# JuanJoZP/cfd-hemodynamic

Measured on AMD Instinct MI355X. Metric: time-steps/sec, dfg_1 ~1M DOF (stabilized_schur), higher is better.
Workload: dtype f64 (fp32 only in the AMG matrix values of the flexible preconditioner and in a read-only copy of the Krylov basis that Gram-Schmidt reads in solves of >= 20 iterations)

## Files before the change

### cfd_hemodynamic_amd/_lib.py

```python
from __future__ import annotations

import ctypes as C
import os
import subprocess

import numpy as np

_HERE = os.path.dirname(os.path.abspath(__file__))
_SO = os.path.join(_HERE, "libcfdh.so")
_LIB = None

dp = C.POINTER(C.c_double)
ip = C.POINTER(C.c_int32)
lp = C.POINTER(C.c_int64)


class Options(C.Structure):
    _fields_ = [
        ("snes_rtol", C.c_double), ("snes_atol", C.c_double), ("snes_stol", C.c_double), ("snes_max_it", C.c_int32),
        ("ksp_rtol", C.c_double), ("ksp_atol", C.c_double), ("ksp_max_it", C.c_int32), ("ksp_restart", C.c_int32),
        ("cheb_degree", C.c_int32), ("cheb_ratio", C.c_double), ("schur_full", C.c_int32),
        ("amg_smooth_degree", C.c_int32), ("amg_smooth_ratio", C.c_double), ("amg_theta", C.c_double),
        ("amg_max_coarse", C.c_int32), ("pc_refresh", C.c_int32), ("remove_p_mean", C.c_int32), ("verbose", C.c_int32),
        ("pc_type", C.c_int32), ("cc_smooth_degree", C.c_int32), ("ksp_guess", C.c_int32),
    ]


class Stats(C.Structure):
    _fields_ = [
        ("newton_its", C.c_int32), ("krylov_its", C.c_int32), ("reason", C.c_int32), ("pc_refreshes", C.c_int32),
        ("fnorm0", C.c_double), ("fnorm", C.c_double), ("ms_assemble", C.c_double), ("ms_solve", C.c_double),
        ("ms_pc_setup", C.c_double), ("ms_total", C.c_double),
    ]


class IpcsStats(C.Structure):
    _fields_ = [
        ("its", C.c_int32 * 3), ("reason", C.c_int32 * 3), ("rel_res", C.c_double * 3), ("ms_assemble", C.c_double),
        ("ms_solve", C.c_double * 3), ("ms_total", C.c_double), ("launches", C.c_int32), ("host_syncs", C.c_int32),
    ]


ALLREDUCE_FN = C.CFUNCTYPE(C.c_int, C.c_void_p, dp, C.c_int, C.c_int)
EXCHANGE_FN = C.CFUNCTYPE(C.c_int, C.c_void_p, dp, dp)

SYMBOLS = [
    "cfdh_create", "cfdh_create_elem", "cfdh_create_elem_part", "cfdh_set_facet_markers", "cfdh_destroy", "cfdh_last_error", "cfdh_abi_version", "cfdh_set_params", "cfdh_default_options",
    "cfdh_set_options", "cfdh_clear_dirichlet", "cfdh_add_dirichlet", "cfdh_update_dirichlet", "cfdh_set_state", "cfdh_get_solution",
    "cfdh_get_previous", "cfdh_get_residual", "cfdh_advance", "cfdh_advance_field", "cfdh_set_time_scheme", "cfdh_set_previous2", "cfdh_get_previous2",
    "cfdh_shift_history", "cfdh_set_boundary_terms", "cfdh_set_formulation", "cfdh_set_pressure_boundaries", "cfdh_assemble", "cfdh_get_csr", "cfdh_spmv", "cfdh_solve_step",
    "cfdh_functional", "cfdh_wall_shear_stress", "cfdh_set_global_pressure_space", "cfdh_set_halo", "cfdh_comm_unique_id", "cfdh_comm_init", "cfdh_comm_set_callbacks",
    "cfdh_profile_enable", "cfdh_profile_get", "cfdh_profile_reset", "cfdh_info",
    "cfdh_set_schur_pcd", "cfdh_set_ksp_forcing", "cfdh_get_newton_history", "cfdh_get_pcd_operator", "cfdh_apply_preconditioner",
    "cfdh_get_amg_operator", "cfdh_get_amg_vectors",
    "cfdh_create_ipcs", "cfdh_ipcs_set_form", "cfdh_ipcs_set_tolerances", "cfdh_ipcs_step", "cfdh_ipcs_get_operator", "cfdh_ipcs_get_intermediate",
    "cfdh_ipcs_apply_pressure_pc",
]


def build(force=False):
    src = os.path.join(_HERE, "csrc")
    newest = max(os.path.getmtime(os.path.join(src, f)) for f in os.listdir(src)
                 if f.endswith((".hip", ".cpp", ".hpp", ".h")))
    hdr = os.path.join(os.path.dirname(_HERE), "include", "cfdh.h")
    if os.path.exists(hdr):
        newest = max(newest, os.path.getmtime(hdr))
    if force or not os.path.exists(_SO) or os.path.getmtime(_SO) < newest:
        if not os.path.exists("/opt/rocm/bin/hipcc") and os.path.exists(_SO):
            return _SO
        subprocess.check_call(["make", "-C", src, "-s", "-j4"])
    return _SO


def lib():
    global _LIB
    if _LIB is not None:
        return _LIB
    if not os.path.exists(_SO):
        raise RuntimeError(
            "libcfdh.so is missing (%s): build it with `python -c 'import __graft_entry__ as g; g.build()'`; "
            "this package has no CPU fallback" % _SO)
    L = C.CDLL(_SO)
    vp = C.c_void_p
    L.cfdh_create.argtypes = [C.POINTER(vp), C.c_int, C.c_int, C.c_int64, C.c_int64, C.c_int64, ip, dp, C.c_int64, ip, ip, ip]
    L.cfdh_create_elem.argtypes = [C.POINTER(vp), C.c_int, C.c_int, C.c_int, C.c_int64, C.c_int64, ip, dp, C.c_int64, ip, ip, ip]
    L.cfdh_create_elem_part.argtypes = [C.POINTER(vp), C.c_int, C.c_int, C.c_int, C.c_int64, C.c_int64, C.c_int64, ip, dp, C.c_int64, ip, ip, ip]
    L.cfdh_set_facet_markers.argtypes = [vp, C.c_int64, ip]
    L.cfdh_destroy.argtypes = [vp]
    L.cfdh_destroy.restype = None
    L.cfdh_last_error.argtypes = [vp]
    L.cfdh_last_error.restype = C.c_char_p
    L.cfdh_set_params.argtypes = [vp, C.c_double, C.c_double, C.c_double, C.c_double, dp]
    L.cfdh_default_options.argtypes = [C.POINTER(Options)]
    L.cfdh_set_options.argtypes = [vp, C.POINTER(Options)]
    L.cfdh_clear_dirichlet.argtypes = [vp]
    L.cfdh_add_dirichlet.argtypes = [vp, C.c_int, C.c_int64, ip, dp]
    L.cfdh_update_dirichlet.argtypes = [vp, C.c_int, C.c_int64, ip, dp]
    L.cfdh_set_state.argtypes = [vp, dp, dp, dp, dp]
    L.cfdh_get_solution.argtypes = [vp, dp, dp]
    L.cfdh_set_time_scheme.argtypes = [vp, C.c_double, C.c_double, C.c_double, C.c_double]
    L.cfdh_set_previous2.argtypes = [vp, dp]
    L.cfdh_get_previous2.argtypes = [vp, dp]
    L.cfdh_shift_history.argtypes = [vp]
    L.cfdh_wall_shear_stress.argtypes = [vp, dp]
    L.cfdh_set_boundary_terms.argtypes = [vp, C.c_int, C.c_int, C.c_double]
    L.cfdh_set_formulation.argtypes = [vp, C.c_int]
    L.cfdh_set_pressure_boundaries.argtypes = [vp, C.c_int, ip, dp, C.c_double]
    L.cfdh_get_residual.argtypes = [vp, dp, dp]
    L.cfdh_get_previous.argtypes = [vp, dp, dp]
    L.cfdh_advance.argtypes = [vp]
    L.cfdh_advance_field.argtypes = [vp, C.c_int]
    L.cfdh_assemble.argtypes = [vp, C.c_int]
    L.cfdh_get_csr.argtypes = [vp, lp, ip, ip, dp]
    L.cfdh_spmv.argtypes = [vp, dp, dp]
    L.cfdh_solve_step.argtypes = [vp, C.POINTER(Stats)]
    L.cfdh_functional.argtypes = [vp, C.c_int, C.c_int, dp]
    L.cfdh_set_halo.argtypes = [vp, C.c_int, ip, lp, ip, lp, ip]
    L.cfdh_set_global_pressure_space.argtypes = [vp, C.c_int64, C.c_int64, ip, dp, ip, C.c_int64, ip]
    L.cfdh_comm_unique_id.argtypes = [C.c_void_p]
    L.cfdh_comm_init.argtypes = [vp, C.c_void_p, C.c_int, C.c_int]
    L.cfdh_comm_set_callbacks.argtypes = [vp, ALLREDUCE_FN, EXCHANGE_FN, C.c_void_p, C.c_int, C.c_int]
    L.cfdh_profile_enable.argtypes = [vp, C.c_int]
    L.cfdh_profile_get.argtypes = [vp, C.c_int, dp, lp]
    L.cfdh_profile_reset.argtypes = [vp]
    L.cfdh_info.argtypes = [vp, C.c_int]
    L.cfdh_info.restype = C.c_int64
    L.cfdh_set_schur_pcd.argtypes = [vp, C.c_int, C.c_int, C.c_int]
    L.cfdh_set_ksp_forcing.argtypes = [vp, C.c_int, C.c_double, C.c_double, C.c_double, C.c_double, C.c_double]
    L.cfdh_get_newton_history.argtypes = [vp, ip, dp, dp, ip, dp]
    L.cfdh_get_pcd_operator.argtypes = [vp, lp, ip, ip, dp, dp]
    L.cfdh_apply_preconditioner.argtypes = [vp, dp, dp]
    L.cfdh_get_amg_operator.argtypes = [vp, C.c_int, C.c_int, C.c_int, lp, lp, lp, ip, ip, dp]
    L.cfdh_get_amg_vectors.argtypes = [vp, C.c_int, C.c_int, C.c_int, lp, dp]
    L.cfdh_create_ipcs.argtypes = [C.POINTER(vp), C.c_int, C.c_int, C.c_int64, C.c_int64, C.c_int64, ip, dp, C.c_int64, ip, ip, ip]
    L.cfdh_ipcs_set_form.argtypes = [vp, C.c_double, C.c_double]
    L.cfdh_ipcs_set_tolerances.argtypes = [vp, dp, C.c_double, ip]
    L.cfdh_ipcs_step.argtypes = [vp, C.POINTER(IpcsStats)]
    L.cfdh_ipcs_get_operator.argtypes = [vp, C.c_int, lp, ip, ip, dp]
    L.cfdh_ipcs_get_intermediate.argtypes = [vp, C.c_int, dp]
    L.cfdh_ipcs_apply_pressure_pc.argtypes = [vp, dp, dp]
    _LIB = L
    return L


def _dp(a):
    return None if a is None else a.ctypes.data_as(dp)


def _ip(a):
    return None if a is None else a.ctypes.data_as(ip)


def _lp(a):
    return None if a is None else a.ctypes.data_as(lp)


class CfdhError(RuntimeError):
    pass


def _raise(code, msg):
    if code == -1:
        raise ValueError(msg)
    raise CfdhError(msg)


FORM_CONVECTIVE, FORM_ROTATIONAL = 0, 1
PC_SELFP, PC_CAHOUET_CHABARD, PC_PCD = 0, 1, 2
AMG_HIER_A, AMG_HIER_P, AMG_HIER_H = 0, 1, 2
AMG_OP_A, AMG_OP_P, AMG_OP_G, AMG_OP_SB, AMG_OP_SC = 0, 1, 2, 3, 4
(AMG_VEC_DINV, AMG_VEC_WDINV, AMG_VEC_AGG, AMG_VEC_COARSE_INV, AMG_VEC_D, AMG_VEC_LAMBDA, AMG_VEC_CC_SCALARS, AMG_VEC_CC_ML,
 AMG_VEC_CC_PBC, AMG_VEC_SPGEMM_ROWS, AMG_VEC_SHAPE, AMG_VEC_ORDER, AMG_VEC_A00_LMAX, AMG_VEC_A00_DINV) = range(14)
EW_DEFAULTS = (0.3, 0.9, 1.0, (1.0 + 5.0 ** 0.5) / 2.0, 0.1)


class Context:

    def __init__(self, x, cells, facet_cells, facet_local, facet_marker, nv_owned=None, device=0, etype=0):
        L = lib()
        self.L = L
        x = np.asarray(x, dtype=np.float64)
        cells = np.asarray(cells)
        self.etype = int(etype)
        self.dim = (3 if x.shape[1] >= 3 and cells.shape[1] in (8, 10) or (self.etype == 3 and cells.shape[1] == 4) else 2) if self.etype \
            else cells.shape[1] - 1
        if self.dim not in (2, 3) or x.shape[1] < self.dim:
            raise ValueError("cells must be triangles [nc,3] or tetrahedra [nc,4] with matching coordinates")
        nodes = {(1, 2): 6, (2, 2): 4, (3, 2): 3, (1, 3): 10, (2, 3): 8, (3, 3): 4}
        if self.etype and cells.shape[1] != nodes[(self.etype, self.dim)]:
            raise ValueError("element type %d needs %d nodes per cell for gdim %d" % (self.etype, nodes[(self.etype, self.dim)], self.dim))
        self.x = np.ascontiguousarray(x[:, : self.dim]).copy()
        self.cells = np.ascontiguousarray(cells, dtype=np.int32)
        self.nv = len(self.x)
        self.nvo = self.nv if nv_owned is None else int(nv_owned)
        fc = np.ascontiguousarray(facet_cells, dtype=np.int32)
        fl = np.ascontiguousarray(facet_local, dtype=np.int32)
        fm = np.ascontiguousarray(facet_marker, dtype=np.int32)
        h = C.c_void_p()
        if self.etype:
            if self.nvo != self.nv:
                rc = L.cfdh_create_elem_part(C.byref(h), int(device), self.dim, self.etype, self.nv, self.nvo, len(self.cells), _ip(self.cells),
                                             _dp(self.x), len(fc), _ip(fc), _ip(fl), _ip(fm))
            else:
                rc = L.cfdh_create_elem(C.byref(h), int(device), self.dim, self.etype, self.nv, len(self.cells), _ip(self.cells), _dp(self.x),
                                        len(fc), _ip(fc), _ip(fl), _ip(fm))
        else:
            rc = L.cfdh_create(C.byref(h), int(device), self.dim, self.nv, self.nvo, len(self.cells), _ip(self.cells), _dp(self.x),
                               len(fc), _ip(fc), _ip(fl), _ip(fm))
        if rc != 0:
            _raise(rc, "cfdh_create failed: " + L.cfdh_last_error(None).decode())
        self.h = h
        self._cb = None

    def close(self):
# ... 135 lines not shown
        if rc != 0:
            msg = self.L.cfdh_last_error(self.h).decode()
            if rc == -4:
                raise RuntimeError("Did not converge, reason: %d. (%s)" % (st.reason, msg))
            _raise(rc, msg)
        return st

    def functional(self, kind, marker=0):
        out = C.c_double()
        self._chk(self.L.cfdh_functional(self.h, int(kind), int(marker), C.byref(out)))
        return out.value

    def set_halo(self, nbr_rank, send_ptr, send_idx, recv_ptr, recv_idx):
        a = np.ascontiguousarray(nbr_rank, dtype=np.int32)
        sp_ = np.ascontiguousarray(send_ptr, dtype=np.int64)
        si = np.ascontiguousarray(send_idx, dtype=np.int32)
        rp = np.ascontiguousarray(recv_ptr, dtype=np.int64)
        ri = np.ascontiguousarray(recv_idx, dtype=np.int32)
        self._chk(self.L.cfdh_set_halo(self.h, len(a), _ip(a), _lp(sp_), _ip(si), _lp(rp), _ip(ri)))

    def set_global_pressure_space(self, x_global, cells_global, owned_global, pbc_nodes_global):
        xg = np.ascontiguousarray(x_global, dtype=np.float64)[:, : self.dim].copy()
        cg = np.ascontiguousarray(cells_global, dtype=np.int32)
        og = np.ascontiguousarray(owned_global, dtype=np.int32)
        pb = np.ascontiguousarray(pbc_nodes_global, dtype=np.int32)
        self._chk(self.L.cfdh_set_global_pressure_space(self.h, len(xg), len(cg), _ip(cg), _dp(xg), _ip(og), len(pb), _ip(pb)))

    def comm_init_rccl(self, uid_bytes, rank, nranks):
        buf = C.create_string_buffer(bytes(uid_bytes), 128)
        self._chk(self.L.cfdh_comm_init(self.h, buf, int(rank), int(nranks)))

    def comm_set_callbacks(self, allreduce, exchange, rank, nranks):
        self._cb = (ALLREDUCE_FN(allreduce), EXCHANGE_FN(exchange))
        self._chk(self.L.cfdh_comm_set_callbacks(self.h, self._cb[0], self._cb[1], None, int(rank), int(nranks)))

    def profile_enable(self, on=True):
        self._chk(self.L.cfdh_profile_enable(self.h, int(on)))

    def profile_reset(self):
        self._chk(self.L.cfdh_profile_reset(self.h))

    def profile_get(self, kind):
        ms, n = C.c_double(), C.c_int64()
        self._chk(self.L.cfdh_profile_get(self.h, int(kind), C.byref(ms), C.byref(n)))
        return ms.value, n.value

    def info(self, what):
        return int(self.L.cfdh_info(self.h, int(what)))

    def set_schur_pcd(self, inlet_marker, outlet_marker, time_term=1):
        self._chk(self.L.cfdh_set_schur_pcd(self.h, int(inlet_marker), int(outlet_marker), int(time_term)))

    def set_ksp_forcing(self, version=2, rtol_0=None, rtol_max=None, gamma=None, alpha=None, threshold=None):
        a = [d if v is None else float(v) for v, d in zip((rtol_0, rtol_max, gamma, alpha, threshold), EW_DEFAULTS)]
        self._chk(self.L.cfdh_set_ksp_forcing(self.h, int(version), *a))

    def newton_history(self):
        n = C.c_int32()
        self._chk(self.L.cfdh_get_newton_history(self.h, C.byref(n), None, None, None, None))
        fn, rt, rr = np.zeros(n.value), np.zeros(n.value), np.zeros(n.value)
        its = np.zeros(n.value, dtype=np.int32)
        self._chk(self.L.cfdh_get_newton_history(self.h, C.byref(n), _dp(fn), _dp(rt), _ip(its), _dp(rr)))
        return {"fnorm": fn, "ksp_rtol": rt, "ksp_its": its, "ksp_rel_res": rr}

    def get_pcd_operator(self):
        import scipy.sparse as sp
        nnz = C.c_int64()
        self._chk(self.L.cfdh_get_pcd_operator(self.h, C.byref(nnz), None, None, None, None))
        rowptr = np.empty(self.nvo + 1, dtype=np.int32)
        col = np.empty(nnz.value, dtype=np.int32)
        val = np.empty(nnz.value)
        md = np.empty(self.nvo)
        self._chk(self.L.cfdh_get_pcd_operator(self.h, C.byref(nnz), _ip(rowptr), _ip(col), _dp(val), _dp(md)))
        return sp.csr_matrix((val, col, rowptr), shape=(self.nvo, self.nv)), md

    def apply_preconditioner(self, r):
        r = np.ascontiguousarray(r, dtype=np.float64)
        if r.size != (self.dim + 1) * self.nv:
            raise ValueError("monolithic vector of (gdim + 1) nv entries expected")
        z = np.zeros_like(r)
        self._chk(self.L.cfdh_apply_preconditioner(self.h, _dp(r), _dp(z)))
        return z

    def get_amg_operator(self, hier, level, which, raw=False):
        import scipy.sparse as sp
        nr, nc, nnz = C.c_int64(), C.c_int64(), C.c_int64()
        self._chk(self.L.cfdh_get_amg_operator(self.h, int(hier), int(level), int(which), C.byref(nr), C.byref(nc), C.byref(nnz), None, None, None))
        rowptr = np.empty(nr.value + 1, dtype=np.int32)
        col = np.empty(nnz.value, dtype=np.int32)
        val = np.empty(nnz.value)
        self._chk(self.L.cfdh_get_amg_operator(self.h, int(hier), int(level), int(which), C.byref(nr), C.byref(nc), C.byref(nnz), _ip(rowptr),
                                               _ip(col), _dp(val)))
        if raw:
            return rowptr, col, val, (nr.value, nc.value), nnz.value
        return sp.csr_matrix((val, col, rowptr), shape=(nr.value, nc.value))

    def get_amg_vectors(self, hier, level, which):
        n = C.c_int64()
        self._chk(self.L.cfdh_get_amg_vectors(self.h, int(hier), int(level), int(which), C.byref(n), None))
        out = np.empty(n.value)
        self._chk(self.L.cfdh_get_amg_vectors(self.h, int(hier), int(level), int(which), C.byref(n), _dp(out)))
        return out


class IpcsContext(Context):

    def __init__(self, x, cells, nvert, facet_cells, facet_local, facet_marker, device=0):
        L = lib()
        self.L = L
        cells = np.ascontiguousarray(cells, dtype=np.int32)
        if cells.ndim != 2 or cells.shape[1] not in (6, 10):
            raise ValueError("cells must list the 6 nodes of P2 triangles or the 10 nodes of P2 tetrahedra")
        self.dim = 2 if cells.shape[1] == 6 else 3
        self.etype = 1
        self.x = np.ascontiguousarray(np.asarray(x, dtype=np.float64)[:, : self.dim]).copy()
        self.cells = cells
        self.nv = self.nvo = len(self.x)
        self.nvert = int(nvert)
        fc = np.ascontiguousarray(facet_cells, dtype=np.int32)
        fl = np.ascontiguousarray(facet_local, dtype=np.int32)
        fm = np.ascontiguousarray(facet_marker, dtype=np.int32)
        h = C.c_void_p()
        rc = L.cfdh_create_ipcs(C.byref(h), int(device), self.dim, self.nv, self.nvert, len(cells), _ip(cells), _dp(self.x), len(fc), _ip(fc), _ip(fl),
                                _ip(fm))
        if rc != 0:
            _raise(rc, "cfdh_create_ipcs failed: " + L.cfdh_last_error(None).decode())
        self.h = h
        self._cb = None

    def set_state(self, u_prev=None, p_prev=None, u=None, p=None):
        a = [None if v is None else np.ascontiguousarray(v, dtype=np.float64).reshape(-1) for v in (u_prev, p_prev, u, p)]
        for v, n in zip(a, (self.dim * self.nv, self.nvert, self.dim * self.nv, self.nvert)):
            if v is not None and v.size != n:
                raise ValueError("state array has wrong size")
        self._chk(self.L.cfdh_set_state(self.h, _dp(a[0]), _dp(a[1]), _dp(a[2]), _dp(a[3])))

    def get_solution(self, u=None, p=None):
        u = np.empty(self.dim * self.nv) if u is None else u
        p = np.empty(self.nvert) if p is None else p
        self._chk(self.L.cfdh_get_solution(self.h, _dp(u), _dp(p)))
        return u, p

    def get_previous(self, u=None, p=None):
        u = np.empty(self.dim * self.nv) if u is None else u
        p = np.empty(self.nvert) if p is None else p
        self._chk(self.L.cfdh_get_previous(self.h, _dp(u), _dp(p)))
        return u, p

    def set_form(self, conv_coeff, force_coeff):
        self._chk(self.L.cfdh_ipcs_set_form(self.h, float(conv_coeff), float(force_coeff)))

    def set_tolerances(self, rtol=(1e-5, 1e-5, 1e-5), atol=1e-50, max_it=(10000, 10000, 10000)):
        r = np.ascontiguousarray(np.broadcast_to(np.asarray(rtol, dtype=np.float64), (3,)))
        m = np.ascontiguousarray(np.broadcast_to(np.asarray(max_it, dtype=np.int32), (3,)))
        self._chk(self.L.cfdh_ipcs_set_tolerances(self.h, _dp(r), float(atol), _ip(m)))

    def step(self):
        st = IpcsStats()
        rc = self.L.cfdh_ipcs_step(self.h, C.byref(st))
        if rc != 0:
            msg = self.L.cfdh_last_error(self.h).decode()
            if rc == -4:
                bad = [r for r in st.reason if r <= 0]
                raise RuntimeError("Did not converge, reason: %d. (%s)" % (bad[0] if bad else 0, msg))
            _raise(rc, msg)
        return st
# ... 35 lines not shown
```

### cfd_hemodynamic_amd/csrc/cfdh_api.cpp

```cpp
#include <algorithm>
#include <cmath>
#include <numeric>

#include <dlfcn.h>

#include "cfdh_internal.hpp"
#include "cfdh_ipcs.hpp"

std::string g_cfdh_last_error;

int cfdh_prepare_assembly(cfdh_ctx *c);

#define ENTER(c)                         \
  do {                                   \
    if (!(c)) return CFDH_E_ARG;         \
    (void)hipSetDevice((c)->device);     \
  } while (0)

#define NOT_IPCS(c, name)                                                                                                    \
  do {                                                                                                                       \
    if ((c) && (c)->ipcs) return cfdh_fail((c), CFDH_E_STATE, name ": not available on an incremental pressure-correction context (cfdh_create_ipcs)"); \
  } while (0)
#define NEED_IPCS(c, name)                                                                                         \
  do {                                                                                                             \
    if (!(c)) return CFDH_E_ARG;                                                                                   \
    if (!(c)->ipcs) return cfdh_fail((c), CFDH_E_STATE, name ": the context was not created by cfdh_create_ipcs"); \
    (void)hipSetDevice((c)->device);                                                                               \
  } while (0)

static int ipcs_put(cfdh_ctx *c, dbuf<double> &dst, const double *src) {
  if (!src) return 0;
  c->ipcs->n_field_copies++;
  HIPCHK(c, hipMemcpyAsync(dst.p, src, sizeof(double) * dst.n, hipMemcpyHostToDevice, c->stream));
  HIPCHK(c, hipStreamSynchronize(c->stream));
  return 0;
}
static int ipcs_get(cfdh_ctx *c, const dbuf<double> &src, double *dst) {
  if (!dst) return 0;
  c->ipcs->n_field_copies++;
  HIPCHK(c, hipMemcpyAsync(dst, src.p, sizeof(double) * src.n, hipMemcpyDeviceToHost, c->stream));
  HIPCHK(c, hipStreamSynchronize(c->stream));
  return 0;
}
static int ipcs_copy(cfdh_ctx *c, const dbuf<double> &src, dbuf<double> &dst) {
  HIPCHK(c, hipMemcpyAsync(dst.p, src.p, sizeof(double) * src.n, hipMemcpyDeviceToDevice, c->stream));
  return 0;
}

extern "C" {

int cfdh_abi_version(void) { return CFDH_ABI_VERSION; }

const char *cfdh_last_error(const cfdh_ctx *c) { return c ? c->err.c_str() : g_cfdh_last_error.c_str(); }

int cfdh_default_options(cfdh_options *o) {
  if (!o) return CFDH_E_ARG;
  o->snes_rtol = 1e-8; o->snes_atol = 1e-50; o->snes_stol = 1e-8; o->snes_max_it = 100;
  o->ksp_rtol = 1e-5; o->ksp_atol = 1e-50; o->ksp_max_it = 1000; o->ksp_restart = 200;
  o->cheb_degree = 3; o->cheb_ratio = 10.0; o->schur_full = 2;
  o->amg_smooth_degree = 1; o->amg_smooth_ratio = 8.0; o->amg_theta = -1.0; o->amg_max_coarse = 1000;
  o->pc_refresh = 0; o->remove_p_mean = 1; o->verbose = 0; o->pc_type = 1; o->cc_smooth_degree = 2;
  o->ksp_guess = getenv("CFDH_KSP_GUESS") ? atoi(getenv("CFDH_KSP_GUESS")) : 4;
  return 0;
}

static int create_ctx(cfdh_ctx **out, int device, int gdim, int etype, int64_t nv, int64_t nv_owned, int64_t nc, const int32_t *cells,
                      const double *coords, int64_t nfacets, const int32_t *facet_cells, const int32_t *facet_local,
                      const int32_t *facet_marker) {
  if (!out) return cfdh_fail(nullptr, CFDH_E_ARG, "null output pointer");
  *out = nullptr;
  if (gdim != 2 && gdim != 3) return cfdh_fail(nullptr, CFDH_E_ARG, "gdim must be 2 (P1 triangles) or 3 (P1 tetrahedra)");
  if (etype < 0 || etype > 3) return cfdh_fail(nullptr, CFDH_E_ARG, "unknown element type %d", etype);
  if (!cells || !coords || (nfacets > 0 && (!facet_cells || !facet_local)))
    return cfdh_fail(nullptr, CFDH_E_ARG, "null mesh array");
  int ndev = 0;
  if (hipGetDeviceCount(&ndev) != hipSuccess || ndev <= 0)
    return cfdh_fail(nullptr, CFDH_E_HIP, "no HIP device available: libcfdh has no CPU fallback");
  if (device < 0 || device >= ndev) return cfdh_fail(nullptr, CFDH_E_ARG, "device %d out of range (%d devices)", device, ndev);
  cfdh_ctx *c = new (std::nothrow) cfdh_ctx();
  if (!c) return cfdh_fail(nullptr, CFDH_E_NOMEM, "out of host memory");
  c->device = device;
  cfdh_default_options(&c->opt);
  { const char *e = getenv("CFDH_NO_GRAPH"); c->use_graph = !(e && e[0] == '1'); }
  if (c->use_graph && (getenv("ROCP_TOOL_LIBRARIES") || dlsym(RTLD_DEFAULT, "rocprofiler_configure"))) {
    int rt = 0;
    const char *ov = getenv("CFDH_GRAPH_UNDER_PROFILER");
    if (!(ov && ov[0] == '1') && hipRuntimeGetVersion(&rt) == hipSuccess && rt >= 70200000) c->use_graph = false;
  }
  memset(&c->last_stats, 0, sizeof c->last_stats);
  int rc = 0;
  do {
    if (hipSetDevice(device) != hipSuccess) { rc = cfdh_fail(nullptr, CFDH_E_HIP, "hipSetDevice(%d) failed", device); break; }
    if (hipStreamCreateWithFlags(&c->stream, hipStreamNonBlocking) != hipSuccess) { rc = cfdh_fail(nullptr, CFDH_E_HIP, "hipStreamCreate failed"); break; }
    rc = gdim == 3 ? k3_upload_quadrature(c) : k_upload_quadrature(c);
    if (rc) break;
    if (etype != 0) {
      rc = gdim == 3 ? kg3_upload_tables(c) : kg_upload_tables(c);
      if (rc) break;
      rc = gdim == 3 ? cfdh_build_mesh_gen3(c, etype, nv, nv_owned, nc, cells, coords, nfacets, facet_cells, facet_local, facet_marker)
                     : cfdh_build_mesh_gen(c, etype, nv, nv_owned, nc, cells, coords, nfacets, facet_cells, facet_local, facet_marker);
      break;
    }
    rc = gdim == 3 ? cfdh_build_mesh3(c, nv, nv_owned, nc, cells, coords, nfacets, facet_cells, facet_local, facet_marker)
                   : cfdh_build_mesh(c, nv, nv_owned, nc, cells, coords, nfacets, facet_cells, facet_local, facet_marker);
  } while (0);
  if (rc) {
    g_cfdh_last_error = c->err.empty() ? g_cfdh_last_error : c->err;
    cfdh_destroy(c);
    return rc;
  }
  *out = c;
  return 0;
}

int cfdh_create(cfdh_ctx **out, int device, int gdim, int64_t nv, int64_t nv_owned, int64_t nc, const int32_t *cells,
                const double *coords, int64_t nfacets, const int32_t *facet_cells, const int32_t *facet_local,
                const int32_t *facet_marker) {
  return create_ctx(out, device, gdim, CFDH_ELEM_P1, nv, nv_owned, nc, cells, coords, nfacets, facet_cells, facet_local, facet_marker);
}

int cfdh_create_elem(cfdh_ctx **out, int device, int gdim, int elem, int64_t nn, int64_t nc, const int32_t *cells, const double *node_coords,
                     int64_t nfacets, const int32_t *facet_cells, const int32_t *facet_local, const int32_t *facet_marker) {
  return create_ctx(out, device, gdim, elem, nn, nn, nc, cells, node_coords, nfacets, facet_cells, facet_local, facet_marker);
}

int cfdh_create_elem_part(cfdh_ctx **out, int device, int gdim, int elem, int64_t nn, int64_t nn_owned, int64_t nc, const int32_t *cells,
                          const double *node_coords, int64_t nfacets, const int32_t *facet_cells, const int32_t *facet_local, const int32_t *facet_marker) {
  return create_ctx(out, device, gdim, elem, nn, nn_owned, nc, cells, node_coords, nfacets, facet_cells, facet_local, facet_marker);
}

void cfdh_destroy(cfdh_ctx *c) {
  if (!c) return;
  (void)hipSetDevice(c->device);
  if (c->stream) (void)hipStreamSynchronize(c->stream);
  cfdh_ipcs_free(c);
  comm_finalize(c);
  c->hS.clear(); c->hL.clear(); c->hA.clear(); c->hLg.clear();
  for (hipEvent_t e : c->ev_pool) (void)hipEventDestroy(e);
  for (auto &e : c->pc_graphs) for (auto &x : e.exec) if (x) (void)hipGraphExecDestroy(x);
  if (c->h_pinned) (void)hipHostFree(c->h_pinned);
  if (c->h_stage) (void)hipHostFree(c->h_stage);
  if (c->ev_h) (void)hipEventDestroy(c->ev_h);
  if (c->h_big) (void)hipHostFree(c->h_big);
  if (c->h_ring) (void)hipHostFree(c->h_ring);
  for (hipEvent_t e : c->ev_ring) if (e) (void)hipEventDestroy(e);
  hipStream_t s = c->stream;
  delete c;
  if (s) (void)hipStreamDestroy(s);
}

int cfdh_set_params(cfdh_ctx *c, double dt, double rho, double mu, double mu_facet, const double f[3]) {
  ENTER(c);
  if (!(dt > 0) || !(rho > 0) || !(mu > 0)) return cfdh_fail(c, CFDH_E_ARG, "dt, rho, mu must be positive");
  const bool changed = !c->params_set || dt != c->dt || rho != c->rho || mu != c->mu;
  c->dt = dt; c->rho = rho; c->mu = mu; c->muf = mu_facet;
  c->f[0] = f ? f[0] : 0.0; c->f[1] = f ? f[1] : 0.0; c->f[2] = (f && c->dim == 3) ? f[2] : 0.0;
  c->params_set = true;
  if (changed) { c->mom_valid = false; c->pc_valid = false; }
  if (c->ipcs) c->ipcs->assembled = false;
  return 0;
}

int cfdh_set_options(cfdh_ctx *c, const cfdh_options *o) {
  if (!c || !o) return CFDH_E_ARG;
  if (o->ksp_restart < 1 || o->ksp_restart > 1000 || o->cheb_degree < 1 || o->cc_smooth_degree < 1 || !(o->cheb_ratio > 1) || o->amg_smooth_degree < 1 ||
      !(o->amg_smooth_ratio > 1) || o->amg_max_coarse < 8 || o->amg_max_coarse > 4000 || o->ksp_guess < 0 || o->ksp_guess > 8)
    return cfdh_fail(c, CFDH_E_ARG, "option out of range");
  const bool pc_changed = o->amg_theta != c->opt.amg_theta || o->amg_max_coarse != c->opt.amg_max_coarse ||
                          o->amg_smooth_ratio != c->opt.amg_smooth_ratio || o->pc_type != c->opt.pc_type ||
                          o->amg_smooth_degree != c->opt.amg_smooth_degree ||
                          o->schur_full != c->opt.schur_full;
  c->opt = *o;
  if (pc_changed) c->pc_valid = false;
  if (pc_changed && c->ipcs) c->ipcs->pset_dirty = true;
  c->pc_graph_valid = false;
  return 0;
// ... 332 lines not shown
      return cfdh_fail(c, CFDH_E_ARG, "cfdh_set_pressure_boundaries: pressure boundaries need the rotational formulation (cfdh_set_formulation)");
  }
  bool same = (size_t)n == c->pb_markers.size() && beta_nitsche == c->pb_beta;
  for (int k = 0; same && k < n; k++) same = markers[k] == c->pb_markers[k];
  c->pb_values.assign(values, values + n);
  if (same) return 0;
  c->pb_markers.assign(markers, markers + n);
  c->pb_beta = beta_nitsche;
  return upload_cell_facet_flags(c);
}

int cfdh_set_schur_pcd(cfdh_ctx *c, int inlet_marker, int outlet_marker, int time_term) {
  NOT_IPCS(c, "cfdh_set_schur_pcd");
  ENTER(c);
  if (c->gen) return cfdh_fail(c, CFDH_E_ARG, "cfdh_set_schur_pcd: PCD exists for P1 triangles and tetrahedra on the closed-form kernels only");
  if (c->nranks > 1 || c->nvo != c->nv) return cfdh_fail(c, CFDH_E_ARG, "cfdh_set_schur_pcd: PCD is not available in partitioned runs");
  if (time_term != 0 && time_term != 1) return cfdh_fail(c, CFDH_E_ARG, "cfdh_set_schur_pcd: time_term must be 0 or 1");
  const bool markers_changed = !c->pcd_set || inlet_marker != c->pcd_in || outlet_marker != c->pcd_out;
  c->pcd_in = inlet_marker; c->pcd_out = outlet_marker; c->pcd_time = time_term;
  c->pcd_set = true;
  if (markers_changed) { c->pcd_ready = false; c->pc_valid = false; }
  return 0;
}

int cfdh_set_ksp_forcing(cfdh_ctx *c, int version, double rtol_0, double rtol_max, double gamma, double alpha, double threshold) {
  NOT_IPCS(c, "cfdh_set_ksp_forcing");
  ENTER(c);
  if (version != 0 && version != 2) return cfdh_fail(c, CFDH_E_ARG, "cfdh_set_ksp_forcing: version 0 (off) or 2");
  if (version == 2 && !(rtol_0 > 0 && rtol_0 < 1 && rtol_max > 0 && rtol_max < 1 && gamma > 0 && gamma <= 1 && alpha > 1 && alpha <= 2 &&
                        threshold > 0 && threshold < 1))
    return cfdh_fail(c, CFDH_E_ARG, "cfdh_set_ksp_forcing: need 0 < rtol_0, rtol_max, threshold < 1, 0 < gamma <= 1, 1 < alpha <= 2");
  c->ew_version = version;
  if (version == 2) { c->ew_rtol0 = rtol_0; c->ew_rtol_max = rtol_max; c->ew_gamma = gamma; c->ew_alpha = alpha; c->ew_threshold = threshold; }
  return 0;
}

int cfdh_get_newton_history(cfdh_ctx *c, int32_t *n, double *fnorm, double *ksp_rtol, int32_t *ksp_its, double *ksp_rel_res) {
  NOT_IPCS(c, "cfdh_get_newton_history");
  if (!c || !n) return CFDH_E_ARG;
  const size_t m = c->hist_fnorm.size();
  *n = (int32_t)m;
  for (size_t k = 0; k < m; k++) {
    if (fnorm) fnorm[k] = c->hist_fnorm[k];
    if (ksp_rtol) ksp_rtol[k] = c->hist_rtol[k];
    if (ksp_its) ksp_its[k] = c->hist_its[k];
    if (ksp_rel_res) ksp_rel_res[k] = c->hist_relres[k];
  }
  return 0;
}

int cfdh_get_pcd_operator(cfdh_ctx *c, int64_t *nnz, int32_t *rowptr, int32_t *col, double *vals, double *mass_diag) {
  NOT_IPCS(c, "cfdh_get_pcd_operator");
  if (!c || !nnz) return CFDH_E_ARG;
  ENTER(c);
  *nnz = c->nnzv;
  if (!rowptr && !col && !vals && !mass_diag) return 0;
  if (!rowptr || !col || !vals) return cfdh_fail(c, CFDH_E_ARG, "pass all of rowptr/col/vals or none");
  if (c->gen || c->nranks > 1 || c->nvo != c->nv) return cfdh_fail(c, CFDH_E_ARG, "cfdh_get_pcd_operator: P1 contexts on one GPU only");
  if (!c->pcd_set) return cfdh_fail(c, CFDH_E_STATE, "cfdh_get_pcd_operator: cfdh_set_schur_pcd was not called");
  if (!c->params_set || !c->state_set) return cfdh_fail(c, CFDH_E_STATE, "cfdh_get_pcd_operator: parameters and state are needed");
  CHK(k_pcd_assemble(c, c->x.p));
  std::vector<double> K(c->pcd_K.n);
  std::vector<int> sptr(c->pcd_sptr.n);
  HIPCHK(c, hipMemcpyAsync(K.data(), c->pcd_K.p, sizeof(double) * K.size(), hipMemcpyDeviceToHost, c->stream));
  HIPCHK(c, hipMemcpyAsync(sptr.data(), c->pcd_sptr.p, sizeof(int) * sptr.size(), hipMemcpyDeviceToHost, c->stream));
  HIPCHK(c, hipStreamSynchronize(c->stream));
  const int nvo = c->nvo;
  int64_t pos = 0;
  std::vector<std::pair<int, int>> ord;
  for (int vu = 0; vu < nvo; vu++) {
    const int r = c->perm[vu];
    ord.clear();
    for (int k = c->h_vptr[r]; k < c->h_vptr[r + 1]; k++) ord.push_back({c->iperm[c->h_vcol[k]], k - c->h_vptr[r]});
    std::sort(ord.begin(), ord.end());
    rowptr[vu] = (int32_t)pos;
    const size_t base = (size_t)sptr[r >> 6] + (r & 63);
    for (auto &e : ord) { col[pos] = e.first; vals[pos] = K[base + 64 * (size_t)e.second]; pos++; }
  }
  rowptr[nvo] = (int32_t)pos;
  if (mass_diag) for (int vu = 0; vu < nvo; vu++) mass_diag[vu] = c->h_pcd_md[c->perm[vu]];
  return 0;
}

int cfdh_apply_preconditioner(cfdh_ctx *c, const double *r, double *z) {
  NOT_IPCS(c, "cfdh_apply_preconditioner");
  if (!c || !r || !z) return CFDH_E_ARG;
  ENTER(c);
  if (!c->jac_valid) return cfdh_fail(c, CFDH_E_STATE, "no Jacobian assembled yet");
  CHK(cfdh_pc_update(c, false));
  std::vector<double> h;
  pack_vec(c, r, r + (size_t)c->dim * c->nv, h, nullptr);
  CHK(upload_vec(c, h, c->xt.p));
  CHK(cfdh_pc_apply(c, c->xt.p, c->dvec.p));
  std::vector<double> o;
  CHK(download_vec(c, c->dvec.p, o));
  for (int k = 0; k < c->nvo; k++) {
    const int v = c->iperm[k], d = c->dim;
    for (int i = 0; i < d; i++) z[(size_t)d * v + i] = o[(size_t)d * k + i];
    z[(size_t)d * c->nv + v] = o[(size_t)d * c->nvo + k];
  }
  return 0;
}

static int amg_pick(cfdh_ctx *c, const char *name, int hier, int level, AmgHier **H, AmgLevel **L) {
  if (c->nranks > 1 || c->nvo != c->nv) return cfdh_fail(c, CFDH_E_STATE, "%s: one GPU only", name);
  if (!c->pc_valid) return cfdh_fail(c, CFDH_E_STATE, "%s: no preconditioner built yet (cfdh_apply_preconditioner or cfdh_solve_step first)", name);
  *H = nullptr;
  if (hier == CFDH_AMG_HIER_H) {
    if (c->opt.pc_type != 1 || c->Hlev.n <= 0) return cfdh_fail(c, CFDH_E_STATE, "%s: H exists for pc_type 1 only", name);
    *L = &c->Hlev;
    return 0;
  }
  if (hier != CFDH_AMG_HIER_A && hier != CFDH_AMG_HIER_P) return cfdh_fail(c, CFDH_E_ARG, "%s: unknown hierarchy %d", name, hier);
  if (hier == CFDH_AMG_HIER_A && c->opt.pc_type == 0) return cfdh_fail(c, CFDH_E_STATE, "%s: pc_type 0 has no velocity hierarchy", name);
  AmgHier *h = hier == CFDH_AMG_HIER_A ? &c->hA : (c->opt.pc_type == 0 ? &c->hS : &c->hL);
  if (!h->valid) return cfdh_fail(c, CFDH_E_STATE, "%s: hierarchy %d is not built", name, hier);
  if (level < 0 || level >= (int)h->lev.size()) return cfdh_fail(c, CFDH_E_ARG, "%s: level %d of %d", name, level, (int)h->lev.size());
  *H = h;
  *L = h->lev[level];
  return 0;
}

int cfdh_get_amg_operator(cfdh_ctx *c, int hier, int level, int which, int64_t *nrow, int64_t *ncol, int64_t *nnz, int32_t *rowptr,
                          int32_t *col, double *vals) {
  NOT_IPCS(c, "cfdh_get_amg_operator");
  if (!c || !nrow || !ncol || !nnz) return CFDH_E_ARG;
  ENTER(c);
  AmgHier *H = nullptr;
  AmgLevel *L = nullptr;
  CHK(amg_pick(c, "cfdh_get_amg_operator", hier, level, &H, &L));
  if (which < CFDH_AMG_OP_A || which > CFDH_AMG_OP_SC) return cfdh_fail(c, CFDH_E_ARG, "cfdh_get_amg_operator: unknown operator %d", which);
  if (!H) level = 0;
  const CsrDev &M = which == CFDH_AMG_OP_A ? L->A : which == CFDH_AMG_OP_P ? L->P : which == CFDH_AMG_OP_G ? L->G : which == CFDH_AMG_OP_SB ? L->Sb : L->Sc;
  if (M.n <= 0 || !M.rowptr.p || !M.col.p || !M.val.p)
    return cfdh_fail(c, CFDH_E_STATE, "cfdh_get_amg_operator: operator %d of level %d is not kept in fp64 CSR (P: CFDH_AMG_KEEP=1 before the build)", which, level);
  *nrow = M.n; *ncol = M.m; *nnz = M.nnz;
  if (!rowptr && !col && !vals) return 0;
  if (!rowptr || !col || !vals) return cfdh_fail(c, CFDH_E_ARG, "pass all of rowptr/col/vals or none");
  std::vector<int> rp((size_t)M.n + 1), cl((size_t)M.nnz);
  std::vector<double> vl((size_t)M.nnz);
  HIPCHK(c, hipMemcpyAsync(rp.data(), M.rowptr.p, sizeof(int) * rp.size(), hipMemcpyDeviceToHost, c->stream));
  if (M.nnz > 0) {
    HIPCHK(c, hipMemcpyAsync(cl.data(), M.col.p, sizeof(int) * cl.size(), hipMemcpyDeviceToHost, c->stream));
    HIPCHK(c, hipMemcpyAsync(vl.data(), M.val.p, sizeof(double) * vl.size(), hipMemcpyDeviceToHost, c->stream));
  }
  HIPCHK(c, hipStreamSynchronize(c->stream));
  if (rp[M.n] != M.nnz) return cfdh_fail(c, CFDH_E_STATE, "cfdh_get_amg_operator: rowptr ends at %d, the operator holds %d entries", rp[M.n], M.nnz);
  const bool rows0 = level == 0 && which != CFDH_AMG_OP_G && (int)c->perm.size() == M.n;
  const bool cols0 = level == 0 && (which == CFDH_AMG_OP_A || which == CFDH_AMG_OP_SB || which == CFDH_AMG_OP_G) && (int)c->iperm.size() == M.m;
  int64_t pos = 0;
  std::vector<std::pair<int, double>> row;
  for (int ru = 0; ru < M.n; ru++) {
    const int r = rows0 ? c->perm[ru] : ru;
    rowptr[ru] = (int32_t)pos;
    row.clear();
    for (int k = rp[r]; k < rp[r + 1]; k++) row.push_back({cols0 ? c->iperm[cl[k]] : cl[k], vl[k]});
    if (cols0) std::stable_sort(row.begin(), row.end(), [](const std::pair<int, double> &a, const std::pair<int, double> &b) { return a.first < b.first; });
    for (auto &e : row) { col[pos] = e.first; vals[pos] = e.second; pos++; }
  }
  rowptr[M.n] = (int32_t)pos;
  return 0;
}

int cfdh_get_amg_vectors(cfdh_ctx *c, int hier, int level, int which, int64_t *n, double *out) {
  NOT_IPCS(c, "cfdh_get_amg_vectors");
  if (!c || !n) return CFDH_E_ARG;
  ENTER(c);
  AmgHier *H = nullptr;
  AmgLevel *L = nullptr;
  CHK(amg_pick(c, "cfdh_get_amg_vectors", hier, level, &H, &L));
  if (!H) level = 0;
  const bool perm0 = level == 0 && (int)c->perm.size() == L->n;
  auto fetch = [&](const void *src, size_t bytes, void *dst) -> int {
    HIPCHK(c, hipMemcpyAsync(dst, src, bytes, hipMemcpyDeviceToHost, c->stream));
    HIPCHK(c, hipStreamSynchronize(c->stream));
    return 0;
  };
  const int nvo = c->nvo;
  switch (which) {
    case CFDH_AMG_VEC_DINV:
    case CFDH_AMG_VEC_WDINV: {
      const dbuf<double> &v = which == CFDH_AMG_VEC_DINV ? L->dinv : L->wdinv;
// ... 444 lines not shown
      case 26: return I->D;
      case 29: return I->NL;
      case 80: return I->last.launches;
      case 81: return I->nvert;
      case 82: return I->n_field_copies;
      case 83: return 1;
      default: return -1;
    }
  }
  switch (what) {
    case 0: return c->nvo;
    case 1: return c->nv;
    case 2: return c->nc;
    case 3: return c->nnzv;
    case 4: return c->opt.pc_type >= 1 ? c->hL.fine_nnz : c->hS.fine_nnz;
    case 5: return c->ninc;
    case 6: return (int64_t)(c->opt.pc_type >= 1 ? c->hL.lev.size() : c->hS.lev.size());
    case 7: return c->nblk;
    case 8: return c->hA.fine_nnz;
    case 9: return c->gp_allgather ? c->gp_maxcnt : 0;
    case 10: return c->nccl_comm ? 1 : 0;
    case 11: return c->dl0.on ? c->dl0.n1 : 0;
    case 12: return c->ras ? 1 : 0;
    case 13: return c->n_allreduce;
    case 14: return c->n_halo;
    case 15: return c->n_host_sync;
    case 16: return c->n_krylov;
    case 17: return c->n_allgather;
    case 18: return c->nranks;
    case 26: return c->dim;
    case 30: case 31: case 32: case 33: case 34: case 35: case 36: case 37: case 38: case 39:
    case 40: case 41: case 42: case 43: case 44: case 45: case 46: case 47: case 48: case 49:
    case 50: case 51: case 52: case 53: case 54: case 55: case 56: case 57: case 58: case 59:
    case 60: case 61: case 62: case 63: case 64: case 65: case 66: case 67: case 68: case 69: {
      const AmgHier &h = what < 50 ? c->hA : (c->opt.pc_type >= 1 ? c->hL : c->hS);
      const size_t l = (size_t)(what % 10);
      if (l >= h.lev.size()) return 0;
      return ((what / 10) & 1) ? (int64_t)h.lev[l]->n : (int64_t)h.lev[l]->A.nnz;
    }
    case 28: return c->etype;
    case 70: return c->n_guess_solves;
    case 71: return c->n_guess_solves ? (int64_t)(1e6 * c->guess_reduction_sum / (double)c->n_guess_solves) : 0;
    case 29: return c->nloc;
    case 73: return c->n_krylov_discarded;
    case 74: return c->n_pc_builds;
    case 75: return c->pc_valid ? 1 : 0;
    case 76: return c->singular;
    case 77: return c->form;
    case 78: return c->opt.pc_type;
    case 79: return c->ew_version;
    case 72: return c->n_attainable_stops;
    case 27: return (int64_t)(1000.0 * c->ms_pc_build_dev);
    case 19: return c->opt.pc_type >= 1 ? c->hL.nnz_S0 : c->hS.nnz_S0;
    case 20: return c->hA.nnz_S0;
    case 21: return c->opt.pc_type >= 1 ? c->hL.nnz_G0 : c->hS.nnz_G0;
    case 22: return c->hA.nnz_G0;
    case 23: { const AmgHier &h = c->opt.pc_type >= 1 ? c->hL : c->hS; return h.lev.size() > 1 ? h.lev[1]->n : 0; }
    case 24: return c->hA.lev.size() > 1 ? c->hA.lev[1]->n : 0;
    case 25: { const AmgHier &h = c->opt.pc_type >= 1 ? c->hL : c->hS; return h.fused ? 1 : 0; }
    default: return -1;
  }
}


int cfdh_create_ipcs(cfdh_ctx **out, int device, int gdim, int64_t nn, int64_t nvert, int64_t nc, const int32_t *cells, const double *node_coords,
                     int64_t nfacets, const int32_t *facet_cells, const int32_t *facet_local, const int32_t *facet_marker) {
  if (!out) return cfdh_fail(nullptr, CFDH_E_ARG, "null output pointer");
  *out = nullptr;
  if (gdim != 2 && gdim != 3) return cfdh_fail(nullptr, CFDH_E_ARG, "gdim must be 2 (P2/P1 triangles) or 3 (P2/P1 tetrahedra)");
  if (!cells || !node_coords || nfacets < 0 || (nfacets > 0 && (!facet_cells || !facet_local))) return cfdh_fail(nullptr, CFDH_E_ARG, "null mesh array");
  int ndev = 0;
  if (hipGetDeviceCount(&ndev) != hipSuccess || ndev <= 0)
    return cfdh_fail(nullptr, CFDH_E_HIP, "no HIP device available: libcfdh has no CPU fallback");
  if (device < 0 || device >= ndev) return cfdh_fail(nullptr, CFDH_E_ARG, "device %d out of range (%d devices)", device, ndev);
  cfdh_ctx *c = new (std::nothrow) cfdh_ctx();
  if (!c) return cfdh_fail(nullptr, CFDH_E_NOMEM, "out of host memory");
  c->device = device;
  cfdh_default_options(&c->opt);
  c->use_graph = false;
  memset(&c->last_stats, 0, sizeof c->last_stats);
  int rc = 0;
  if (hipSetDevice(device) != hipSuccess) rc = cfdh_fail(nullptr, CFDH_E_HIP, "hipSetDevice(%d) failed", device);
  else if (hipStreamCreateWithFlags(&c->stream, hipStreamNonBlocking) != hipSuccess) rc = cfdh_fail(nullptr, CFDH_E_HIP, "hipStreamCreate failed");
  else rc = cfdh_ipcs_create(c, gdim, nn, nvert, nc, cells, node_coords, nfacets, facet_cells, facet_local, facet_marker);
  if (rc) {
    g_cfdh_last_error = c->err.empty() ? g_cfdh_last_error : c->err;
    cfdh_destroy(c);
    return rc;
  }
  *out = c;
  return 0;
}

int cfdh_ipcs_set_form(cfdh_ctx *c, double conv_coeff, double force_coeff) {
  NEED_IPCS(c, "cfdh_ipcs_set_form");
  if (!(conv_coeff >= 0) || !std::isfinite(conv_coeff) || !std::isfinite(force_coeff)) return cfdh_fail(c, CFDH_E_ARG, "cfdh_ipcs_set_form: conv_coeff >= 0 and finite coefficients");
  c->ipcs->conv_coeff = conv_coeff; c->ipcs->force_coeff = force_coeff; c->ipcs->force_default = false;
  c->ipcs->assembled = false;
  return 0;
}

int cfdh_ipcs_set_tolerances(cfdh_ctx *c, const double rtol[3], double atol, const int32_t max_it[3]) {
  NEED_IPCS(c, "cfdh_ipcs_set_tolerances");
  if (!rtol || !max_it || !(atol >= 0)) return cfdh_fail(c, CFDH_E_ARG, "cfdh_ipcs_set_tolerances: bad arguments");
  for (int k = 0; k < 3; k++)
    if (!(rtol[k] >= 0) || !(rtol[k] < 1) || max_it[k] < 1) return cfdh_fail(c, CFDH_E_ARG, "cfdh_ipcs_set_tolerances: 0 <= rtol < 1, max_it >= 1");
  for (int k = 0; k < 3; k++) { c->ipcs->rtol[k] = rtol[k]; c->ipcs->max_it[k] = max_it[k]; }
  c->ipcs->atol = atol;
  return 0;
}

int cfdh_ipcs_step(cfdh_ctx *c, cfdh_ipcs_stats *stats) {
  NEED_IPCS(c, "cfdh_ipcs_step");
  c->err.clear();
  cfdh_ipcs_stats st;
  const int rc = cfdh_ipcs_step_impl(c, &st);
  if (stats) *stats = st;
  return rc;
}

int cfdh_ipcs_get_operator(cfdh_ctx *c, int which, int64_t *nnz, int32_t *rowptr, int32_t *col, double *vals) {
  NEED_IPCS(c, "cfdh_ipcs_get_operator");
  IpcsData *I = c->ipcs;
  const int D = I->D;
  if (!nnz || which < 0 || which >= 3 + 2 * D) return cfdh_fail(c, CFDH_E_ARG, "cfdh_ipcs_get_operator: which in [0, %d)", 3 + 2 * D);
  const std::vector<int> &ptr = which == 1 ? I->hL.rowptr : which < 3 ? I->hM.rowptr : which < 3 + D ? I->bptr : I->gptr;
  const std::vector<int> &cl = which == 1 ? I->hL.col : which < 3 ? I->hM.col : which < 3 + D ? I->bcol : I->gcol;
  *nnz = (int64_t)cl.size();
  if (!rowptr && !col && !vals) return 0;
  if (!rowptr || !col || !vals) return cfdh_fail(c, CFDH_E_ARG, "pass all of rowptr/col/vals or none");
  std::copy(ptr.begin(), ptr.end(), rowptr);
  std::copy(cl.begin(), cl.end(), col);
  if (which >= 3) {
    const std::vector<double> &v = which < 3 + D ? I->hB : I->hG;
    const int d = which < 3 + D ? which - 3 : which - 3 - D;
    for (size_t k = 0; k < cl.size(); k++) vals[k] = v[(size_t)D * k + d];
    return 0;
  }
  if (which == 0) {
    if (!I->assembled) CHK(cfdh_ipcs_assemble(c));
  } else {
    if (!c->params_set) return cfdh_fail(c, CFDH_E_STATE, "cfdh_set_params was not called");
    I->assembled = false;
    CHK(cfdh_ipcs_assemble(c));
  }
  const double *src = which == 0 ? I->A1v.p : which == 1 ? I->Lv.p : I->RMv.p;
  HIPCHK(c, hipMemcpyAsync(vals, src, sizeof(double) * cl.size(), hipMemcpyDeviceToHost, c->stream));
  HIPCHK(c, hipStreamSynchronize(c->stream));
  return 0;
}

int cfdh_ipcs_get_intermediate(cfdh_ctx *c, int which, double *out) {
  NEED_IPCS(c, "cfdh_ipcs_get_intermediate");
  IpcsData *I = c->ipcs;
  if (!out || which < 0 || which > 4) return cfdh_fail(c, CFDH_E_ARG, "cfdh_ipcs_get_intermediate: which in [0, 4]");
  const dbuf<double> *src[5] = {&I->us, &I->phi, &I->b1, &I->b2, &I->b3};
  I->n_field_copies++;
  HIPCHK(c, hipMemcpyAsync(out, src[which]->p, sizeof(double) * src[which]->n, hipMemcpyDeviceToHost, c->stream));
  HIPCHK(c, hipStreamSynchronize(c->stream));
  return 0;
}

int cfdh_ipcs_apply_pressure_pc(cfdh_ctx *c, const double *r, double *z) {
  NEED_IPCS(c, "cfdh_ipcs_apply_pressure_pc");
  if (!r || !z) return cfdh_fail(c, CFDH_E_ARG, "cfdh_ipcs_apply_pressure_pc: null array");
  return cfdh_ipcs_apply_pc(c, r, z);
// ... 4 lines not shown
```

### cfd_hemodynamic_amd/csrc/cfdh_internal.hpp

```cpp
#pragma once
#include <hip/hip_runtime.h>

#include <cstdint>
#include <cstdio>
#include <cstring>
#include <string>
#include <vector>

#include "cfdh.h"

#ifndef CFDH_MAX_INC
#define CFDH_MAX_INC 256
#endif
#ifndef CFDH_MAX_BV
#define CFDH_MAX_BV 192
#endif
#ifndef CFDH_MAX_BC
#define CFDH_MAX_BC 192
#endif
#ifndef CFDH_MAX_ROWS
#define CFDH_MAX_ROWS 128
#endif

#if defined(__HIPCC__)
__device__ __forceinline__ double cfdh_rsqrt(double x) {
  double y = __builtin_amdgcn_rsq(x);
  const double h = 0.5 * x;
  y = __builtin_fma(y, __builtin_fma(-h * y, y, 0.5), y);
  y = __builtin_fma(y, __builtin_fma(-h * y, y, 0.5), y);
  return y;
}
#endif

template <class T>
struct dbuf {
  T *p = nullptr;
  size_t n = 0;
  dbuf() = default;
  dbuf(const dbuf &) = delete;
  dbuf &operator=(const dbuf &) = delete;
  ~dbuf() { release(); }
  void release() {
    if (p) (void)hipFree(p);
    p = nullptr;
    n = 0;
  }
  hipError_t alloc(size_t count) {
    if (count == n && p) return hipSuccess;
    release();
    if (count == 0) return hipSuccess;
    hipError_t e = hipMalloc((void **)&p, count * sizeof(T));
    if (e == hipSuccess) n = count;
    return e;
  }
  hipError_t upload(const std::vector<T> &h, hipStream_t s) {
    hipError_t e = alloc(h.size());
    if (e != hipSuccess || h.empty()) return e;
    return hipMemcpyAsync(p, h.data(), h.size() * sizeof(T), hipMemcpyHostToDevice, s);
  }
  hipError_t zero(hipStream_t s) { return n ? hipMemsetAsync(p, 0, n * sizeof(T), s) : hipSuccess; }
  void adopt(dbuf &o) {
    if (&o == this) return;
    release();
    p = o.p; n = o.n;
    o.p = nullptr; o.n = 0;
  }
};

struct CsrHost {
  int n = 0, m = 0;
  std::vector<int> rowptr, col;
  std::vector<double> val;
  int nnz() const { return (int)col.size(); }
};

struct CsrDev {
  int n = 0, m = 0, nnz = 0;
  dbuf<int> rowptr, col;
  dbuf<double> val;
  int nslice = 0, sell_maxw = 0;
  dbuf<int> sptr, scol;
  dbuf<float> sval, svalw;
  dbuf<float> valf;
};
enum { CFDH_UP_CSR = 1, CFDH_UP_SELL = 2, CFDH_UP_CSRF = 4};

struct AmgLevel {
  int n = 0;
  CsrDev A, P, R;
  dbuf<double> dinv, wdinv, x, b, r, d0, d1;
  double lmax = 0, lmin = 0;
  CsrDev G, Sb, Sc;
  dbuf<float> D;
  int Dn = 0;
  bool fine = false;
  bool sell = false;
  dbuf<int> agg;
};

struct AmgHier {
  std::vector<AmgLevel *> lev;
  dbuf<double> coarse_inv;
  int coarse_n = 0, ncol = 1;
  long long fine_nnz = 0;
  bool valid = false;
  bool fused = false;
  long long nnz_G0 = 0, nnz_S0 = 0;
  long long spgemm_rows[3] = {0, 0, 0};
  bool keep_host0 = false;
  CsrHost h_A0, h_P0;
  std::vector<double> h_wdinv0;
  void clear() {
    for (AmgLevel *l : lev) delete l;
    lev.clear();
    valid = false;
// ... 59 lines not shown
  bool jac_valid = false;

  int ninc = 0, nblk = 0;
  bool gs_refine_long = false;
  dbuf<unsigned> inc_slot;
  dbuf<unsigned> inc_rank;
  dbuf<int> blk_row;
  dbuf<int> blk_vptr, blk_vlist;
  dbuf<int> blk_cptr, blk_clist;
  dbuf<unsigned> inc_loc;
  dbuf<int> wave_maxlen;

  int a3_nblk = 0;
  dbuf<int> a3_blk_row, a3_blk_iptr;
  dbuf<int> a3_inc_cell;
  dbuf<int> a3_inc_row;
  dbuf<unsigned long long> a3_inc_slots;

  std::vector<unsigned char> h_bcflag;
  std::vector<double> h_bcval;
  std::vector<double> h_bcmult;
  bool bc_dirty = true;
  std::vector<int> bc_touched, bc_pending;
  size_t bc_touched_sent = 0;
  std::vector<int> bc_mark;
  int bc_epoch = 0;
  bool bc_full_upload = true;
  dbuf<int> bc_uidx;
  dbuf<unsigned char> bc_uflag;
  dbuf<double> bc_uval, bc_umult;
  int n_pbc = 0;
  dbuf<unsigned char> bcflag;
  dbuf<double> bcval, bcmult;

  dbuf<int> d_fac_cell, d_fac_local, d_fac_marker;

  dbuf<double> x, xt, xprev, xprev2, F, dvec;
  dbuf<double> wss;
  double ts_theta = 0.5, ts_a[3] = {1.0, -1.0, 0.0};
  bool ds_terms = true;
  double bf_beta = 0.0;
  int bf_marker = -1;
  int form = 0;
  std::vector<int> pb_markers;
  std::vector<double> pb_values;
  double pb_beta = 0.0;
  bool state_set = false;

  dbuf<double> red_partial, red_out;
  double *h_pinned = nullptr;
  double *h_stage = nullptr;
  double *h_pinned_dev = nullptr;
  const double *mirror_src = nullptr;
  int mirror_cnt = 0;
  hipEvent_t ev_h = nullptr;
  static constexpr int KRING = 12;
  double *h_ring = nullptr, *h_ring_dev = nullptr;
  size_t h_ring_stride = 0;
  hipEvent_t ev_ring[KRING] = {};
  long long n_krylov_discarded = 0;
  int red_blocks = 0;

  int kry_m = 0;
  static constexpr int GUESS_NEWTON = 4;
  dbuf<double> guessU, guessX;
  bool guess_stored[GUESS_NEWTON] = {false, false, false, false};
  int guess_m = 0, guess_slot = -1;
  int guess_cnt[GUESS_NEWTON] = {0, 0, 0, 0}, guess_head[GUESS_NEWTON] = {0, 0, 0, 0};
  long long n_guess_solves = 0;
  double guess_reduction_sum = 0.0;
  dbuf<double> kV, kZ, kw, kh;
  dbuf<float> kV32;
  bool krylov_fp32_ok = true;
  int guess_last_its[4] = {0, 0, 0, 0};
  dbuf<double> ky;

  dbuf<double> dinvA;
  double lmaxA = 0;
  dbuf<double> pu0, pu1, pu2, pr, pp0, pp1;
  dbuf<double> prand;
  dbuf<double> cheb_coef;
  struct PcGraph { const double *r; double *z; hipGraphExec_t exec[6]; };
  std::vector<PcGraph> pc_graphs;
  bool pc_graph_valid = false, capturing = false, use_graph = true;
  AmgHier hS;
  AmgHier hL;
  AmgHier hA;
  AmgLevel Hlev;
  dbuf<double> ccMl;
  dbuf<unsigned char> ccPbc;
  double cc_alpha = 0, cc_beta = 0;
  int up0_rows = 0;
  struct Epilogue { bool on = false, done = false; double alpha = 0, beta = 0; const double *zH = nullptr, *r = nullptr; const unsigned char *pbc = nullptr; double *out = nullptr; } epi;
  std::vector<double> h_Lval, h_Ml;
  dbuf<double> d_Lval, d_Ml;
  dbuf<double> amg_rand;
  double ms_pc_build_dev = 0;
  long long bc_version = 0;
  int gp_n = 0;
  CsrHost gp_L;
  bool gp_singular = false, gp_dirty = false;
  AmgHier hLg;
  dbuf<int> gp_l2g;
  dbuf<double> gp_rhs, gp_sol;
  bool ras = false;
  std::vector<int> h_gid;
  std::vector<int> h_g2l;
  dbuf<double> ras_b, ras_x;
  struct RasPlan {
    bool ready = false;
    int maxlen = 0;
    int nent = 0;
    dbuf<int> gptr, gcol, gsrc;
    dbuf<double> gval;
  } rasp;
  struct DistL0 {
    bool on = false;
    bool ghost_rhs = true;
    int n1 = 0;
    CsrDev A;
    CsrDev P;
    CsrDev PT;
    dbuf<double> wdinv, b, xa, r, x1;
  } dl0;
  bool gp_allgather = false;
  int gp_maxcnt = 0;
  dbuf<int> gp_send_idx;
  dbuf<int> gp_src_idx;
  dbuf<double> gp_sendbuf, gp_recvbuf;
  dbuf<double> pcw;
  double *h_big = nullptr;
  size_t h_big_n = 0;
  std::vector<unsigned char> hL_pbc;
  int hL_singular = -1;
  bool pc_valid = false;
  int pc_its_ref = 0;
  int steps_since_refresh = 0;
  int singular = 0;

  int nnbr = 0;
  std::vector<int> nbr_rank;
  std::vector<long long> send_ptr, recv_ptr;
  dbuf<int> send_idx;
  dbuf<double> send_buf;
  std::vector<double> h_send, h_recv;
  int rank = 0, nranks = 1;
  double nvo_global = 0;
  void *nccl_comm = nullptr;
  cfdh_allreduce_fn cb_ar = nullptr;
  cfdh_exchange_fn cb_ex = nullptr;
  void *cb_user = nullptr;

  bool prof_on = false;
  ProfSlot prof[12];
  std::vector<hipEvent_t> ev_pool;
  struct EvRec { int kind; hipEvent_t a, b; };
  std::vector<EvRec> ev_pending;
  size_t ev_next = 0;

  cfdh_stats last_stats;
  long long n_allreduce = 0, n_halo = 0, n_host_sync = 0, n_krylov = 0, n_allgather = 0;
  long long n_attainable_stops = 0;
  long long n_pc_builds = 0;

  bool pcd_set = false, pcd_ready = false;
  int pcd_in = -1, pcd_out = -1, pcd_time = 0;
// ... 2 lines not shown
  dbuf<unsigned> pcd_islot, pcd_fslot;
  dbuf<int> pcd_sptr, pcd_scol, pcd_rlen;
  dbuf<double> pcd_K, pcd_mdinv, pcd_t, pcd_q;
  dbuf<float> pcd_Kf;
  dbuf<unsigned char> pcd_flag;
  std::vector<double> h_pcd_md;
  int ew_version = 0;
  double ew_rtol0 = 0.3, ew_rtol_max = 0.9, ew_gamma = 1.0, ew_alpha = 1.6180339887498949, ew_threshold = 0.1;
  std::vector<double> hist_fnorm, hist_rtol, hist_relres;
  std::vector<int> hist_its;
  double ksp_last_relres = 0;
};

#define CFDH_MAX_PBND 8

int cfdh_fail(cfdh_ctx *c, int code, const char *fmt, ...);
#define HIPCHK(c, call)                                                                           \
  do {                                                                                            \
    hipError_t e_ = (call);                                                                       \
    if (e_ != hipSuccess) return cfdh_fail((c), CFDH_E_HIP, "%s: %s (%s:%d)", #call, hipGetErrorString(e_), \
                                           __FILE__, __LINE__);                                   \
  } while (0)
#define CHK(call)            \
  do {                       \
    int r_ = (call);         \
    if (r_ != 0) return r_;  \
  } while (0)

int cfdh_build_mesh(cfdh_ctx *c, int64_t nv, int64_t nvo, int64_t nc, const int32_t *cells, const double *coords,
                    int64_t nfac, const int32_t *fcell, const int32_t *flocal, const int32_t *fmarker);
int cfdh_amg_setup(cfdh_ctx *c, AmgHier &H, const CsrHost &A, bool singular, int ncol);
int cfdh_level_setup(cfdh_ctx *c, AmgLevel &L, const CsrHost &A, double ratio, int ncol, std::vector<double> *w_out = nullptr);
int cfdh_upload_csr(cfdh_ctx *c, const CsrHost &H, CsrDev &D, const std::vector<double> *colw = nullptr, int parts = CFDH_UP_CSR | CFDH_UP_SELL);
int cfdh_aggregate_host_csr(const CsrHost &A, double theta, std::vector<int> &agg);

bool cfdh_amg_dev_enabled(const cfdh_ctx *c);
int cfdh_amg_setup_dev(cfdh_ctx *c, AmgHier &H, CsrDev &A0, bool singular, int ncol);
int cfdh_level_setup_dev(cfdh_ctx *c, AmgLevel &L, CsrDev &A, double ratio, int ncol);
int cfdh_proxy_dev(cfdh_ctx *c, CsrDev &out);
int cfdh_proxy_ras_dev(cfdh_ctx *c, CsrDev &out);
int cfdh_cc_h_dev(cfdh_ctx *c, double alpha, double beta, CsrDev &out);

#define CFDH3_MAX_SLOTS 320
int cfdh_build_mesh3(cfdh_ctx *c, int64_t nv, int64_t nvo, int64_t nc, const int32_t *cells, const double *coords,
                     int64_t nfac, const int32_t *fcell, const int32_t *flocal, const int32_t *fmarker);
int k3_upload_quadrature(cfdh_ctx *c);
int k3_moments(cfdh_ctx *c);
int k3_assemble(cfdh_ctx *c, const double *xstate, int mode);
int k3_spmv_full(cfdh_ctx *c, const double *x, double *y);
int k3_spmv_full_multi(cfdh_ctx *c, const double *X, double *Y, int ld, int nvec);
int k3_spmv_block(cfdh_ctx *c, int blk, const double *x, double *y, const double *b);
int k3_spmv_block_ghost(cfdh_ctx *c, int blk, const double *xv, double *y, const double *b);
int k3_nullspace_test(cfdh_ctx *c, double *nrm, double *absnrm);
int k3_functional(cfdh_ctx *c, int kind, int marker, double *out);
int k3_wss(cfdh_ctx *c, double *out);

int kg_upload_tables(cfdh_ctx *c);
int cfdh_build_mesh_gen(cfdh_ctx *c, int etype, int64_t nv, int64_t nv_owned, int64_t nc, const int32_t *cells, const double *coords, int64_t nfac,
                        const int32_t *fcell, const int32_t *flocal, const int32_t *fmarker);
int cfdh_gen_element_stiffness(const cfdh_ctx *c, const int32_t *v, const double *X, double *K);
int cfdh_facet_nodes(const cfdh_ctx *c, int f, int out[3]);
int kg_assemble(cfdh_ctx *c, const double *xstate, int mode);
int kg_functional_partials(cfdh_ctx *c, int kind, int marker, int nb);
int kg_wss(cfdh_ctx *c, double *out);

int kg3_upload_tables(cfdh_ctx *c);
int cfdh_build_mesh_gen3(cfdh_ctx *c, int etype, int64_t nv, int64_t nv_owned, int64_t nc, const int32_t *cells, const double *coords, int64_t nfac,
                         const int32_t *fcell, const int32_t *flocal, const int32_t *fmarker);
int cfdh_gen3_element_stiffness(const cfdh_ctx *c, const int32_t *v, const double *X, double *K);
int cfdh_facet_nodes3(const cfdh_ctx *c, int f, int out[8]);
int kg3_assemble(cfdh_ctx *c, const double *xstate, int mode);
int kg3_functional_partials(cfdh_ctx *c, int kind, int marker, int nb);
int kg3_wss(cfdh_ctx *c, double *out);

int cfdh_pcd_setup(cfdh_ctx *c);
int k_pcd_assemble(cfdh_ctx *c, const double *xstate);
int k_pcd_apply(cfdh_ctx *c, const double *r, double *s);

void prof_begin(cfdh_ctx *c, int kind);
void prof_end(cfdh_ctx *c, int kind);
void prof_flush(cfdh_ctx *c);

int k_upload_quadrature(cfdh_ctx *c);
int k_halo_pack(cfdh_ctx *c, const double *vec);
int v_pointwise_mult(cfdh_ctx *c, int n, const double *a, const double *b, double *out);
int k_moments(cfdh_ctx *c);
int k_assemble(cfdh_ctx *c, const double *xstate, int mode);
int k_spmv_full(cfdh_ctx *c, const double *x, double *y);
int k_spmv_full_multi(cfdh_ctx *c, const double *X, double *Y, int ld, int nvec);
int k_spmv_block(cfdh_ctx *c, int blk, const double *x, double *y, const double *b, double alpha);
int k_spmv_block_ghost(cfdh_ctx *c, int blk, const double *xv, double *y, const double *b);
int k_extract_diag(cfdh_ctx *c);
int k_cheb_a00(cfdh_ctx *c, const double *b, double *x);
int k_cheb_a00_coeffs(cfdh_ctx *c);
int k_csr_spmv(cfdh_ctx *c, const CsrDev &A, const double *x, double *y, int mode, const double *b);
int k_csr_spmv_ncol(cfdh_ctx *c, const CsrDev &A, const double *x, double *y, int mode, const double *b, int ncol);
int k_amg_vcycle(cfdh_ctx *c, AmgHier &H, const double *b, double *x);
int k_level_smooth(cfdh_ctx *c, AmgLevel *L, const double *b, double *x, int degree);
bool k_cc_cheb2_scale(cfdh_ctx *c, AmgLevel *L, const double *b, double *x, const double *ml, double *y);
int k_cc_scale(cfdh_ctx *c, int n, const double *ml, const double *z, double *y);
int k_dl0_down(cfdh_ctx *c, const double *halo_vec);
int k_dl0_up(cfdh_ctx *c, double *out);
int k_ext_pack(cfdh_ctx *c, const double *vec, double *out);
int k_scatter_global(cfdh_ctx *c, int n, const int *l2g, const double *loc, double *glob);
int k_gather_global(cfdh_ctx *c, int n, const int *l2g, const double *glob, double *loc);
int k_cc_combine(cfdh_ctx *c, int n, double alpha, double beta, const double *t, const double *z, const double *r, const unsigned char *pbc, double *out, double *out2 = nullptr);
int k_nullspace_test(cfdh_ctx *c, double *nrm, double *absnrm);
int k_bc_scatter(cfdh_ctx *c, int n, int ncomp, const int *idx, const unsigned char *flag, const double *val, const double *mult);

int v_copy(cfdh_ctx *c, int n, const double *x, double *y);
int v_zero(cfdh_ctx *c, int n, double *y);
int v_axpy(cfdh_ctx *c, int n, double a, const double *x, double *y);
int v_waxpy(cfdh_ctx *c, int n, double a, const double *x, const double *y, double *w);
int v_scale(cfdh_ctx *c, int n, double a, double *x);
int v_dot(cfdh_ctx *c, int n, const double *x, const double *y, double *out_host);
int v_norm2(cfdh_ctx *c, int n, const double *x, double *out_host);
int v_norminf_diff(cfdh_ctx *c, int n, const double *x, const double *y, double *out_host);
int v_sub_mean(cfdh_ctx *c, int n, double *p);
int v_multidot(cfdh_ctx *c, int n, const double *V, int ld, int nvec, const double *w, double *h_dev, bool with_ww, double *mirror = nullptr,
               bool reduce_ranks = true);
int v_scale_to(cfdh_ctx *c, int n, double a, const double *x, double *y);
int v_multidot32(cfdh_ctx *c, int n, const float *V, int ld, int nvec, const double *w, double *h_dev, double *mirror);
int v_gs_update32(cfdh_ctx *c, int n, const float *V, int ld, int nvec, const double *h_dev, const double *w, double *vn, float *v32n,
                  double *s_dev, double *mirror);
int v_store32(cfdh_ctx *c, int n, const double *v, float *v32);
int v_gram(cfdh_ctx *c, int n, const double *W, int ld, int k, const double *b, double *out_dev);
int v_multiaxpy(cfdh_ctx *c, int n, const double *V, int ld, int nvec, const double *h_dev, double *w);
int v_gs_update_normalize(cfdh_ctx *c, int n, const double *V, int ld, int nvec, const double *h_dev, const double *w, double *vn, double *s_dev);
int v_norm_to_dev(cfdh_ctx *c, int n, const double *w, double *out_dev);
int v_norm_to_dev_local(cfdh_ctx *c, int n, const double *w, double *out_dev);
int v_scale_inv_dev(cfdh_ctx *c, int n, const double *w, const double *nrm_dev, double *v);
int v_lincomb(cfdh_ctx *c, int n, const double *Z, int ld, int nvec, const double *y_dev, double *x);
int v_pack_state(cfdh_ctx *c, const double *u_user, const double *p_user, double *dst);
int k_functional(cfdh_ctx *c, int kind, int marker, double *out);
int k_wss(cfdh_ctx *c, double *out);

int comm_allreduce_dev(cfdh_ctx *c, double *dev, int n, int op);
int comm_allgather_dev(cfdh_ctx *c, const double *send, double *recv, int count);
int comm_halo(cfdh_ctx *c, double *vec);
int comm_finalize(cfdh_ctx *c);

int cfdh_pc_update(cfdh_ctx *c, bool force_refresh);
int cfdh_pc_apply(cfdh_ctx *c, const double *r, double *z);
int cfdh_host_threads();
int cfdh_fgmres(cfdh_ctx *c, const double *b, double *x, int *its, int *reason, double bnorm = -1.0);
int v_norm2_pair(cfdh_ctx *c, int n, const double *x, const double *y, double *nx, double *ny);
int cfdh_newton_step(cfdh_ctx *c, cfdh_stats *st);
int cfdh_download_blocks(cfdh_ctx *c, std::vector<double> &a00, std::vector<double> &a01, std::vector<double> &a10,
                         std::vector<double> &a11);
```

### cfd_hemodynamic_amd/csrc/cfdh_kernels.hip

```cpp
#include <hip/hip_runtime.h>

#include <cmath>

#include "cfdh_internal.hpp"
#include "cfdh_quad_tri.h"

#define TPB 256
#define NTLOAD(p) __builtin_nontemporal_load(p)

__constant__ double d_qw[CFDH_NQ];
__constant__ double d_ql[CFDH_NQ][3];

int k_upload_quadrature(cfdh_ctx *c) {
  HIPCHK(c, hipMemcpyToSymbol(HIP_SYMBOL(d_qw), CFDH_QW, sizeof(CFDH_QW)));
  HIPCHK(c, hipMemcpyToSymbol(HIP_SYMBOL(d_ql), CFDH_QL, sizeof(CFDH_QL)));
  return 0;
}

void prof_begin(cfdh_ctx *c, int kind) {
  if (!c->prof_on || c->capturing) return;
  if (c->ev_next + 2 > c->ev_pool.size()) {
    for (int i = 0; i < 64; i++) { hipEvent_t e; if (hipEventCreate(&e) != hipSuccess) return; c->ev_pool.push_back(e); }
  }
  cfdh_ctx::EvRec r;
  r.kind = kind; r.a = c->ev_pool[c->ev_next++]; r.b = c->ev_pool[c->ev_next++];
  (void)hipEventRecord(r.a, c->stream);
  c->ev_pending.push_back(r);
}
void prof_end(cfdh_ctx *c, int kind) {
  if (!c->prof_on || c->capturing || c->ev_pending.empty()) return;
  (void)kind;
  (void)hipEventRecord(c->ev_pending.back().b, c->stream);
  if (c->ev_pending.size() >= 4096) prof_flush(c);
}
void prof_flush(cfdh_ctx *c) {
  if (c->ev_pending.empty()) return;
  (void)hipStreamSynchronize(c->stream);
  for (auto &r : c->ev_pending) {
    float ms = 0;
    if (hipEventElapsedTime(&ms, r.a, r.b) == hipSuccess) { c->prof[r.kind].total_ms += ms; c->prof[r.kind].launches++; }
  }
  c->ev_pending.clear();
  c->ev_next = 0;
}

#include "cfdh_wave.hpp"

__device__ __forceinline__ int uoff(int w, int nvo) { return w < nvo ? 2 * w : 3 * w; }
__device__ __forceinline__ int poff(int w, int nvo) { return w < nvo ? 2 * nvo + w : 3 * w + 2; }

__global__ __launch_bounds__(TPB) void moments_kernel(int nc, int nvo, const int *__restrict__ cells,
                                                      const double *__restrict__ coords,
                                                      const double *__restrict__ un, double *__restrict__ mom,
                                                      double dt, double nu) {
  int e = blockIdx.x * TPB + threadIdx.x;
  if (e >= nc) return;
  int v0 = cells[3 * e], v1 = cells[3 * e + 1], v2 = cells[3 * e + 2];
  double2 X0 = *(const double2 *)(coords + 2 * v0), X1 = *(const double2 *)(coords + 2 * v1), X2 = *(const double2 *)(coords + 2 * v2);
  double u0x = un[uoff(v0, nvo)], u0y = un[uoff(v0, nvo) + 1];
  double u1x = un[uoff(v1, nvo)], u1y = un[uoff(v1, nvo) + 1];
  double u2x = un[uoff(v2, nvo)], u2y = un[uoff(v2, nvo) + 1];
  double det = (X1.x - X0.x) * (X2.y - X0.y) - (X1.y - X0.y) * (X2.x - X0.x);
  double area = 0.5 * fabs(det);
  double d01 = hypot(X0.x - X1.x, X0.y - X1.y), d12 = hypot(X1.x - X2.x, X1.y - X2.y), d20 = hypot(X2.x - X0.x, X2.y - X0.y);
  double h = fmax(d01, fmax(d12, d20));
  double ih2 = 1.0 / (h * h);
  double t2 = 4.0 / (dt * dt), t3 = 16.0 * nu * nu * ih2 * ih2;
  double hr = h / (2.0 * nu);
  double m00 = 0, m01 = 0, m02 = 0, m11 = 0, m12 = 0, m22 = 0, L = 0;
#pragma unroll 7
  for (int q = 0; q < CFDH_NQ; q++) {
    double l0 = d_ql[q][0], l1 = d_ql[q][1], l2 = d_ql[q][2], wq = d_qw[q];
    double ux = l0 * u0x + l1 * u1x + l2 * u2x;
    double uy = l0 * u0y + l1 * u1y + l2 * u2y;
    double s = ux * ux + uy * uy;
    double t1 = fmax(4.0 * s, 1e-30) * ih2;
    double tau = cfdh_rsqrt(t1 + t2 + t3);
    double vn = s > 1e-280 ? s * cfdh_rsqrt(s) : 0.0;
    double Re = vn * hr;
    double z = (Re <= 3.0) ? Re * (1.0 / 3.0) : 1.0;
    double tl = vn * h * z * 0.5;
    double w = wq * tau;
    m00 += w * l0 * l0; m01 += w * l0 * l1; m02 += w * l0 * l2;
    m11 += w * l1 * l1; m12 += w * l1 * l2; m22 += w * l2 * l2;
    L += wq * tl;
  }
  double4 *o = (double4 *)(mom + 8 * (size_t)e);
  o[0] = make_double4(area * m00, area * m01, area * m02, area * m11);
  o[1] = make_double4(area * m12, area * m22, area * L, 0.0);
}

int k_moments(cfdh_ctx *c) {
  if (c->gen) { c->mom_valid = true; return 0; }
  if (c->dim == 3) return k3_moments(c);
// ... 386 lines not shown
        if (fl0 & 2u) { J00[0][1][1] = p.bcmult[3 * row + 1]; Fr[1] = xrow[1] - p.bcval[3 * row + 1]; }
        if (fl0 & 4u) { J11[0] = p.bcmult[3 * row + 2]; Fr[2] = xrow[2] - p.bcval[3 * row + 2]; }
      }
      if (WJ) {
        const size_t s0 = sb + (meta & 255);
        *(double2 *)(p.A00 + 4 * s0) = make_double2(J00[0][0][0], J00[0][0][1]);
        *(double2 *)(p.A00 + 4 * s0 + 2) = make_double2(J00[0][1][0], J00[0][1][1]);
        *(double2 *)(p.A01 + 2 * s0) = make_double2(J01[0][0], J01[0][1]);
        *(double2 *)(p.A10 + 2 * s0) = make_double2(J10[0][0], J10[0][1]);
        p.A11[s0] = J11[0];
      }
      *(double2 *)(p.F + 2 * (size_t)row) = make_double2(Fr[0], Fr[1]);
      p.F[2 * (size_t)nvo + row] = Fr[2];
    }
  }
#ifdef CFDH_ASM_TIMING
  __builtin_amdgcn_s_waitcnt(0);
  ts[5] = __builtin_readcyclecounter();
  if (t == 0 && p.dbg)
    for (int k = 0; k < 6; k++) p.dbg[8 * (size_t)blk + k] = ts[k];
#endif
}

int k_assemble(cfdh_ctx *c, const double *xstate, int mode) {
  if (c->gen) return c->dim == 3 ? kg3_assemble(c, xstate, mode) : kg_assemble(c, xstate, mode);
  if (c->dim == 3) return k3_assemble(c, xstate, mode);
  AsmArgs a;
  a.coords = c->coords.p; a.mom = c->mom.p; a.x = xstate; a.un = c->xprev.p; a.un2 = c->xprev2.p; a.bcval = c->bcval.p; a.bcmult = c->bcmult.p;
  a.vptr = c->vptr.p;
  a.blk_vptr = c->blk_vptr.p; a.blk_vlist = c->blk_vlist.p; a.blk_cptr = c->blk_cptr.p; a.blk_clist = c->blk_clist.p; a.inc_loc = c->inc_loc.p; a.wave_maxlen = c->wave_maxlen.p;
  a.blk_row = c->blk_row.p;
  a.inc_slot = c->inc_slot.p; a.inc_rank = c->inc_rank.p; a.cflag = c->cflag.p; a.bcflag = c->bcflag.p;
  a.A00 = c->A00.p; a.A01 = c->A01.p; a.A10 = c->A10.p; a.A11 = c->A11.p; a.F = c->F.p;
  a.nvo = c->nvo; a.dt = c->dt; a.rho = c->rho; a.mu = c->mu; a.muf = c->muf; a.fx = c->f[0]; a.fy = c->f[1];
  a.theta = c->ts_theta; a.a0 = c->ts_a[0]; a.a1 = c->ts_a[1]; a.a2 = c->ts_a[2];
  a.beta_bf = c->bf_beta * c->rho; a.ds_terms = c->ds_terms ? 1 : 0;
  const bool hist2 = c->ts_a[2] != 0.0;
#ifdef CFDH_ASM_TIMING
  static long long *dbg = nullptr;
  static int dbg_calls = 0;
  if (!dbg) hipMalloc(&dbg, sizeof(long long) * 8 * (size_t)c->nblk);
  a.dbg = dbg;
#endif
  prof_begin(c, 0);
  const dim3 gr(c->nblk), bl(CFDH_MAX_INC);
  const bool bf = c->bf_beta > 0.0 && c->bf_marker >= 0;
#define CFDH_ASM_LAUNCH(H2, BFV)                                                                   \
  do {                                                                                             \
    if (mode == 1) hipLaunchKernelGGL((asm_kernel<1, H2, BFV>), gr, bl, 0, c->stream, a);         \
    else if (mode == 2) hipLaunchKernelGGL((asm_kernel<2, H2, BFV>), gr, bl, 0, c->stream, a);    \
    else hipLaunchKernelGGL((asm_kernel<0, H2, BFV>), gr, bl, 0, c->stream, a);                   \
  } while (0)
  if (!hist2 && !bf) CFDH_ASM_LAUNCH(false, false);
  else if (hist2 && !bf) CFDH_ASM_LAUNCH(true, false);
  else if (!hist2 && bf) CFDH_ASM_LAUNCH(false, true);
  else CFDH_ASM_LAUNCH(true, true);
#undef CFDH_ASM_LAUNCH
  prof_end(c, 0);
  HIPCHK(c, hipGetLastError());
#ifdef CFDH_ASM_TIMING
  if (mode == 1 && (++dbg_calls % 20) == 0) {
    std::vector<long long> h(8 * (size_t)c->nblk);
    hipStreamSynchronize(c->stream);
    hipMemcpy(h.data(), dbg, sizeof(long long) * h.size(), hipMemcpyDeviceToHost);
    double acc[5] = {0, 0, 0, 0, 0};
    long long tmin = h[0], tmax = h[5];
    for (int b = 0; b < c->nblk; b++) {
      for (int k = 0; k < 5; k++) acc[k] += (double)(h[8 * (size_t)b + k + 1] - h[8 * (size_t)b + k]);
      tmin = std::min(tmin, h[8 * (size_t)b]); tmax = std::max(tmax, h[8 * (size_t)b + 5]);
    }
    fprintf(stderr, "[asm timing] ticks per block: stage-issue %.0f, barrier %.0f, element %.0f, reduce %.0f, stores+drain %.0f; kernel span %lld ticks, %d blocks\n",
            acc[0] / c->nblk, acc[1] / c->nblk, acc[2] / c->nblk, acc[3] / c->nblk, acc[4] / c->nblk, tmax - tmin, c->nblk);
  }
#endif
  if (mode == 1) c->jac_valid = true;
  return 0;
}

__global__ __launch_bounds__(TPB) void spmv_full_kernel(int nvo, const int *__restrict__ vptr,
                                                        const int *__restrict__ vcol, const double *__restrict__ A00,
                                                        const double *__restrict__ A01, const double *__restrict__ A10,
                                                        const double *__restrict__ A11, const double *__restrict__ x,
                                                        double *__restrict__ y) {
  const int gid = blockIdx.x * TPB + threadIdx.x;
  const int row = gid >> 3, l = gid & 7;
  double a0 = 0, a1 = 0, a2 = 0;
  if (row < nvo) {
    const int ks = vptr[row], ke = vptr[row + 1];
    for (int k = ks + l; k < ke; k += 8) {
      const int w = vcol[k];
      const int uo = uoff(w, nvo), po = poff(w, nvo);
      const double xu0 = x[uo], xu1 = x[uo + 1], xp = x[po];
      const double2 b0 = *(const double2 *)(A00 + 4 * (size_t)k), b1 = *(const double2 *)(A00 + 4 * (size_t)k + 2);
      const double2 c01 = *(const double2 *)(A01 + 2 * (size_t)k), c10 = *(const double2 *)(A10 + 2 * (size_t)k);
      const double c11 = A11[k];
      a0 += b0.x * xu0 + b0.y * xu1 + c01.x * xp;
      a1 += b1.x * xu0 + b1.y * xu1 + c01.y * xp;
      a2 += c10.x * xu0 + c10.y * xu1 + c11 * xp;
    }
  }
  a0 = group8_sum(a0); a1 = group8_sum(a1); a2 = group8_sum(a2);
  if (row < nvo && l == 0) {
    *(double2 *)(y + 2 * (size_t)row) = make_double2(a0, a1);
    y[2 * (size_t)nvo + row] = a2;
  }
}


template <int NV>
__global__ __launch_bounds__(TPB) void spmv_full_multi_kernel(int nvo, const int *__restrict__ vptr, const int *__restrict__ vcol,
                                                              const double *__restrict__ A00, const double *__restrict__ A01,
                                                              const double *__restrict__ A10, const double *__restrict__ A11,
                                                              const double *__restrict__ X, double *__restrict__ Y, size_t ld) {
  const int gid = blockIdx.x * TPB + threadIdx.x;
  const int row = gid >> 3, l = gid & 7;
  double a0[NV], a1[NV], a2[NV];
#pragma unroll
  for (int v = 0; v < NV; v++) a0[v] = a1[v] = a2[v] = 0.0;
  if (row < nvo) {
    const int ks = vptr[row], ke = vptr[row + 1];
    for (int k = ks + l; k < ke; k += 8) {
      const int w = vcol[k];
      const int uo = uoff(w, nvo), po = poff(w, nvo);
      const double2 b0 = *(const double2 *)(A00 + 4 * (size_t)k), b1 = *(const double2 *)(A00 + 4 * (size_t)k + 2);
      const double2 c01 = *(const double2 *)(A01 + 2 * (size_t)k), c10 = *(const double2 *)(A10 + 2 * (size_t)k);
      const double c11 = A11[k];
#pragma unroll
      for (int v = 0; v < NV; v++) {
        const double *x = X + (size_t)v * ld;
        const double xu0 = x[uo], xu1 = x[uo + 1], xp = x[po];
        a0[v] += b0.x * xu0 + b0.y * xu1 + c01.x * xp;
        a1[v] += b1.x * xu0 + b1.y * xu1 + c01.y * xp;
        a2[v] += c10.x * xu0 + c10.y * xu1 + c11 * xp;
      }
    }
  }
#pragma unroll
  for (int v = 0; v < NV; v++) {
    const double s0 = group8_sum(a0[v]), s1 = group8_sum(a1[v]), s2 = group8_sum(a2[v]);
    if (row < nvo && l == 0) {
      double *y = Y + (size_t)v * ld;
      *(double2 *)(y + 2 * (size_t)row) = make_double2(s0, s1);
      y[2 * (size_t)nvo + row] = s2;
    }
  }
}

int k_spmv_full_multi(cfdh_ctx *c, const double *X, double *Y, int ld, int nvec) {
  if (c->dim == 3) return k3_spmv_full_multi(c, X, Y, ld, nvec);
  if (nvec < 2 || nvec > 4) {
    for (int v = 0; v < nvec; v++) CHK(k_spmv_full(c, X + (size_t)v * ld, Y + (size_t)v * ld));
    return 0;
  }
  const long long nthreads = 8ll * c->nvo;
  const dim3 gr((unsigned)((nthreads + TPB - 1) / TPB)), bl(TPB);
#define CFDH_SPMM(NV) hipLaunchKernelGGL((spmv_full_multi_kernel<NV>), gr, bl, 0, c->stream, c->nvo, c->vptr.p, c->vcol.p, c->A00.p, \
                                         c->A01.p, c->A10.p, c->A11.p, X, Y, (size_t)ld)
  if (nvec == 2) CFDH_SPMM(2); else if (nvec == 3) CFDH_SPMM(3); else CFDH_SPMM(4);
#undef CFDH_SPMM
  HIPCHK(c, hipGetLastError());
  return 0;
}

int k_spmv_full(cfdh_ctx *c, const double *x, double *y) {
  if (c->dim == 3) return k3_spmv_full(c, x, y);
  const long long nthreads = 8ll * c->nvo;
  prof_begin(c, 1);
  hipLaunchKernelGGL(spmv_full_kernel, dim3((unsigned)((nthreads + TPB - 1) / TPB)), dim3(TPB), 0, c->stream, c->nvo,
                     c->vptr.p, c->vcol.p, c->A00.p, c->A01.p, c->A10.p, c->A11.p, x, y);
  prof_end(c, 1);
  HIPCHK(c, hipGetLastError());
  return 0;
}

template <int BLK, int MODE>
__global__ __launch_bounds__(TPB) void spmv_blk_kernel(int nvo, const int *__restrict__ vptr, const int *__restrict__ vcol,
                                                       const double *__restrict__ A, const double *__restrict__ x,
                                                       double *__restrict__ y, const double *__restrict__ bvec) {
  const int gid = blockIdx.x * TPB + threadIdx.x;
  const int row = gid >> 3, l = gid & 7;
  double a0 = 0, a1 = 0;
  if (row < nvo) {
    const int ks = vptr[row], ke = vptr[row + 1];
    for (int k = ks + l; k < ke; k += 8) {
      const int w = vcol[k];
      if (w >= nvo) continue;
      if (BLK == 1) {
        const double2 xx = *(const double2 *)(x + 2 * (size_t)w);
        const double2 b0 = *(const double2 *)(A + 4 * (size_t)k), b1 = *(const double2 *)(A + 4 * (size_t)k + 2);
        a0 += b0.x * xx.x + b0.y * xx.y; a1 += b1.x * xx.x + b1.y * xx.y;
      } else if (BLK == 2) {
        const double xp = x[w];
        const double2 cc = *(const double2 *)(A + 2 * (size_t)k);
        a0 += cc.x * xp; a1 += cc.y * xp;
      } else if (BLK == 3) {
        const double2 xx = *(const double2 *)(x + 2 * (size_t)w);
        const double2 cc = *(const double2 *)(A + 2 * (size_t)k);
        a0 += cc.x * xx.x + cc.y * xx.y;
      } else {
        a0 += A[k] * x[w];
      }
    }
  }
  a0 = group8_sum(a0);
  if (BLK <= 2) a1 = group8_sum(a1);
  if (row < nvo && l == 0) {
    if (BLK <= 2) {
      double2 o = make_double2(a0, a1);
      if (MODE == 1) { const double2 bb = *(const double2 *)(bvec + 2 * (size_t)row); o.x = bb.x - o.x; o.y = bb.y - o.y; }
      *(double2 *)(y + 2 * (size_t)row) = o;
    } else {
      y[row] = (MODE == 1) ? bvec[row] - a0 : a0;
    }
  }
}

__global__ __launch_bounds__(TPB) void spmv_a01_resid_kernel(int nvo, const int *__restrict__ vptr, const int *__restrict__ vcol,
                                                             const double *__restrict__ A, const double *__restrict__ x,
                                                             double *__restrict__ y, const double *__restrict__ bvec) {
  const int gid = blockIdx.x * TPB + threadIdx.x;
  const int row = gid >> 2, l = gid & 3;
  double a0 = 0, a1 = 0;
  double2 bb = make_double2(0.0, 0.0);
  if (row < nvo) {
    const int ks = vptr[row], ke = vptr[row + 1];
    if (l == 0) bb = *(const double2 *)(bvec + 2 * (size_t)row);
    const int k0 = ks + l, k1 = k0 + 4;
    const bool h0 = k0 < ke, h1 = k1 < ke;
    const int q0 = h0 ? k0 : ks, q1 = h1 ? k1 : ks;
    const int w0 = vcol[q0], w1 = vcol[q1];
    const double2 c0 = *(const double2 *)(A + 2 * (size_t)q0), c1 = *(const double2 *)(A + 2 * (size_t)q1);
    const double x0 = (h0 && w0 < nvo) ? x[w0] : 0.0, x1 = (h1 && w1 < nvo) ? x[w1] : 0.0;
    a0 = c0.x * x0 + c1.x * x1;
    a1 = c0.y * x0 + c1.y * x1;
    for (int k = k1 + 4; k < ke; k += 4) {
      const int w = vcol[k];
      if (w >= nvo) continue;
      const double xp = x[w];
      const double2 cc = *(const double2 *)(A + 2 * (size_t)k);
      a0 += cc.x * xp; a1 += cc.y * xp;
    }
  }
  a0 = quad_sum(a0); a1 = quad_sum(a1);
  if (row < nvo && l == 0) *(double2 *)(y + 2 * (size_t)row) = make_double2(bb.x - a0, bb.y - a1);
}

template <int GB>
__global__ __launch_bounds__(TPB) void spmv_blk_ghost_kernel(int nvo, const int *__restrict__ vptr, const int *__restrict__ vcol,
                                                             const double *__restrict__ A, const double *__restrict__ xv,
                                                             double *__restrict__ y, const double *__restrict__ bvec) {
  const int gid = blockIdx.x * TPB + threadIdx.x;
  const int row = gid >> 3, l = gid & 7;
  double a0 = 0, a1 = 0;
  if (row < nvo) {
    const int ks = vptr[row], ke = vptr[row + 1];
    for (int k = ks + l; k < ke; k += 8) {
      const int w = vcol[k];
      const double2 cc = *(const double2 *)(A + 2 * (size_t)k);
      if (GB == 2) {
        const double xp = xv[poff(w, nvo)];
        a0 += cc.x * xp; a1 += cc.y * xp;
      } else {
        const int uo = uoff(w, nvo);
        a0 += cc.x * xv[uo] + cc.y * xv[uo + 1];
      }
    }
  }
  a0 = group8_sum(a0);
  if (GB == 2) a1 = group8_sum(a1);
  if (row < nvo && l == 0) {
    if (GB == 2) {
      const double2 bb = *(const double2 *)(bvec + 2 * (size_t)row);
      *(double2 *)(y + 2 * (size_t)row) = make_double2(bb.x - a0, bb.y - a1);
    } else {
      y[row] = bvec[row] - a0;
    }
  }
}
int k_spmv_block_ghost(cfdh_ctx *c, int blk, const double *xv, double *y, const double *b) {
  if (c->dim == 3) return k3_spmv_block_ghost(c, blk, xv, y, b);
  const long long nthreads = 8ll * c->nvo;
  dim3 grid((unsigned)((nthreads + TPB - 1) / TPB)), block(TPB);
  if (blk == 2) hipLaunchKernelGGL((spmv_blk_ghost_kernel<2>), grid, block, 0, c->stream, c->nvo, c->vptr.p, c->vcol.p, c->A01.p, xv, y, b);
  else hipLaunchKernelGGL((spmv_blk_ghost_kernel<3>), grid, block, 0, c->stream, c->nvo, c->vptr.p, c->vcol.p, c->A10.p, xv, y, b);
  HIPCHK(c, hipGetLastError());
  return 0;
}

int k_spmv_block(cfdh_ctx *c, int blk, const double *x, double *y, const double *b, double ) {
  if (c->dim == 3) return k3_spmv_block(c, blk, x, y, b);
  const long long nthreads = 8ll * c->nvo;
  dim3 grid((unsigned)((nthreads + TPB - 1) / TPB)), block(TPB);
  const int mode = b ? 1 : 0;
#define LAUNCH_BLK(B, M, AP) hipLaunchKernelGGL((spmv_blk_kernel<B, M>), grid, block, 0, c->stream, c->nvo, c->vptr.p, c->vcol.p, AP, x, y, b)
  if (blk == 1) { if (mode) LAUNCH_BLK(1, 1, c->A00.p); else LAUNCH_BLK(1, 0, c->A00.p); }
  else if (blk == 2) {
    if (mode) {
      const long long n4 = 4ll * c->nvo;
      hipLaunchKernelGGL(spmv_a01_resid_kernel, dim3((unsigned)((n4 + TPB - 1) / TPB)), block, 0, c->stream, c->nvo, c->vptr.p,
                         c->vcol.p, c->A01.p, x, y, b);
    } else {
      LAUNCH_BLK(2, 0, c->A01.p);
    }
  }
  else if (blk == 3) { if (mode) LAUNCH_BLK(3, 1, c->A10.p); else LAUNCH_BLK(3, 0, c->A10.p); }
  else { if (mode) LAUNCH_BLK(4, 1, c->A11.p); else LAUNCH_BLK(4, 0, c->A11.p); }
#undef LAUNCH_BLK
  HIPCHK(c, hipGetLastError());
  return 0;
}

__global__ __launch_bounds__(TPB) void extract_diag_kernel(int nvo, const int *__restrict__ vdiag,
                                                           const double *__restrict__ A00, double *__restrict__ dinv) {
  const int row = blockIdx.x * TPB + threadIdx.x;
  if (row >= nvo) return;
  const size_t k = (size_t)vdiag[row];
  const double d0 = A00[4 * k], d1 = A00[4 * k + 3];
  *(double2 *)(dinv + 2 * (size_t)row) = make_double2(1.0 / d0, 1.0 / d1);
}

int k_extract_diag(cfdh_ctx *c) {
  hipLaunchKernelGGL(extract_diag_kernel, dim3((c->nvo + TPB - 1) / TPB), dim3(TPB), 0, c->stream, c->nvo, c->vdiag.p,
                     c->A00.p, c->dinvA.p);
  HIPCHK(c, hipGetLastError());
  return 0;
}

template <bool FIRST, bool LAST>
__global__ __launch_bounds__(TPB) void cheb_a00_step_kernel(int nvo, const int *__restrict__ vptr,
                                                            const int *__restrict__ vcol, const double *__restrict__ A00,
                                                            const double *__restrict__ dinv, const double *__restrict__ rin,
                                                            double *__restrict__ rout, const double *__restrict__ dold,
                                                            double *__restrict__ dnew, double *__restrict__ x,
                                                            const double *__restrict__ coef, int kstep) {
  const double c1 = coef[2 * kstep], c2 = coef[2 * kstep + 1], itheta = coef[0];
  const int gid = blockIdx.x * TPB + threadIdx.x;
  const int row = gid >> 3, l = gid & 7;
  double a0 = 0, a1 = 0;
  if (row < nvo) {
    const int ks = vptr[row], ke = vptr[row + 1];
    for (int k = ks + l; k < ke; k += 8) {
      const int w = vcol[k];
      if (w >= nvo) continue;
      double2 xx;
      if (FIRST) {
        const double2 dj = *(const double2 *)(dinv + 2 * (size_t)w), rj = *(const double2 *)(rin + 2 * (size_t)w);
        xx = make_double2(dj.x * rj.x * itheta, dj.y * rj.y * itheta);
      } else {
        xx = *(const double2 *)(dold + 2 * (size_t)w);
      }
      const double2 b0 = *(const double2 *)(A00 + 4 * (size_t)k), b1 = *(const double2 *)(A00 + 4 * (size_t)k + 2);
      a0 += b0.x * xx.x + b0.y * xx.y; a1 += b1.x * xx.x + b1.y * xx.y;
    }
  }
  a0 = group8_sum(a0); a1 = group8_sum(a1);
  if (row < nvo && l == 0) {
    const size_t o = 2 * (size_t)row;
    const double2 ri = *(const double2 *)(rin + o), di = *(const double2 *)(dinv + o);
    double2 dd;
    if (FIRST) dd = make_double2(di.x * ri.x * itheta, di.y * ri.y * itheta);
    else dd = *(const double2 *)(dold + o);
    const double r0 = ri.x - a0, r1 = ri.y - a1;
    const double n0 = c1 * dd.x + c2 * di.x * r0, n1 = c1 * dd.y + c2 * di.y * r1;
    if (!LAST) {
      *(double2 *)(rout + o) = make_double2(r0, r1);
      *(double2 *)(dnew + o) = make_double2(n0, n1);
    }
    if (FIRST) {
      *(double2 *)(x + o) = make_double2(dd.x + n0, dd.y + n1);
    } else {
      double2 xo = *(double2 *)(x + o);
      xo.x += n0; xo.y += n1;
      *(double2 *)(x + o) = xo;
    }
  }
}

__global__ __launch_bounds__(TPB) void cheb_init_kernel(int n, const double *__restrict__ dinv, const double *__restrict__ b,
                                                        double *__restrict__ d0, double *__restrict__ x, double itheta,
                                                        int accumulate, const double *__restrict__ coef) {
  const int i = blockIdx.x * TPB + threadIdx.x;
  if (i >= n) return;
  if (coef) itheta = coef[0];
  const double v = dinv[i] * b[i] * itheta;
  d0[i] = v;
  x[i] = accumulate ? x[i] + v : v;
}

int k_cheb_a00_coeffs(cfdh_ctx *c) {
  const double lmax = c->lmaxA, lmin = lmax / c->opt.cheb_ratio;
  const double theta = 0.5 * (lmax + lmin), delta = 0.5 * (lmax - lmin);
  const double sigma = theta / delta;
  double rho = 1.0 / sigma;
  std::vector<double> h(2 * 16 + 2, 0.0);
  h[0] = 1.0 / theta;
  for (int k = 1; k < c->opt.cheb_degree && k < 16; k++) {
    const double rho_new = 1.0 / (2.0 * sigma - rho);
    h[2 * k] = rho_new * rho; h[2 * k + 1] = 2.0 * rho_new / delta;
    rho = rho_new;
  }
  HIPCHK(c, c->cheb_coef.alloc(h.size()));
  HIPCHK(c, hipMemcpyAsync(c->cheb_coef.p, h.data(), sizeof(double) * h.size(), hipMemcpyHostToDevice, c->stream));
  HIPCHK(c, hipStreamSynchronize(c->stream));
  return 0;
}

int k_cheb_a00(cfdh_ctx *c, const double *b, double *x) {
  const int nu = 2 * c->nvo, deg = c->opt.cheb_degree;
  double *dold = c->pu1.p, *dnew = c->pu2.p, *r = c->pr.p;
  if (deg == 1) {
    hipLaunchKernelGGL(cheb_init_kernel, dim3((nu + TPB - 1) / TPB), dim3(TPB), 0, c->stream, nu, c->dinvA.p, b, dold, x,
                       0.0, 0, c->cheb_coef.p);
    HIPCHK(c, hipGetLastError());
    return 0;
  }
  const long long nthreads = 8ll * c->nvo;
  dim3 grid((unsigned)((nthreads + TPB - 1) / TPB)), block(TPB);
  for (int k = 1; k < deg; k++) {
    const bool first = (k == 1), last = (k == deg - 1);
    prof_begin(c, 3);
#define LAUNCH_A00(F, LST) hipLaunchKernelGGL((cheb_a00_step_kernel<F, LST>), grid, block, 0, c->stream, c->nvo, c->vptr.p, c->vcol.p, c->A00.p, c->dinvA.p, first ? b : r, r, dold, dnew, x, c->cheb_coef.p, k)
    if (first) { if (last) LAUNCH_A00(true, true); else LAUNCH_A00(true, false); }
    else { if (last) LAUNCH_A00(false, true); else LAUNCH_A00(false, false); }
#undef LAUNCH_A00
    prof_end(c, 3);
    std::swap(dold, dnew);
  }
  HIPCHK(c, hipGetLastError());
  return 0;
}

struct d3 { double x, y, z; };
__device__ __forceinline__ d3 vzero(const d3 *) { return d3{0.0, 0.0, 0.0}; }
__device__ __forceinline__ d3 vfma(double a, d3 x, d3 acc) { return d3{acc.x + a * x.x, acc.y + a * x.y, acc.z + a * x.z}; }
__device__ __forceinline__ d3 vsub(d3 a, d3 b) { return d3{a.x - b.x, a.y - b.y, a.z - b.z}; }
__device__ __forceinline__ d3 vadd(d3 a, d3 b) { return d3{a.x + b.x, a.y + b.y, a.z + b.z}; }
__device__ __forceinline__ d3 vscale(double a, d3 x) { return d3{a * x.x, a * x.y, a * x.z}; }
__device__ __forceinline__ d3 g8(d3 v) { return d3{group8_sum(v.x), group8_sum(v.y), group8_sum(v.z)}; }
__device__ __forceinline__ d3 wsum(d3 v) { return d3{wave_sum(v.x), wave_sum(v.y), wave_sum(v.z)}; }
__device__ __forceinline__ double vzero(const double *) { return 0.0; }
__device__ __forceinline__ double2 vzero(const double2 *) { return make_double2(0.0, 0.0); }
__device__ __forceinline__ double vfma(double a, double x, double acc) { return acc + a * x; }
__device__ __forceinline__ double2 vfma(double a, double2 x, double2 acc) { return make_double2(acc.x + a * x.x, acc.y + a * x.y); }
__device__ __forceinline__ double vsub(double a, double b) { return a - b; }
__device__ __forceinline__ double2 vsub(double2 a, double2 b) { return make_double2(a.x - b.x, a.y - b.y); }
__device__ __forceinline__ double vadd(double a, double b) { return a + b; }
__device__ __forceinline__ double2 vadd(double2 a, double2 b) { return make_double2(a.x + b.x, a.y + b.y); }
__device__ __forceinline__ double vscale(double a, double x) { return a * x; }
__device__ __forceinline__ double2 vscale(double a, double2 x) { return make_double2(a * x.x, a * x.y); }
__device__ __forceinline__ double g8(double v) { return group8_sum(v); }
__device__ __forceinline__ double2 g8(double2 v) { return make_double2(group8_sum(v.x), group8_sum(v.y)); }
__device__ __forceinline__ double wsum(double v) { return wave_sum(v); }
__device__ __forceinline__ double2 wsum(double2 v) { return make_double2(wave_sum(v.x), wave_sum(v.y)); }

template <int MAXW, typename T>
__device__ __forceinline__ T sell_row_dot(const int *__restrict__ sp, const int *__restrict__ sc, const float *__restrict__ sv,
                                          const T *__restrict__ x, int sl, int lane, T a) {
  sl = __builtin_amdgcn_readfirstlane(sl);
  const int p0 = sp[sl], w = (sp[sl + 1] - p0) >> 6;
  int cidx[MAXW];
  float cval[MAXW];
#pragma unroll
  for (int k = 0; k < MAXW; k++)
    if (k < w) { const int p = p0 + k * 64 + lane; cidx[k] = NTLOAD(sc + p); cval[k] = NTLOAD(sv + p); }
  T g[MAXW];
#pragma unroll
  for (int k = 0; k < MAXW; k++)
    if (k < w) g[k] = x[cidx[k]];
#pragma unroll
  for (int k = 0; k < MAXW; k++)
    if (k < w) a = vfma((double)cval[k], g[k], a);
  for (int k = MAXW; k < w; k++) { const int p = p0 + k * 64 + lane; a = vfma((double)sv[p], x[sc[p]], a); }
  return a;
}

template <int MODE, typename T>
__global__ __launch_bounds__(TPB) void csr_spmv_kernel(int n, const int *__restrict__ rowptr, const int *__restrict__ col,
                                                       const double *__restrict__ val, const T *__restrict__ x,
                                                       T *__restrict__ y, const T *__restrict__ b) {
  const int gid = blockIdx.x * TPB + threadIdx.x;
  const int row = gid >> 3, l = gid & 7;
  T a = vzero((const T *)nullptr);
  if (row < n) {
    const int ks = rowptr[row], ke = rowptr[row + 1];
    for (int k = ks + l; k < ke; k += 8) a = vfma(val[k], x[col[k]], a);
  }
  a = g8(a);
  if (row < n && l == 0) {
    if (MODE == 0) y[row] = a;
    else if (MODE == 1) y[row] = vsub(b[row], a);
    else if (MODE == 2) y[row] = vadd(y[row], a);
    else y[row] = vadd(b[row], a);
  }
}

template <typename T>
static int csr_spmv_t(cfdh_ctx *c, const CsrDev &A, const T *x, T *y, int mode, const T *b) {
  const long long nthreads = 8ll * A.n;
  dim3 grid((unsigned)((nthreads + TPB - 1) / TPB)), block(TPB);
  if (mode == 0) hipLaunchKernelGGL((csr_spmv_kernel<0, T>), grid, block, 0, c->stream, A.n, A.rowptr.p, A.col.p, A.val.p, x, y, b);
  else if (mode == 1) hipLaunchKernelGGL((csr_spmv_kernel<1, T>), grid, block, 0, c->stream, A.n, A.rowptr.p, A.col.p, A.val.p, x, y, b);
  else if (mode == 2) hipLaunchKernelGGL((csr_spmv_kernel<2, T>), grid, block, 0, c->stream, A.n, A.rowptr.p, A.col.p, A.val.p, x, y, b);
  else hipLaunchKernelGGL((csr_spmv_kernel<3, T>), grid, block, 0, c->stream, A.n, A.rowptr.p, A.col.p, A.val.p, x, y, b);
  HIPCHK(c, hipGetLastError());
  return 0;
}
int k_csr_spmv(cfdh_ctx *c, const CsrDev &A, const double *x, double *y, int mode, const double *b) {
  return csr_spmv_t<double>(c, A, x, y, mode, b);
}
int k_csr_spmv_ncol(cfdh_ctx *c, const CsrDev &A, const double *x, double *y, int mode, const double *b, int ncol) {
  if (ncol == 2) return csr_spmv_t<double2>(c, A, (const double2 *)x, (double2 *)y, mode, (const double2 *)b);
  if (ncol == 3) return csr_spmv_t<d3>(c, A, (const d3 *)x, (d3 *)y, mode, (const d3 *)b);
  return csr_spmv_t<double>(c, A, x, y, mode, b);
}

template <int MODE, bool LAST>
__global__ __launch_bounds__(TPB) void cheb_csr_step_kernel(int n, const int *__restrict__ rowptr, const int *__restrict__ col,
                                                            const double *__restrict__ val, const double *__restrict__ dinv,
                                                            const double *__restrict__ rin, double *__restrict__ rout,
                                                            const double *__restrict__ dold, double *__restrict__ dnew,
                                                            double *__restrict__ x, double c1, double c2, double itheta) {
  const int gid = blockIdx.x * TPB + threadIdx.x;
  const int row = gid >> 3, l = gid & 7;
  double a = 0;
  if (row < n) {
    const int ks = rowptr[row], ke = rowptr[row + 1];
    for (int k = ks + l; k < ke; k += 8) {
      const int j = col[k];
      a += val[k] * (MODE == 1 ? dinv[j] * rin[j] * itheta : dold[j]);
    }
  }
  a = group8_sum(a);
  if (row < n && l == 0) {
    const double di = dinv[row], ri = rin[row];
    const double dd = (MODE == 1) ? di * ri * itheta : dold[row];
    const double r = ri - a;
    const double dn = c1 * dd + c2 * di * r;
    if (!LAST) { rout[row] = r; dnew[row] = dn; }
    if (MODE == 0) x[row] += dn;
    else if (MODE == 1) x[row] = dd + dn;
    else x[row] += dd + dn;
  }
}

__global__ __launch_bounds__(TPB) void csr_resid_init_kernel(int n, const int *__restrict__ rowptr, const int *__restrict__ col,
                                                             const double *__restrict__ val, const double *__restrict__ dinv,
                                                             const double *__restrict__ b, const double *__restrict__ x,
                                                             double *__restrict__ r, double *__restrict__ d0, double itheta) {
  const int gid = blockIdx.x * TPB + threadIdx.x;
  const int row = gid >> 3, l = gid & 7;
  double a = 0;
  if (row < n) {
    const int ks = rowptr[row], ke = rowptr[row + 1];
    for (int k = ks + l; k < ke; k += 8) a += val[k] * x[col[k]];
  }
  a = group8_sum(a);
  if (row < n && l == 0) {
    const double rr = b[row] - a;
    r[row] = rr;
    d0[row] = dinv[row] * rr * itheta;
  }
}

static int level_cheb(cfdh_ctx *c, AmgLevel *L, const double *b, double *x, bool zero_guess, int deg, bool prof) {
  const int n = L->n;
  const double theta = 0.5 * (L->lmax + L->lmin), delta = 0.5 * (L->lmax - L->lmin), sigma = theta / delta;
  double rho = 1.0 / sigma;
  double *dold = L->d0.p, *dnew = L->d1.p, *r = L->r.p;
  const double *rin = b;
  const double itheta = 1.0 / theta;
  const long long nthreads = 8ll * n;
  dim3 grid((unsigned)((nthreads + TPB - 1) / TPB)), block(TPB);
  const int *rp = L->A.rowptr.p, *cl = L->A.col.p;
  const double *vl = L->A.val.p, *di = L->dinv.p;
  if (deg == 1) {
    if (!zero_guess) { CHK(k_csr_spmv(c, L->A, x, r, 1, b)); rin = r; }
    hipLaunchKernelGGL(cheb_init_kernel, dim3((n + TPB - 1) / TPB), block, 0, c->stream, n, di, rin, dold, x, itheta,
                       zero_guess ? 0 : 1, (const double *)nullptr);
    HIPCHK(c, hipGetLastError());
    return 0;
  }
  if (!zero_guess) {
    hipLaunchKernelGGL(csr_resid_init_kernel, grid, block, 0, c->stream, n, rp, cl, vl, di, b, x, r, dold, itheta);
    rin = r;
  }
  for (int k = 1; k < deg; k++) {
    const double rho_new = 1.0 / (2.0 * sigma - rho);
    const double c1 = rho_new * rho, c2 = 2.0 * rho_new / delta;
    const bool last = (k == deg - 1);
    const int mode = (k == 1) ? (zero_guess ? 1 : 2) : 0;
    if (prof) prof_begin(c, 4);
#define LAUNCH_STEP(M, LST) hipLaunchKernelGGL((cheb_csr_step_kernel<M, LST>), grid, block, 0, c->stream, n, rp, cl, vl, di, rin, r, dold, dnew, x, c1, c2, itheta)
    if (mode == 1) { if (last) LAUNCH_STEP(1, true); else LAUNCH_STEP(1, false); }
    else if (mode == 2) { if (last) LAUNCH_STEP(2, true); else LAUNCH_STEP(2, false); }
    else { if (last) LAUNCH_STEP(0, true); else LAUNCH_STEP(0, false); }
#undef LAUNCH_STEP
    if (prof) prof_end(c, 4);
    rin = r;
    std::swap(dold, dnew);
    rho = rho_new;
  }
  HIPCHK(c, hipGetLastError());
  return 0;
}
int k_level_smooth(cfdh_ctx *c, AmgLevel *L, const double *b, double *x, int degree) { return level_cheb(c, L, b, x, true, degree, false); }

__global__ __launch_bounds__(TPB) void sell_cheb2_scale_kernel(int n, const int *__restrict__ sptr, const int *__restrict__ scol,
                                                               const float *__restrict__ svalw, const double *__restrict__ wdinv,
                                                               const double *__restrict__ dinv, const double *__restrict__ b,
                                                               double *__restrict__ x, const double *__restrict__ ml,
                                                               double *__restrict__ y, double c1, double c2) {
  const int row = blockIdx.x * TPB + threadIdx.x;
  if (row >= n) return;
  const int sl = row >> 6, lane = row & 63;
  const int p0 = sptr[sl], w = (sptr[sl + 1] - p0) >> 6;
  (void)p0; (void)w;
  const double a = sell_row_dot<10, double>(sptr, scol, svalw, b, sl, lane, 0.0);
  const double bi = b[row];
  const double dd = wdinv[row] * bi;
  const double xv = dd + (c1 * dd + c2 * dinv[row] * (bi - a));
  x[row] = xv;
  y[row] = ml[row] * xv;
}
bool k_cc_cheb2_scale(cfdh_ctx *c, AmgLevel *L, const double *b, double *x, const double *ml, double *y) {
  const int n = L->n;
  if (!(L->A.nnz <= 20ll * n && n >= 16384)) return false;
  const double theta = 0.5 * (L->lmax + L->lmin), delta = 0.5 * (L->lmax - L->lmin), sigma = theta / delta;
  const double rho = 1.0 / sigma, rho_new = 1.0 / (2.0 * sigma - rho);
  const double c1 = rho_new * rho, c2 = 2.0 * rho_new / delta;
  hipLaunchKernelGGL(sell_cheb2_scale_kernel, dim3((n + TPB - 1) / TPB), dim3(TPB), 0, c->stream, n, L->A.sptr.p, L->A.scol.p,
                     L->A.svalw.p, L->wdinv.p, L->dinv.p, b, x, ml, y, c1, c2);
  return hipGetLastError() == hipSuccess;
}

template <typename T>
__global__ __launch_bounds__(64) void dense_mv_kernel(int n, const double *__restrict__ Minv, const T *__restrict__ b,
                                                      T *__restrict__ y) {
  const int row = blockIdx.x, l = threadIdx.x;
  T a = vzero((const T *)nullptr);
  for (int k = l; k < n; k += 64) a = vfma(Minv[(size_t)row * n + k], b[k], a);
  a = wsum(a);
  if (l == 0) y[row] = a;
}

template <typename T>
__global__ __launch_bounds__(TPB) void jacobi_pre_kernel(int n, const int *__restrict__ rowptr, const int *__restrict__ col,
                                                         const double *__restrict__ val, const double *__restrict__ wdinv,
                                                         const T *__restrict__ b, T *__restrict__ xa, T *__restrict__ r) {
  const int gid = blockIdx.x * TPB + threadIdx.x;
  const int row = gid >> 3, l = gid & 7;
  T a = vzero((const T *)nullptr);
  if (row < n) {
    const int ks = rowptr[row], ke = rowptr[row + 1];
    for (int k = ks + l; k < ke; k += 8) {
      const int j = col[k];
      a = vfma(val[k] * wdinv[j], b[j], a);
    }
  }
  a = g8(a);
  if (row < n && l == 0) {
    const T bi = b[row];
    xa[row] = vscale(wdinv[row], bi);
    r[row] = vsub(bi, a);
  }
}
template <typename T>
__global__ __launch_bounds__(TPB) void jacobi_post_kernel(int n, const int *__restrict__ rowptr, const int *__restrict__ col,
                                                          const double *__restrict__ val, const double *__restrict__ wdinv,
                                                          const T *__restrict__ b, const T *__restrict__ xin,
                                                          T *__restrict__ xout) {
  const int gid = blockIdx.x * TPB + threadIdx.x;
  const int row = gid >> 3, l = gid & 7;
  T a = vzero((const T *)nullptr);
  if (row < n) {
    const int ks = rowptr[row], ke = rowptr[row + 1];
    for (int k = ks + l; k < ke; k += 8) a = vfma(val[k], xin[col[k]], a);
  }
  a = g8(a);
  if (row < n && l == 0) {
    xout[row] = vadd(xin[row], vscale(wdinv[row], vsub(b[row], a)));
  }
}

template <int MODE, typename T>
__global__ __launch_bounds__(TPB) void sell_spmv_kernel(int n, const int *__restrict__ sptr, const int *__restrict__ scol,
                                                        const float *__restrict__ sval, const T *__restrict__ x,
                                                        T *__restrict__ y, const T *__restrict__ b) {
  const int row = blockIdx.x * TPB + threadIdx.x;
  if (row >= n) return;
  const int sl = row >> 6, lane = row & 63;
  const int p0 = sptr[sl], w = (sptr[sl + 1] - p0) >> 6;
  T a = vzero((const T *)nullptr);
#pragma unroll 4
  for (int k = 0; k < w; k++) {
    const int p = p0 + k * 64 + lane;
    a = vfma((double)sval[p], x[scol[p]], a);
  }
  if (MODE == 0) y[row] = a;
  else if (MODE == 1) y[row] = vsub(b[row], a);
  else if (MODE == 2) y[row] = vadd(y[row], a);
  else y[row] = vadd(b[row], a);
}
template <typename T>
__global__ __launch_bounds__(TPB) void sell_jacobi_pre_kernel(int n, const int *__restrict__ sptr, const int *__restrict__ scol,
                                                              const float *__restrict__ svalw, const double *__restrict__ wdinv,
                                                              const T *__restrict__ b, T *__restrict__ xa, T *__restrict__ r) {
  const int row = blockIdx.x * TPB + threadIdx.x;
  if (row >= n) return;
  const int sl = row >> 6, lane = row & 63;
  const int p0 = sptr[sl], w = (sptr[sl + 1] - p0) >> 6;
  T a = vzero((const T *)nullptr);
#pragma unroll 4
  for (int k = 0; k < w; k++) {
    const int p = p0 + k * 64 + lane;
    a = vfma((double)svalw[p], b[scol[p]], a);
  }
  const T bi = b[row];
  xa[row] = vscale(wdinv[row], bi);
  r[row] = vsub(bi, a);
}
template <typename T>
__global__ __launch_bounds__(TPB) void sell_jacobi_post_kernel(int n, const int *__restrict__ sptr, const int *__restrict__ scol,
                                                               const float *__restrict__ sval, const double *__restrict__ wdinv,
                                                               const T *__restrict__ b, const T *__restrict__ xin,
                                                               T *__restrict__ xout) {
  const int row = blockIdx.x * TPB + threadIdx.x;
  if (row >= n) return;
  const int sl = row >> 6, lane = row & 63;
  const int p0 = sptr[sl], w = (sptr[sl + 1] - p0) >> 6;
  T a = vzero((const T *)nullptr);
#pragma unroll 4
  for (int k = 0; k < w; k++) {
    const int p = p0 + k * 64 + lane;
    a = vfma((double)sval[p], xin[scol[p]], a);
  }
  xout[row] = vadd(xin[row], vscale(wdinv[row], vsub(b[row], a)));
}

template <typename T>
static int amg_cycle_jacobi(cfdh_ctx *c, AmgHier &H, size_t lev, const T *b, T *x, int prof) {
  AmgLevel *L = H.lev[lev];
  if (lev + 1 == H.lev.size()) {
    if (H.coarse_n > 0) {
      hipLaunchKernelGGL((dense_mv_kernel<T>), dim3(H.coarse_n), dim3(64), 0, c->stream, H.coarse_n, H.coarse_inv.p, b, x);
    } else {
      const int n = L->n;
      dim3 block(TPB), gridC((unsigned)((8ll * n + TPB - 1) / TPB));
      T *xa = (T *)L->d0.p, *r = (T *)L->r.p;
      hipLaunchKernelGGL((jacobi_pre_kernel<T>), gridC, block, 0, c->stream, n, L->A.rowptr.p, L->A.col.p, L->A.val.p,
                         L->wdinv.p, b, xa, r);
      hipLaunchKernelGGL((jacobi_post_kernel<T>), gridC, block, 0, c->stream, n, L->A.rowptr.p, L->A.col.p, L->A.val.p,
                         L->wdinv.p, b, (const T *)xa, x);
    }
    HIPCHK(c, hipGetLastError());
    return 0;
  }
  AmgLevel *N = H.lev[lev + 1];
  const int n = L->n;
  const bool sell = L->A.nnz <= 12ll * n && n >= 16384;
  dim3 block(TPB), gridS((unsigned)((n + TPB - 1) / TPB)), gridC((unsigned)((8ll * n + TPB - 1) / TPB));
  T *xa = (T *)L->d0.p, *x1 = (T *)L->d1.p, *r = (T *)L->r.p;
  if (prof && lev == 0) prof_begin(c, prof);
  if (sell)
    hipLaunchKernelGGL((sell_jacobi_pre_kernel<T>), gridS, block, 0, c->stream, n, L->A.sptr.p, L->A.scol.p, L->A.svalw.p,
                       L->wdinv.p, b, xa, r);
  else
    hipLaunchKernelGGL((jacobi_pre_kernel<T>), gridC, block, 0, c->stream, n, L->A.rowptr.p, L->A.col.p, L->A.val.p,
                       L->wdinv.p, b, xa, r);
  if (prof && lev == 0) prof_end(c, prof);
  CHK(csr_spmv_t<T>(c, L->R, r, (T *)N->b.p, 0, (const T *)nullptr));
  CHK(amg_cycle_jacobi<T>(c, H, lev + 1, (const T *)N->b.p, (T *)N->x.p, prof));
  if (sell)
    hipLaunchKernelGGL((sell_spmv_kernel<3, T>), gridS, block, 0, c->stream, n, L->P.sptr.p, L->P.scol.p, L->P.sval.p,
                       (const T *)N->x.p, x1, (const T *)xa);
  else
    CHK(csr_spmv_t<T>(c, L->P, (const T *)N->x.p, x1, 3, xa));
  if (prof && lev == 0) prof_begin(c, prof);
  if (sell)
    hipLaunchKernelGGL((sell_jacobi_post_kernel<T>), gridS, block, 0, c->stream, n, L->A.sptr.p, L->A.scol.p, L->A.sval.p,
                       L->wdinv.p, b, x1, x);
  else
    hipLaunchKernelGGL((jacobi_post_kernel<T>), gridC, block, 0, c->stream, n, L->A.rowptr.p, L->A.col.p, L->A.val.p,
                       L->wdinv.p, b, x1, x);
  if (prof && lev == 0) prof_end(c, prof);
  HIPCHK(c, hipGetLastError());
  return 0;
}

template <int LPR>
__device__ __forceinline__ double lpr_sum(double v) {
  v = group8_sum(v);
  if (LPR >= 16) v += dpp_shuffle<0x140>(v);
  if (LPR >= 32) v += __shfl_xor(v, 16);
  if (LPR >= 64) v += __shfl_xor(v, 32);
  return v;
}
template <int LPR> __device__ __forceinline__ double lsum(double v) { return lpr_sum<LPR>(v); }
template <int LPR> __device__ __forceinline__ double2 lsum(double2 v) { return make_double2(lpr_sum<LPR>(v.x), lpr_sum<LPR>(v.y)); }
template <int LPR> __device__ __forceinline__ d3 lsum(d3 v) { return d3{lpr_sum<LPR>(v.x), lpr_sum<LPR>(v.y), lpr_sum<LPR>(v.z)}; }

__device__ __forceinline__ double epi_apply(double acc, int row, double alpha, double beta, const double *zH, const double *r, const unsigned char *pbc) {
  return (pbc[row] & 1) ? r[row] : alpha * acc + beta * zH[row];
}
__device__ __forceinline__ double2 epi_apply(double2 acc, int, double, double, const double *, const double *, const unsigned char *) { return acc; }
__device__ __forceinline__ double epi_value(double acc, unsigned flag, double alpha, double beta, double zh, double r) { return (flag & 1u) ? r : alpha * acc + beta * zh; }
__device__ __forceinline__ double2 epi_value(double2 acc, unsigned, double, double, double, double) { return acc; }
__device__ __forceinline__ d3 epi_apply(d3 acc, int, double, double, const double *, const double *, const unsigned char *) { return acc; }
__device__ __forceinline__ d3 epi_value(d3 acc, unsigned, double, double, double, double) { return acc; }

template <int LPR, typename VT, typename T>
__global__ __launch_bounds__(TPB) void fused_down_kernel(int n, const int *__restrict__ rowptr, const int *__restrict__ col,
                                                         const VT *__restrict__ val, const T *__restrict__ x, T *__restrict__ y) {
  const int gid = blockIdx.x * TPB + threadIdx.x;
  const int row = gid / LPR, l = gid % LPR;
  T a = vzero((const T *)nullptr);
  if (row < n) {
    const int ks = rowptr[row], ke = rowptr[row + 1];
    int cidx[4];
    VT cval[4];
#pragma unroll
    for (int q = 0; q < 4; q++) { const int k = ks + l + q * LPR; if (k < ke) { cidx[q] = col[k]; cval[q] = val[k]; } }
    T g[4];
#pragma unroll
    for (int q = 0; q < 4; q++) { const int k = ks + l + q * LPR; if (k < ke) g[q] = x[cidx[q]]; }
#pragma unroll
    for (int q = 0; q < 4; q++) { const int k = ks + l + q * LPR; if (k < ke) a = vfma((double)cval[q], g[q], a); }
    for (int k = ks + l + 4 * LPR; k < ke; k += LPR) a = vfma((double)val[k], x[col[k]], a);
  }
  a = lsum<LPR>(a);
  if (row < n && l == 0) y[row] = a;
}
template <typename T>
__global__ __launch_bounds__(TPB) void fused_up_csr_kernel(int n, const int *__restrict__ rpB, const int *__restrict__ clB,
                                                           const double *__restrict__ vlB, const T *__restrict__ b,
                                                           const int *__restrict__ rpC, const int *__restrict__ clC,
                                                           const double *__restrict__ vlC, const T *__restrict__ xc,
                                                           T *__restrict__ x, double ea, double eb, const double *__restrict__ ezH,
                                                           const double *__restrict__ er, const unsigned char *__restrict__ epbc) {
  const int gid = blockIdx.x * TPB + threadIdx.x;
  const int row = gid >> 3, l = gid & 7;
  T a = vzero((const T *)nullptr);
  if (row < n) {
    const int kb = rpB[row] + l, keB = rpB[row + 1];
    int kc = 0, keC = 0;
    if (rpC) { kc = rpC[row] + l; keC = rpC[row + 1]; }
    int cb[2], cc[2];
    double vb[2], vc[2];
#pragma unroll
    for (int q = 0; q < 2; q++) {
      if (kb + 8 * q < keB) { cb[q] = clB[kb + 8 * q]; vb[q] = vlB[kb + 8 * q]; }
      if (kc + 8 * q < keC) { cc[q] = clC[kc + 8 * q]; vc[q] = vlC[kc + 8 * q]; }
    }
    T gb[2], gc[2];
#pragma unroll
    for (int q = 0; q < 2; q++) {
      if (kb + 8 * q < keB) gb[q] = b[cb[q]];
      if (kc + 8 * q < keC) gc[q] = xc[cc[q]];
    }
#pragma unroll
    for (int q = 0; q < 2; q++) {
      if (kb + 8 * q < keB) a = vfma(vb[q], gb[q], a);
      if (kc + 8 * q < keC) a = vfma(vc[q], gc[q], a);
    }
    for (int k = kb + 16; k < keB; k += 8) a = vfma(vlB[k], b[clB[k]], a);
    for (int k = kc + 16; k < keC; k += 8) a = vfma(vlC[k], xc[clC[k]], a);
  }
  a = g8(a);
  if (row < n && l == 0) x[row] = epbc ? epi_apply(a, row, ea, eb, ezH, er, epbc) : a;
}
template <typename T, bool WIDE>
__global__ __launch_bounds__(TPB) void fused_up_sell_kernel(int n, const int *__restrict__ spB, const int *__restrict__ scB,
                                                            const float *__restrict__ svB, const T *__restrict__ b,
                                                            const int *__restrict__ spC, const int *__restrict__ scC,
                                                            const float *__restrict__ svC, const T *__restrict__ xc,
                                                            T *__restrict__ x, double ea, double eb, const double *__restrict__ ezH,
                                                            const double *__restrict__ er, const unsigned char *__restrict__ epbc) {
  const int row = blockIdx.x * TPB + threadIdx.x;
  if (row >= n) return;
  const int sl = __builtin_amdgcn_readfirstlane(row >> 6), lane = row & 63;
  T a = vzero((const T *)nullptr);
  double e_zh = 0.0, e_r = 0.0;
  unsigned e_f = 0;
  if (epbc) { e_f = epbc[row]; e_zh = ezH[row]; e_r = er[row]; }
  constexpr int MW = sizeof(T) > 8 ? 8 : 10;
  const int pB = spB[sl], wB = (spB[sl + 1] - pB) >> 6;
  int pC = 0, wC = 0;
  if (spC) { pC = spC[sl]; wC = (spC[sl + 1] - pC) >> 6; }
  const int wmax = wB > wC ? wB : wC;
  for (int k0 = 0; k0 < (WIDE ? wmax : 1); k0 += MW) {
    int cB[MW], cC[MW];
    float vB[MW], vC[MW];
#pragma unroll
    for (int k = 0; k < MW; k++) if (k0 + k < wB) { const int p = pB + (k0 + k) * 64 + lane; cB[k] = NTLOAD(scB + p); vB[k] = NTLOAD(svB + p); }
#pragma unroll
    for (int k = 0; k < MW; k++) if (k0 + k < wC) { const int p = pC + (k0 + k) * 64 + lane; cC[k] = NTLOAD(scC + p); vC[k] = NTLOAD(svC + p); }
    T gB[MW], gC[MW];
#pragma unroll
    for (int k = 0; k < MW; k++) if (k0 + k < wB) gB[k] = b[cB[k]];
#pragma unroll
    for (int k = 0; k < MW; k++) if (k0 + k < wC) gC[k] = xc[cC[k]];
#pragma unroll
    for (int k = 0; k < MW; k++) if (k0 + k < wB) a = vfma((double)vB[k], gB[k], a);
#pragma unroll
    for (int k = 0; k < MW; k++) if (k0 + k < wC) a = vfma((double)vC[k], gC[k], a);
  }
  if (!WIDE) {
    for (int k = MW; k < wB; k++) { const int p = pB + k * 64 + lane; a = vfma((double)svB[p], b[scB[p]], a); }
    for (int k = MW; k < wC; k++) { const int p = pC + k * 64 + lane; a = vfma((double)svC[p], xc[scC[p]], a); }
  }
  x[row] = epbc ? epi_value(a, e_f, ea, eb, e_zh, e_r) : a;
}
template <typename T>
__global__ __launch_bounds__(TPB) void fused_up_dense_kernel(int n, const int *__restrict__ rpB, const int *__restrict__ clB,
                                                             const double *__restrict__ vlB, const T *__restrict__ b,
                                                             const float *__restrict__ D, int nc, const T *__restrict__ bc,
                                                             T *__restrict__ x) {
  const int gid = blockIdx.x * TPB + threadIdx.x;
  const int row = gid >> 6, l = gid & 63;
  T a = vzero((const T *)nullptr);
  if (row < n) {
    for (int k = rpB[row] + l, ke = rpB[row + 1]; k < ke; k += 64) a = vfma(vlB[k], b[clB[k]], a);
    const float *Dr = D + (size_t)row * nc;
    float dv[12];
    T bv[12];
#pragma unroll
    for (int q = 0; q < 12; q++) { const int j = l + 64 * q; if (j < nc) { dv[q] = Dr[j]; bv[q] = bc[j]; } }
#pragma unroll
    for (int q = 0; q < 12; q++) { const int j = l + 64 * q; if (j < nc) a = vfma((double)dv[q], bv[q], a); }
    for (int j = l + 768; j < nc; j += 64) a = vfma((double)Dr[j], bc[j], a);
  }
  a = wsum(a);
  if (row < n && l == 0) x[row] = a;
}

template <typename VT, typename T>
static void launch_down(cfdh_ctx *c, const CsrDev &G, const VT *val, const T *x, T *y) {
  const long long avg = G.n > 0 ? (G.nnz + G.n - 1) / G.n : 1;
  const int lpr = avg > 96 ? 64 : (avg > 48 ? 32 : (avg > 20 ? 16 : 8));
  dim3 block(TPB), grid((unsigned)(((long long)G.n * lpr + TPB - 1) / TPB));
  if (lpr == 64) hipLaunchKernelGGL((fused_down_kernel<64, VT, T>), grid, block, 0, c->stream, G.n, G.rowptr.p, G.col.p, val, x, y);
  else if (lpr == 32) hipLaunchKernelGGL((fused_down_kernel<32, VT, T>), grid, block, 0, c->stream, G.n, G.rowptr.p, G.col.p, val, x, y);
  else if (lpr == 16) hipLaunchKernelGGL((fused_down_kernel<16, VT, T>), grid, block, 0, c->stream, G.n, G.rowptr.p, G.col.p, val, x, y);
  else hipLaunchKernelGGL((fused_down_kernel<8, VT, T>), grid, block, 0, c->stream, G.n, G.rowptr.p, G.col.p, val, x, y);
}

template <typename T>
static int amg_cycle_fused(cfdh_ctx *c, AmgHier &H, const T *b, T *x, int prof, int l0 = 0) {
  const int nl = (int)H.lev.size();
  for (int l = l0; l + 1 < nl; l++) {
    AmgLevel *L = H.lev[l], *N = H.lev[l + 1];
    const T *src = l == l0 ? b : (const T *)L->b.p;
    if (prof && l == 0) prof_begin(c, prof + 4);
    if (L->fine) launch_down<float, T>(c, L->G, L->G.valf.p, src, (T *)N->b.p);
    else launch_down<double, T>(c, L->G, L->G.val.p, src, (T *)N->b.p);
    if (prof && l == 0) prof_end(c, prof + 4);
  }
  int l = nl - 1;
  {
    AmgLevel *L = H.lev[l];
    const T *bl = l == l0 ? b : (const T *)L->b.p;
    T *xl = l == l0 ? x : (T *)L->x.p;
    if (nl - 2 >= l0 && H.lev[nl - 2]->Dn > 0) {
      AmgLevel *U = H.lev[nl - 2];
      const T *bu = nl - 2 == l0 ? b : (const T *)U->b.p;
      T *xu = nl - 2 == l0 ? x : (T *)U->x.p;
      const int un = (nl - 2 == 0 && c->up0_rows > 0 && c->up0_rows < U->n) ? c->up0_rows : U->n;
      hipLaunchKernelGGL((fused_up_dense_kernel<T>), dim3((unsigned)((64ll * un + TPB - 1) / TPB)), dim3(TPB), 0, c->stream, un,
                         U->Sb.rowptr.p, U->Sb.col.p, U->Sb.val.p, bu, U->D.p, U->Dn, bl, xu);
      l = nl - 3;
    } else {
      if (H.coarse_n > 0)
        hipLaunchKernelGGL((dense_mv_kernel<T>), dim3(H.coarse_n), dim3(64), 0, c->stream, H.coarse_n, H.coarse_inv.p, bl, xl);
      else if (L->sell)
        hipLaunchKernelGGL((fused_up_sell_kernel<T, true>), dim3((unsigned)((L->n + TPB - 1) / TPB)), dim3(TPB), 0, c->stream, L->n,
                           L->Sb.sptr.p, L->Sb.scol.p, L->Sb.sval.p, bl, (const int *)nullptr, (const int *)nullptr,
                           (const float *)nullptr, (const T *)nullptr, xl, 0.0, 0.0, (const double *)nullptr, (const double *)nullptr,
                           (const unsigned char *)nullptr);
      else
        hipLaunchKernelGGL((fused_up_csr_kernel<T>), dim3((unsigned)((8ll * L->n + TPB - 1) / TPB)), dim3(TPB), 0, c->stream, L->n,
                           L->Sb.rowptr.p, L->Sb.col.p, L->Sb.val.p, bl, (const int *)nullptr, (const int *)nullptr,
                           (const double *)nullptr, (const T *)nullptr, xl, 0.0, 0.0, (const double *)nullptr, (const double *)nullptr,
                           (const unsigned char *)nullptr);
      l = nl - 2;
    }
  }
  for (; l >= l0; l--) {
    AmgLevel *L = H.lev[l], *N = H.lev[l + 1];
    const T *bl = l == l0 ? b : (const T *)L->b.p;
    T *xl = l == l0 ? x : (T *)L->x.p;
    const bool epi = l == 0 && c->epi.on && sizeof(T) == sizeof(double);
    const double ea = epi ? c->epi.alpha : 0.0, eb = epi ? c->epi.beta : 0.0;
    const double *ezH = epi ? c->epi.zH : nullptr, *er = epi ? c->epi.r : nullptr;
    const unsigned char *epbc = epi ? c->epi.pbc : nullptr;
    if (epi) { xl = (T *)c->epi.out; c->epi.done = true; }
    const int nrow = (l == 0 && c->up0_rows > 0 && c->up0_rows < L->n) ? c->up0_rows : L->n;
    if (prof && l == 0) prof_begin(c, prof);
    if (L->sell && L->Sb.sell_maxw <= 14 && L->Sc.sell_maxw <= 14)
      hipLaunchKernelGGL((fused_up_sell_kernel<T, false>), dim3((unsigned)((nrow + TPB - 1) / TPB)), dim3(TPB), 0, c->stream, nrow,
                         L->Sb.sptr.p, L->Sb.scol.p, L->Sb.sval.p, bl, L->Sc.sptr.p, L->Sc.scol.p, L->Sc.sval.p, (const T *)N->x.p, xl,
                         ea, eb, ezH, er, epbc);
// ... 932 lines not shown
```

### cfd_hemodynamic_amd/csrc/cfdh_solver.cpp

```cpp
#include <algorithm>
#include <chrono>
#include <cmath>

#include "cfdh_internal.hpp"

int cfdh_host_threads();

static double wall_ms() {
  using namespace std::chrono;
  return duration<double, std::milli>(steady_clock::now().time_since_epoch()).count();
}

int cfdh_download_blocks(cfdh_ctx *c, std::vector<double> &a00, std::vector<double> &a01, std::vector<double> &a10,
                         std::vector<double> &a11) {
  const size_t nz = (size_t)c->nnzv, d = (size_t)c->dim;
  a00.resize(d * d * nz); a01.resize(d * nz); a10.resize(d * nz); a11.resize(nz);
  HIPCHK(c, hipMemcpyAsync(a00.data(), c->A00.p, sizeof(double) * d * d * nz, hipMemcpyDeviceToHost, c->stream));
  HIPCHK(c, hipMemcpyAsync(a01.data(), c->A01.p, sizeof(double) * d * nz, hipMemcpyDeviceToHost, c->stream));
  HIPCHK(c, hipMemcpyAsync(a10.data(), c->A10.p, sizeof(double) * d * nz, hipMemcpyDeviceToHost, c->stream));
  HIPCHK(c, hipMemcpyAsync(a11.data(), c->A11.p, sizeof(double) * nz, hipMemcpyDeviceToHost, c->stream));
  HIPCHK(c, hipStreamSynchronize(c->stream));
  return 0;
}

// ... 386 lines not shown
    HIPCHK(c, hipStreamSynchronize(c->stream));
    c->ms_pc_build_dev = wall_ms() - t0;
    return 0;
  }
  c->cc_alpha = c->rho * c->ts_a[0] / (c->ts_theta * c->dt);
  c->cc_beta = c->mu;
  {
    CsrDev Hd;
    CHK(cfdh_cc_h_dev(c, c->cc_alpha, c->cc_beta, Hd));
    CHK(cfdh_level_setup_dev(c, c->Hlev, Hd, 8.0, 1));
  }
  HIPCHK(c, hipStreamSynchronize(c->stream));
  c->ms_pc_build_dev = wall_ms() - t0;
  if (c->opt.verbose)
    fprintf(stderr, "[cfdh] preconditioner built on the device: velocity hierarchy %.1f ms, pressure Laplacian %.1f ms, H %.1f ms\n", t1 - t0, t2 - t1,
            wall_ms() - t2);
  return 0;
}
static int build_cc(cfdh_ctx *c) {
  static const bool host_multi = (getenv("CFDH_AMG_HOST_MULTI") && getenv("CFDH_AMG_HOST_MULTI")[0] == '1') ||
                                 (getenv("CFDH_PC_HOST_ASSEMBLY") && getenv("CFDH_PC_HOST_ASSEMBLY")[0] == '1');
  if (c->nranks > 1 && cfdh_amg_dev_enabled(c) && !host_multi) return build_cc_dev(c);
  if (c->nranks == 1 && cfdh_amg_dev_enabled(c)) {
    const int rc = build_cc_dev(c);
    if (rc == 0) return 0;
    if (c->opt.verbose) fprintf(stderr, "[cfdh] device-side hierarchy set-up failed (%s): host build\n", c->err.c_str());
    c->hL.clear(); c->hA.clear();
  }
  return build_cc_host(c);
}

int cfdh_pc_update(cfdh_ctx *c, bool refresh_amg) {
  const int nu = c->dim * c->nvo;
  if (c->opt.pc_type == 2) {
    if (c->gen) return cfdh_fail(c, CFDH_E_ARG, "pc_type 2 (PCD) exists for P1 triangles and tetrahedra on the closed-form kernels only");
    if (c->nranks > 1 || c->nvo != c->nv) return cfdh_fail(c, CFDH_E_ARG, "pc_type 2 (PCD) is not available in partitioned runs");
    if (!c->pcd_set) return cfdh_fail(c, CFDH_E_STATE, "pc_type 2 (PCD) needs cfdh_set_schur_pcd");
  } else if (c->dim == 3 && c->opt.pc_type != 1) {
    return cfdh_fail(c, CFDH_E_ARG, "tetrahedral contexts support pc_type 1 and 2 only");
  }
  if (c->opt.pc_type == 1 || c->opt.pc_type == 2) {
    if (refresh_amg || !c->pc_valid) {
      c->pc_graph_valid = false;
      CHK(build_cc(c));
      c->pc_valid = true;
      c->pc_its_ref = 0;
      c->steps_since_refresh = 0;
      c->last_stats.pc_refreshes++;
    c->n_pc_builds++;
    }
    if (c->opt.pc_type == 2) CHK(k_pcd_assemble(c, c->x.p));
    return 0;
  }
  CHK(k_extract_diag(c));
  double *v = c->pu0.p, *w = c->pu1.p;
  CHK(v_copy(c, nu, c->prand.p, v));
  double lam = 1.0;
  for (int it = 0; it < 8; it++) {
    CHK(k_spmv_block(c, 1, v, w, nullptr, 0));
    CHK(v_pointwise_mult(c, nu, w, c->dinvA.p, w));
    CHK(v_norm_to_dev(c, nu, w, c->red_out.p + 4));
    CHK(v_scale_inv_dev(c, nu, w, c->red_out.p + 4, v));
  }
  HIPCHK(c, hipMemcpyAsync(c->h_pinned, c->red_out.p + 4, sizeof(double), hipMemcpyDeviceToHost, c->stream));
  HIPCHK(c, hipStreamSynchronize(c->stream));
  lam = c->h_pinned[0];
  if (!(lam > 0) || !std::isfinite(lam)) return cfdh_fail(c, CFDH_E_DIVERGED, "non-finite spectral estimate of D^-1 A00 (NaN in the Jacobian?)");
  c->lmaxA = 1.15 * lam;
  CHK(k_cheb_a00_coeffs(c));
  if (refresh_amg || !c->pc_valid) {
    c->pc_graph_valid = false;
    CsrHost S;
    CHK(build_schur_host(c, S));
    bool any_pbc = false;
    for (int i = 0; i < c->nvo; i++) any_pbc |= (c->h_bcflag[i] & (1u << c->dim)) != 0;
    CHK(cfdh_amg_setup(c, c->hS, S, c->singular != 0 || !any_pbc, 1));
    c->pc_valid = true;
    c->pc_its_ref = 0;
    c->steps_since_refresh = 0;
    c->last_stats.pc_refreshes++;
    c->n_pc_builds++;
  }
  return 0;
}

static bool ras_ghost_rhs() {
  static const bool on = !(getenv("CFDH_RAS_GHOST_RHS") && getenv("CFDH_RAS_GHOST_RHS")[0] == '0');
  return on;
}

static int pcd_stage(cfdh_ctx *c, const double *r, double *z, int stage) {
  const int nvo = c->nvo, nu = c->dim * nvo;
  const double *ru = r, *rp = r + nu;
  double *zu = z, *zp = z + nu;
  const bool upper = c->opt.schur_full == 2;
  switch (stage) {
    case 0:
      if (!upper) CHK(k_amg_vcycle(c, c->hA, ru, c->pu0.p));
      return 0;
    case 1:
      if (!upper) CHK(k_spmv_block(c, 3, c->pu0.p, c->pp0.p, rp, 0));
      return k_pcd_apply(c, upper ? rp : c->pp0.p, c->pu1.p);
    case 2: {
      static const int lcycles = getenv("CFDH_L_CYCLES") ? atoi(getenv("CFDH_L_CYCLES")) : 1;
      if (lcycles > 1 && c->hL.lev.size() >= 1 && c->hL.lev[0]->A.val.p) {
        AmgLevel *L0 = c->hL.lev[0];
        CHK(k_amg_vcycle(c, c->hL, c->pu1.p, c->pu2.p));
        for (int cyc = 1; cyc < lcycles; cyc++) {
          CHK(k_csr_spmv(c, L0->A, c->pu2.p, L0->r.p, 1, c->pu1.p));
          CHK(k_amg_vcycle(c, c->hL, L0->r.p, L0->d0.p));
          CHK(v_axpy(c, nvo, 1.0, L0->d0.p, c->pu2.p));
        }
        return k_cc_combine(c, nvo, 1.0, c->mu, c->pu2.p, c->pcd_t.p, c->pcd_q.p, c->pcd_flag.p, zp);
      }
      c->epi.on = true; c->epi.done = false;
      c->epi.alpha = 1.0; c->epi.beta = c->mu; c->epi.zH = c->pcd_t.p; c->epi.r = c->pcd_q.p;
      c->epi.pbc = c->pcd_flag.p; c->epi.out = zp;
      const int rc = k_amg_vcycle(c, c->hL, c->pu1.p, c->pu2.p);
      c->epi.on = false;
      CHK(rc);
      if (c->epi.done) { c->epi.done = false; return 0; }
      return k_cc_combine(c, nvo, 1.0, c->mu, c->pu2.p, c->pcd_t.p, c->pcd_q.p, c->pcd_flag.p, zp);
    }
    case 3:
      if (c->opt.schur_full) {
        CHK(k_spmv_block(c, 2, zp, c->pu0.p, ru, 0));
        CHK(k_amg_vcycle(c, c->hA, c->pu0.p, zu));
      } else {
        CHK(v_copy(c, nu, c->pu0.p, zu));
      }
      return 0;
    default:
      return 0;
  }
}

static int pc_stage(cfdh_ctx *c, const double *r, double *z, int stage) {
  const int nvo = c->nvo, nu = c->dim * nvo;
  const double *ru = r, *rp = r + nu;
  double *zu = z, *zp = z + nu;
  const bool multi = c->nranks > 1;
  const bool global_p = c->gp_n > 0 && multi;
  if (c->opt.pc_type == 2) return pcd_stage(c, r, z, stage);
  if (c->opt.pc_type == 1) {
    const bool upper = c->opt.schur_full == 2;
    const bool dist = global_p && c->dl0.on;
    int ls = stage;
    if (dist) ls = stage <= 1 ? stage : (stage == 2 ? 10 : stage - 1);
    switch (ls) {
      case 0:
        if (upper) return 0;
        CHK(k_amg_vcycle(c, c->hA, ru, multi ? c->pcw.p : c->pu0.p));
        return 0;
      case 1:
        if (upper) {  }
        else if (multi) CHK(k_spmv_block_ghost(c, 3, c->pcw.p, c->pp0.p, rp));
        else CHK(k_spmv_block(c, 3, c->pu0.p, c->pp0.p, rp, 0));
        {
          double *y = !dist ? c->pu1.p : (c->dl0.ghost_rhs ? c->pcw.p + nu : c->dl0.b.p);
          if (!(c->opt.cc_smooth_degree == 2 && k_cc_cheb2_scale(c, &c->Hlev, upper ? rp : c->pp0.p, c->pp1.p, c->ccMl.p, y))) {
            CHK(k_level_smooth(c, &c->Hlev, upper ? rp : c->pp0.p, c->pp1.p, c->opt.cc_smooth_degree));
            CHK(k_cc_scale(c, nvo, c->ccMl.p, c->pp1.p, y));
          }
        }
        if (dist) {
        } else if (global_p && c->gp_allgather) {
          CHK(k_gather_global(c, nvo, c->gp_send_idx.p, c->pu1.p, c->gp_sendbuf.p));
        } else if (global_p) {
          CHK(v_zero(c, c->gp_n, c->gp_rhs.p));
          CHK(k_scatter_global(c, nvo, c->gp_l2g.p, c->pu1.p, c->gp_rhs.p));
        }
        return 0;
      case 10:
        return k_dl0_down(c, c->pcw.p);
      case 2:
        if (dist) {
          CHK(k_dl0_up(c, c->pu2.p));
        } else if (global_p) {
          if (c->gp_allgather) CHK(k_gather_global(c, c->gp_n, c->gp_src_idx.p, c->gp_recvbuf.p, c->gp_rhs.p));
          CHK(k_amg_vcycle(c, c->hLg, c->gp_rhs.p, c->gp_sol.p));
          CHK(k_gather_global(c, nvo, c->gp_l2g.p, c->gp_sol.p, c->pu2.p));
        } else {
          static const int lcycles = getenv("CFDH_L_CYCLES") ? atoi(getenv("CFDH_L_CYCLES")) : 1;
          if (lcycles > 1 && c->hL.lev.size() >= 1 && c->hL.lev[0]->A.val.p) {
            AmgLevel *L0 = c->hL.lev[0];
            CHK(k_amg_vcycle(c, c->hL, c->pu1.p, c->pu2.p));
            for (int cyc = 1; cyc < lcycles; cyc++) {
              CHK(k_csr_spmv(c, L0->A, c->pu2.p, L0->r.p, 1, c->pu1.p));
              CHK(k_amg_vcycle(c, c->hL, L0->r.p, L0->d0.p));
              CHK(v_axpy(c, nvo, 1.0, L0->d0.p, c->pu2.p));
            }
            CHK(k_cc_combine(c, nvo, c->cc_alpha, c->cc_beta, c->pu2.p, c->pp1.p, upper ? rp : c->pp0.p, c->ccPbc.p, zp));
            if (multi && c->opt.schur_full) CHK(v_copy(c, nvo, zp, c->pcw.p + nu));
            return 0;
          }
          c->epi.on = true; c->epi.done = false;
          c->epi.alpha = c->cc_alpha; c->epi.beta = c->cc_beta; c->epi.zH = c->pp1.p; c->epi.r = upper ? rp : c->pp0.p;
          c->epi.pbc = c->ccPbc.p; c->epi.out = zp;
          const int rc = k_amg_vcycle(c, c->hL, c->pu1.p, c->pu2.p);
          c->epi.on = false;
          CHK(rc);
        }
        if (c->epi.done) {
          c->epi.done = false;
          if (multi && c->opt.schur_full) CHK(v_copy(c, nvo, zp, c->pcw.p + nu));
        } else {
          CHK(k_cc_combine(c, nvo, c->cc_alpha, c->cc_beta, c->pu2.p, c->pp1.p, upper ? rp : c->pp0.p, c->ccPbc.p, zp,
                           (multi && c->opt.schur_full) ? c->pcw.p + nu : nullptr));
        }
        return 0;
      case 3:
        if (c->opt.schur_full) {
          if (multi) CHK(k_spmv_block_ghost(c, 2, c->pcw.p, c->ras ? c->pcw.p : c->pu0.p, ru));
          else CHK(k_spmv_block(c, 2, zp, c->pu0.p, ru, 0));
          if (multi && c->ras) {
            if (!ras_ghost_rhs()) CHK(v_zero(c, c->NL - c->NO, c->pcw.p + c->NO));
          }
          else {
            CHK(k_amg_vcycle(c, c->hA, c->pu0.p, zu));
            static const int acycles = getenv("CFDH_A_CYCLES") ? atoi(getenv("CFDH_A_CYCLES")) : 1;
            if (acycles > 1 && !multi && c->hA.lev[0]->A.val.p) {
              AmgLevel *L0 = c->hA.lev[0];
              for (int cyc = 1; cyc < acycles; cyc++) {
                CHK(k_csr_spmv_ncol(c, L0->A, zu, L0->r.p, 1, c->pu0.p, c->dim));
                CHK(k_amg_vcycle(c, c->hA, L0->r.p, L0->d0.p));
                CHK(v_axpy(c, nu, 1.0, L0->d0.p, zu));
              }
            }
          }
        } else {
          CHK(v_copy(c, nu, multi ? c->pcw.p : c->pu0.p, zu));
        }
        return 0;
      case 4:
        if (multi && c->ras && c->opt.schur_full) {
          CHK(k_ext_pack(c, c->pcw.p, c->ras_b.p));
          if (c->hA.fused && c->opt.amg_smooth_degree == 1 && c->hA.lev.size() >= 2) {
            c->up0_rows = nvo;
            const int rc = k_amg_vcycle(c, c->hA, c->ras_b.p, zu);
            c->up0_rows = 0;
            CHK(rc);
          } else {
            CHK(k_amg_vcycle(c, c->hA, c->ras_b.p, c->ras_x.p));
            CHK(v_copy(c, nu, c->ras_x.p, zu));
          }
        }
        return 0;
      default:
        return 0;
    }
  }
  if (stage != 0) return 0;
  CHK(k_cheb_a00(c, ru, c->pu0.p));
  CHK(k_spmv_block(c, 3, c->pu0.p, c->pp0.p, rp, 0));
  CHK(k_amg_vcycle(c, c->hS, c->pp0.p, zp));
  if (c->opt.schur_full) {
    CHK(k_spmv_block(c, 2, zp, c->pu0.p, ru, 0));
    CHK(k_cheb_a00(c, c->pu0.p, zu));
  } else {
    CHK(v_copy(c, nu, c->pu0.p, zu));
  }
  return 0;
}

static int pc_exchange(cfdh_ctx *c, int stage) {
  if (c->nranks <= 1 || c->opt.pc_type != 1) return 0;
  const bool dist = c->gp_n > 0 && c->dl0.on;
  int ls = stage;
  if (dist) ls = stage <= 1 ? stage : (stage == 2 ? 10 : stage - 1);
  switch (ls) {
    case 0: return c->opt.schur_full == 2 ? 0 : comm_halo(c, c->pcw.p);
    case 1:
      if (c->gp_n <= 0) return 0;
      if (dist) return c->dl0.ghost_rhs ? comm_halo(c, c->pcw.p) : 0;
      if (c->gp_allgather) return comm_allgather_dev(c, c->gp_sendbuf.p, c->gp_recvbuf.p, c->gp_maxcnt);
      return comm_allreduce_dev(c, c->gp_rhs.p, c->gp_n, 0);
    case 10: return comm_allreduce_dev(c, c->hLg.lev[1]->b.p, c->dl0.n1, 0);
    case 2: return c->opt.schur_full ? comm_halo(c, c->pcw.p) : 0;
    case 3: return (c->ras && c->opt.schur_full && ras_ghost_rhs()) ? comm_halo(c, c->pcw.p) : 0;
    default: return 0;
  }
}

int cfdh_pc_apply(cfdh_ctx *c, const double *r, double *z) {
  const int nvo = c->nvo;
  const bool graph = c->use_graph && !c->prof_on;
  const bool multi = c->nranks > 1 && c->opt.pc_type == 1;
  if (multi && !c->pcw.p) { HIPCHK(c, c->pcw.alloc(c->NL)); HIPCHK(c, c->pcw.zero(c->stream)); }
  if (!graph) {
    for (int st = 0; st < 6; st++) { CHK(pc_stage(c, r, z, st)); CHK(pc_exchange(c, st)); }
  } else {
    if (!c->pc_graph_valid) {
      for (auto &e : c->pc_graphs) for (auto &x : e.exec) if (x) (void)hipGraphExecDestroy(x);
      c->pc_graphs.clear();
      c->pc_graph_valid = true;
    }
    cfdh_ctx::PcGraph *pg = nullptr;
    for (auto &e : c->pc_graphs) if (e.r == r && e.z == z) { pg = &e; break; }
    if (!pg) {
      cfdh_ctx::PcGraph ng{r, z, {nullptr, nullptr, nullptr, nullptr, nullptr, nullptr}};
      for (int gidx = 0; gidx < (multi ? 6 : 1); gidx++) {
        hipGraph_t g = nullptr;
        HIPCHK(c, hipStreamBeginCapture(c->stream, hipStreamCaptureModeThreadLocal));
        c->capturing = true;
        int rc = 0;
        if (multi) rc = pc_stage(c, r, z, gidx);
        else for (int st = 0; st < 6 && !rc; st++) rc = pc_stage(c, r, z, st);
        c->capturing = false;
        hipError_t e = hipStreamEndCapture(c->stream, &g);
        if (rc) return rc;
        if (e != hipSuccess || !g) return cfdh_fail(c, CFDH_E_HIP, "hipStreamEndCapture: %s", hipGetErrorString(e));
        e = hipGraphInstantiate(&ng.exec[gidx], g, nullptr, nullptr, 0);
        (void)hipGraphDestroy(g);
        if (e != hipSuccess) return cfdh_fail(c, CFDH_E_HIP, "hipGraphInstantiate: %s", hipGetErrorString(e));
      }
      c->pc_graphs.push_back(ng);
      pg = &c->pc_graphs.back();
    }
    if (!multi) {
      HIPCHK(c, hipGraphLaunch(pg->exec[0], c->stream));
    } else {
      for (int st = 0; st < 6; st++) { HIPCHK(c, hipGraphLaunch(pg->exec[st], c->stream)); CHK(pc_exchange(c, st)); }
    }
  }
  if (c->singular) CHK(v_sub_mean(c, nvo, z + (size_t)c->dim * nvo));
  return 0;
}

static int ensure_krylov(cfdh_ctx *c) {
  const int m = c->opt.ksp_restart;
  if (c->kry_m == m && c->kV.p) return 0;
  const size_t NL = ((size_t)c->NL + 1) & ~(size_t)1;
  c->pc_graph_valid = false;
  HIPCHK(c, c->kV.alloc(NL * (m + 1)));
  HIPCHK(c, c->kZ.alloc(NL * m));
  HIPCHK(c, c->kw.alloc(NL));
  HIPCHK(c, c->kh.alloc(std::max(2 * (size_t)(m + 2) + 8, (size_t)8 * (8 + 1))));
  HIPCHK(c, c->ky.alloc(m + 8));
  if (c->h_ring) { (void)hipHostFree(c->h_ring); c->h_ring = nullptr; }
  c->h_ring_stride = ((size_t)m + 5) & ~(size_t)1;
  HIPCHK(c, hipHostMalloc((void **)&c->h_ring, sizeof(double) * c->h_ring_stride * (cfdh_ctx::KRING + 1)));
  HIPCHK(c, hipHostGetDevicePointer((void **)&c->h_ring_dev, c->h_ring, 0));
  for (auto &e : c->ev_ring) if (!e) HIPCHK(c, hipEventCreateWithFlags(&e, hipEventDisableTiming));
  HIPCHK(c, c->kV.zero(c->stream)); HIPCHK(c, c->kZ.zero(c->stream)); HIPCHK(c, c->kw.zero(c->stream));
  if ((size_t)(m + 2) * 1024 > c->red_partial.n) HIPCHK(c, c->red_partial.alloc((size_t)(m + 2) * 1024 + 1024));
  c->kry_m = m;
  return 0;
}

static int guess_ensure(cfdh_ctx *c) {
  const int m = c->opt.ksp_guess;
  const size_t ld = ((size_t)c->NL + 1) & ~(size_t)1;
  if (m == c->guess_m && (m == 0 || c->guessU.p)) return 0;
  c->guess_m = m;
  for (int k = 0; k < cfdh_ctx::GUESS_NEWTON; k++) c->guess_cnt[k] = c->guess_head[k] = 0;
  if (m > 0) {
    HIPCHK(c, c->guessU.alloc(ld * (size_t)m * cfdh_ctx::GUESS_NEWTON)); HIPCHK(c, c->guessU.zero(c->stream));
    HIPCHK(c, c->guessX.alloc(ld * (size_t)cfdh_ctx::GUESS_NEWTON));
  }
  return 0;
}

static int guess_project(cfdh_ctx *c, const double *b, double *x, bool *used) {
  *used = false;
  CHK(guess_ensure(c));
  const int slot = c->guess_slot, m = c->guess_m;
  if (m <= 0 || slot < 0 || slot >= cfdh_ctx::GUESS_NEWTON || c->guess_cnt[slot] == 0 || c->kry_m < m + 1) return 0;
  const int k = c->guess_cnt[slot], n = c->NO;
  const size_t ld = ((size_t)c->NL + 1) & ~(size_t)1;
  double *U = c->guessU.p + ld * (size_t)m * slot;
  double *V = c->kV.p, *Z = c->kZ.p, *hd = c->kh.p;
  if (c->nranks > 1) {
    for (int i = 0; i < k; i++) {
      double *t = V + (size_t)(i + 1) * ld;
      CHK(v_copy(c, n, U + (size_t)i * ld, t));
      CHK(comm_halo(c, t));
    }
    CHK(k_spmv_full_multi(c, V + ld, Z, (int)ld, k));
  } else {
    CHK(k_spmv_full_multi(c, U, Z, (int)ld, k));
  }
  std::vector<double> G((size_t)k * k), g(k), y(k, 0.0);
  HIPCHK(c, hipMemsetAsync(hd, 0, sizeof(double) * 8 * (size_t)(k + 1), c->stream));
  CHK(v_gram(c, n, Z, (int)ld, k, b, hd));
  CHK(comm_allreduce_dev(c, hd, 8 * (k + 1), 0));
  HIPCHK(c, hipMemcpyAsync(c->h_pinned, hd, sizeof(double) * 8 * (size_t)(k + 1), hipMemcpyDeviceToHost, c->stream));
  HIPCHK(c, hipStreamSynchronize(c->stream));
  c->n_host_sync++;
  for (int i = 0; i <= k; i++)
    for (int q = 0; q < k; q++) (i < k ? G[(size_t)q * k + i] : g[q]) = c->h_pinned[(size_t)i * 8 + q];
  if (c->opt.verbose > 1) {
    double bb = 0.0;
    CHK(v_norm2(c, n, b, &bb));
    fprintf(stderr, "[cfdh]     guess diag (newton %d): cos(W_i, b) =", slot);
    for (int i = 0; i < k; i++) fprintf(stderr, " %.6f", g[i] / (std::sqrt(G[(size_t)i * k + i]) * bb));
    fprintf(stderr, "; |W_i|/|b| =");
    for (int i = 0; i < k; i++) fprintf(stderr, " %.4f", std::sqrt(G[(size_t)i * k + i]) / bb);
    fprintf(stderr, "\n");
  }
  std::vector<int> piv;
  std::vector<double> Lc((size_t)k * k, 0.0), dg(k);
  std::vector<char> taken(k, 0);
  for (int i = 0; i < k; i++) dg[i] = G[(size_t)i * k + i];
  const double dmax0 = *std::max_element(dg.begin(), dg.end());
  if (!(dmax0 > 0.0) || !std::isfinite(dmax0)) return 0;
  for (int r = 0; r < k; r++) {
    int p = -1;
    for (int i = 0; i < k; i++) if (!taken[i] && (p < 0 || dg[i] > dg[p])) p = i;
    if (p < 0 || !(dg[p] > 1e-10 * G[(size_t)p * k + p]) || !(dg[p] > 1e-14 * dmax0)) break;
// ... 95 lines not shown
  for (;;) {
    double beta;
    if (first) {
      beta = bn;
    } else {
      if (!(guessed && its == 0 && j_prev == 0)) {
        CHK(comm_halo(c, x));
        CHK(k_spmv_full(c, x, w));
        CHK(v_waxpy(c, n, -1.0, w, b, V));
      } else if (getenv("CFDH_GUESS_CHECK")) {
        double diff = 0.0;
        CHK(comm_halo(c, x));
        CHK(k_spmv_full(c, x, w));
        CHK(v_waxpy(c, n, -1.0, w, b, w));
        CHK(v_waxpy(c, n, -1.0, V, w, w));
        CHK(v_norm2(c, n, w, &diff));
        if (!(diff <= 1e-10 * bn)) return cfdh_fail(c, CFDH_E_STATE, "projected guess: |(b - J x0) - (b - W y)| = %.3e |b|", diff / bn);
      }
      CHK(v_norm2(c, n, V, &beta));
      c->ksp_last_relres = beta / bn;
      if (guessed && its == 0 && j_prev == 0) {
        c->n_guess_solves++; c->guess_reduction_sum += beta / bn;
        if (o.verbose) fprintf(stderr, "[cfdh]     projected guess (newton %d, %d vectors): |r0| / |b| = %.3e\n", c->guess_slot, c->guess_cnt[c->guess_slot], beta / bn);
      }
      if (use32 && j_prev > 0 && beta > 10.0 * std::max(est_prev, tol)) {
        use32 = false; c->krylov_fp32_ok = false;
        if (o.verbose) fprintf(stderr, "[cfdh]     fgmres: true residual %.3e vs recurrence %.3e after a %d-vector cycle with the fp32 basis copy: switched off\n", beta, est_prev, j_prev);
      } else if (!c->gs_refine_long && j_prev > 0 && beta > 10.0 * std::max(est_prev, tol)) {
        c->gs_refine_long = true;
        if (o.verbose) fprintf(stderr, "[cfdh]     fgmres: true residual %.3e vs recurrence %.3e after a %d-vector cycle: re-orthogonalising long cycles from now on\n", beta, est_prev, j_prev);
        if (beta > beta_start && j_prev > 0) {
          for (int i = 0; i < j_prev; i++) y[i] = -y[i];
          HIPCHK(c, hipMemcpyAsync(c->ky.p, y.data(), sizeof(double) * j_prev, hipMemcpyHostToDevice, c->stream));
          CHK(v_lincomb(c, n, Z, (int)ld, j_prev, c->ky.p, x));
          HIPCHK(c, hipStreamSynchronize(c->stream));
          est_prev = beta_start;
          continue;
        }
      }
      static const bool no_attainable = getenv("CFDH_NO_ATTAINABLE_STOP") && getenv("CFDH_NO_ATTAINABLE_STOP")[0] == '1';
      if (j_prev > 0 && est_prev <= tol && beta > tol && !no_attainable) {
        if (last_true > 0.0 && beta > 0.5 * last_true && (beta <= 10.0 * tol || beta <= 1e-6 * bn)) {
          if (o.verbose) fprintf(stderr, "[cfdh]     fgmres: true residual %.3e stays above the tolerance %.3e although the recurrence converged twice: attainable accuracy, stopping\n", beta, tol);
          reason = CFDH_KSP_CONVERGED_ATTAINABLE;
          c->n_attainable_stops++;
          break;
        }
        last_true = beta;
      } else {
        last_true = -1.0;
      }
      beta_start = beta;
    }
    c->ksp_last_relres = beta / bn;
    if (beta <= tol) { reason = 2; break; }
    if (its >= o.ksp_max_it) { reason = -3; break; }
    if (!std::isfinite(beta)) { reason = -9; break; }
    if (first) CHK(v_scale_to(c, n, 1.0 / beta, b, V));
    else CHK(v_scale(c, n, 1.0 / beta, V));
    if (use32) CHK(v_store32(c, n, V, V32));
    first = false;
    std::fill(g.begin(), g.end(), 0.0);
    g[0] = beta;
    static const int refine_env = getenv("CFDH_GS_REFINE_FROM") ? atoi(getenv("CFDH_GS_REFINE_FROM")) : -1;
    static const int lag_env = getenv("CFDH_KSP_LAG") ? atoi(getenv("CFDH_KSP_LAG")) : cfdh_ctx::KRING - 3;
    const int refine_from = refine_env >= 0 ? refine_env : (c->gs_refine_long ? 24 : (1 << 30));
    const int lagmax = (o.ksp_rtol < 1e-7 || c->prof_on) ? 0 : std::max(0, std::min(lag_env, cfdh_ctx::KRING - 3));
    const int its_base = its;
    const int maxl = std::min(m, o.ksp_max_it - its_base);
    int j = 0;
    int jl = 0;
    const int e_its = (gslot >= 0 && gslot < cfdh_ctx::GUESS_NEWTON) ? c->guess_last_its[gslot] : 0;
    int need = std::max(1, std::min(e_its - its - 2, 3));
    double res_hist[4] = {beta, 0, 0, 0};
    int nhist = 1;
    bool done = false;
    double *s_dev = hd + 2 * (m + 2) + 1;
    const size_t rs = c->h_ring_stride;
    auto launch = [&](int jj) -> int {
      double *vj = V + (size_t)jj * ld, *zj = Z + (size_t)jj * ld, *vn = V + (size_t)(jj + 1) * ld;
      double *slot = c->h_ring_dev + (size_t)(jj % cfdh_ctx::KRING) * rs;
      CHK(cfdh_pc_apply(c, vj, zj));
      CHK(comm_halo(c, zj));
      CHK(k_spmv_full(c, zj, w));
      if (use32) {
        CHK(v_multidot32(c, n, V32, (int)ld32, jj + 1, w, hd, slot));
        CHK(v_gs_update32(c, n, V32, (int)ld32, jj + 1, hd, w, vn, V32 + (size_t)(jj + 1) * ld32, s_dev, slot + (jj + 2)));
        HIPCHK(c, hipEventRecord(c->ev_ring[jj % cfdh_ctx::KRING], c->stream));
      } else {
        CHK(v_multidot(c, n, V, (int)ld, jj + 1, w, hd, true, slot));
        HIPCHK(c, hipEventRecord(c->ev_ring[jj % cfdh_ctx::KRING], c->stream));
        CHK(v_gs_update_normalize(c, n, V, (int)ld, jj + 1, hd, w, vn, s_dev));
      }
      return 0;
    };
    while (!done && reason == 0) {
      const bool sync_now = lagmax == 0 || j >= refine_from;
      const int ahead = sync_now ? 1 : std::max(1, std::min(need - (need >= 4 ? 1 : 0), lagmax + 1));
      while (jl < maxl && jl - j < ahead) { CHK(launch(jl)); jl++; }
      if (jl == j) break;
      int upto = jl;
      if (!sync_now && jl - j > 1 && jl < maxl && need > jl - j) upto = jl - 1;
      c->n_host_sync++;
      HIPCHK(c, hipEventSynchronize(c->ev_ring[(upto - 1) % cfdh_ctx::KRING]));
      for (; j < upto && !done; ) {
        const double *hs = c->h_ring + (size_t)(j % cfdh_ctx::KRING) * rs;
        double *vn = V + (size_t)(j + 1) * ld;
        double ww = hs[j + 1], hh2 = 0.0;
        for (int i = 0; i <= j; i++) { hh[i] = hs[i]; hh2 += hh[i] * hh[i]; }
        double nrm2 = use32 ? hs[j + 2] * hs[j + 2] : ww - hh2;
        static const double eta2_env = getenv("CFDH_GS_ETA2") ? atof(getenv("CFDH_GS_ETA2")) : 1e-6;
        const double eta2 = (o.ksp_rtol < 1e-7 || j >= refine_from) ? 0.5 : eta2_env;
        const bool refine = !(nrm2 > eta2 * ww);
        double hnorm;
        if (refine) {
          if (jl > j + 1) { c->n_krylov_discarded += jl - (j + 1); jl = j + 1; }
          CHK(v_multidot(c, n, V, (int)ld, j + 1, vn, hd + (m + 2), true));
          CHK(v_multiaxpy(c, n, V, (int)ld, j + 1, hd + (m + 2), vn));
          if (use32) CHK(v_norm_to_dev(c, n, vn, hd + 2 * (m + 2)));
          HIPCHK(c, hipMemcpyAsync(c->h_pinned, hd + (m + 2), sizeof(double) * (m + 4), hipMemcpyDeviceToHost, c->stream));
          c->n_host_sync++;
          HIPCHK(c, hipStreamSynchronize(c->stream));
          const double s = use32 ? hs[j + 2] : ((nrm2 > 0.0 && nrm2 <= ww) ? std::sqrt(nrm2) : std::sqrt(ww));
          double h22 = 0.0;
          for (int i = 0; i <= j; i++) { hh[i] += s * c->h_pinned[i]; h22 += c->h_pinned[i] * c->h_pinned[i]; }
          double vnorm;
          if (use32) vnorm = c->h_pinned[m + 2];
          else {
            const double d2 = c->h_pinned[j + 1] - h22;
            vnorm = d2 > 0.0 ? std::sqrt(d2) : 0.0;
          }
          hnorm = s * vnorm;
          if (use32) { CHK(v_scale_inv_dev(c, n, vn, hd + 2 * (m + 2), vn)); CHK(v_store32(c, n, vn, V32 + (size_t)(j + 1) * ld32)); }
          else CHK(v_scale(c, n, vnorm > 0.0 ? 1.0 / vnorm : 0.0, vn));
        } else {
          hnorm = std::sqrt(nrm2);
        }
        double *Hj = &H[(size_t)j * (m + 1)];
        for (int i = 0; i <= j; i++) Hj[i] = hh[i];
        Hj[j + 1] = hnorm;
        for (int i = 0; i < j; i++) {
          const double t = cs[i] * Hj[i] + sn[i] * Hj[i + 1];
          Hj[i + 1] = -sn[i] * Hj[i] + cs[i] * Hj[i + 1];
          Hj[i] = t;
        }
        const double d = std::hypot(Hj[j], Hj[j + 1]);
        if (!(d > 0) || !std::isfinite(d)) { reason = -9; j++; break; }
        cs[j] = Hj[j] / d; sn[j] = Hj[j + 1] / d;
        Hj[j] = d; Hj[j + 1] = 0.0;
        g[j + 1] = -sn[j] * g[j]; g[j] = cs[j] * g[j];
        its++;
        j++;
        const double res = std::fabs(g[j]);
        if (o.verbose > 1) fprintf(stderr, "[cfdh]     fgmres %3d  |r|/|b| = %.3e\n", its, res / bn);
        if (res <= tol) { done = true; break; }
        if (nhist < 4) res_hist[nhist++] = res;
        else { res_hist[0] = res_hist[1]; res_hist[1] = res_hist[2]; res_hist[2] = res_hist[3]; res_hist[3] = res; }
        const double rho = std::pow(res / res_hist[0], 1.0 / (nhist - 1));
        int n_rem = (rho > 0.0 && rho < 0.97) ? (int)std::ceil(std::log(tol / res) / std::log(rho)) : (1 << 20);
        if (nhist == 2) n_rem = std::min(n_rem, 3);
        need = std::max(1, e_its > 0 ? std::min(n_rem, std::max(e_its - its, 1) + 2) : n_rem);
      }
      if (done || reason != 0) break;
    }
    if (jl > j) c->n_krylov_discarded += jl - j;
    if (reason == -9) break;
    for (int i = j - 1; i >= 0; i--) {
      double s = g[i];
      for (int k = i + 1; k < j; k++) s -= H[(size_t)k * (m + 1) + i] * y[k];
      y[i] = s / H[(size_t)i * (m + 1) + i];
    }
    double *ystage = c->h_ring + c->h_ring_stride * cfdh_ctx::KRING;
    for (int i = 0; i < j; i++) ystage[i] = y[i];
    HIPCHK(c, hipMemcpyAsync(c->ky.p, ystage, sizeof(double) * j, hipMemcpyHostToDevice, c->stream));
    CHK(v_lincomb(c, n, Z, (int)ld, j, c->ky.p, x));
    est_prev = std::fabs(g[j]);
    j_prev = j;
    (void)done;
  }
  c->n_krylov += its;
  *its_out = its;
  *reason_out = reason;
  if (gslot >= 0 && gslot < cfdh_ctx::GUESS_NEWTON) c->guess_last_its[gslot] = its;
  if (reason > 0) CHK(guess_store(c, x));
  return 0;
}

static int upload_bc(cfdh_ctx *c) {
  if (!c->bc_dirty) return 0;
  const int st = c->dim + 1;
  c->bc_pending.insert(c->bc_pending.end(), c->bc_touched.begin() + (std::ptrdiff_t)std::min(c->bc_touched_sent, c->bc_touched.size()), c->bc_touched.end());
  if ((int)c->bc_mark.size() != c->nv) { c->bc_mark.assign(c->nv, -1); c->bc_full_upload = true; }
  c->bc_epoch++;
  size_t K = 0;
  for (int v : c->bc_pending)
    if (c->bc_mark[v] != c->bc_epoch) { c->bc_mark[v] = c->bc_epoch; c->bc_pending[K++] = v; }
  c->bc_pending.resize(K);
  if (c->bc_touched.size() > 4 * (size_t)c->nv) { std::sort(c->bc_touched.begin(), c->bc_touched.end()); c->bc_touched.erase(std::unique(c->bc_touched.begin(), c->bc_touched.end()), c->bc_touched.end()); }
  c->bc_touched_sent = c->bc_touched.size();
// ... 167 lines not shown
```

### include/cfdh.h

```cpp
#ifndef CFDH_H
#define CFDH_H

#include <stdint.h>

#ifdef __cplusplus
extern "C" {
#endif

#define CFDH_ABI_VERSION 1

enum {
  CFDH_OK = 0,
  CFDH_E_ARG = -1,
  CFDH_E_HIP = -2,
  CFDH_E_STATE = -3,
  CFDH_E_DIVERGED = -4,
  CFDH_E_COMM = -5,
  CFDH_E_NOMEM = -6
};

enum {
  CFDH_CONVERGED_FNORM_ABS = 2,
  CFDH_CONVERGED_FNORM_RELATIVE = 3,
  CFDH_CONVERGED_SNORM_RELATIVE = 4,
// ... 6 lines not shown
  CFDH_KSP_CONVERGED_RTOL = 2,
  CFDH_KSP_CONVERGED_ATTAINABLE = 12,
  CFDH_KSP_DIVERGED_ITS = -3,
  CFDH_KSP_DIVERGED_NANORINF = -9
};

typedef struct cfdh_ctx cfdh_ctx;

typedef struct cfdh_options {
  double snes_rtol, snes_atol, snes_stol;
  int32_t snes_max_it;
  double ksp_rtol, ksp_atol;
  int32_t ksp_max_it, ksp_restart;
  int32_t cheb_degree;
  double cheb_ratio;
  int32_t schur_full;
  int32_t amg_smooth_degree;
  double amg_smooth_ratio;
  double amg_theta;
  int32_t amg_max_coarse;
  int32_t pc_refresh;
  int32_t remove_p_mean;
  int32_t verbose;
  int32_t pc_type;
  int32_t cc_smooth_degree;
  int32_t ksp_guess;
} cfdh_options;

typedef struct cfdh_stats {
  int32_t newton_its, krylov_its, reason, pc_refreshes;
  double fnorm0, fnorm;
  double ms_assemble, ms_solve, ms_pc_setup, ms_total;
} cfdh_stats;


int cfdh_create(cfdh_ctx **out, int device, int gdim, int64_t nv, int64_t nv_owned, int64_t nc,
                const int32_t *cells, const double *coords, int64_t nfacets, const int32_t *facet_cells,
                const int32_t *facet_local, const int32_t *facet_marker);
enum { CFDH_ELEM_P1 = 0, CFDH_ELEM_P2_TRIANGLE = 1, CFDH_ELEM_Q1_QUADRILATERAL = 2, CFDH_ELEM_P1_GENERIC = 3 };
int cfdh_create_elem(cfdh_ctx **out, int device, int gdim, int elem, int64_t nn, int64_t nc, const int32_t *cells,
                     const double *node_coords, int64_t nfacets, const int32_t *facet_cells, const int32_t *facet_local,
                     const int32_t *facet_marker);
int cfdh_create_elem_part(cfdh_ctx **out, int device, int gdim, int elem, int64_t nn, int64_t nn_owned, int64_t nc, const int32_t *cells,
                          const double *node_coords, int64_t nfacets, const int32_t *facet_cells, const int32_t *facet_local,
                          const int32_t *facet_marker);
int cfdh_set_facet_markers(cfdh_ctx *ctx, int64_t nfacets, const int32_t *markers);
void cfdh_destroy(cfdh_ctx *ctx);
const char *cfdh_last_error(const cfdh_ctx *ctx);
int cfdh_abi_version(void);

int cfdh_set_params(cfdh_ctx *ctx, double dt, double rho, double mu, double mu_facet, const double f[3]);
int cfdh_default_options(cfdh_options *opt);
int cfdh_set_options(cfdh_ctx *ctx, const cfdh_options *opt);


int cfdh_clear_dirichlet(cfdh_ctx *ctx);
int cfdh_add_dirichlet(cfdh_ctx *ctx, int field, int64_t n, const int32_t *nodes, const double *values);
int cfdh_update_dirichlet(cfdh_ctx *ctx, int field, int64_t n, const int32_t *nodes, const double *values);


int cfdh_set_state(cfdh_ctx *ctx, const double *u_prev, const double *p_prev, const double *u, const double *p);
int cfdh_get_solution(cfdh_ctx *ctx, double *u, double *p);
int cfdh_get_previous(cfdh_ctx *ctx, double *u_prev, double *p_prev);
int cfdh_get_residual(cfdh_ctx *ctx, double *ru, double *rp);
int cfdh_advance(cfdh_ctx *ctx);
int cfdh_advance_field(cfdh_ctx *ctx, int field);


int cfdh_set_time_scheme(cfdh_ctx *ctx, double theta, double a0, double a1, double a2);

int cfdh_set_boundary_terms(cfdh_ctx *ctx, int ds_terms, int backflow_marker, double beta);


enum { CFDH_FORM_CONVECTIVE = 0, CFDH_FORM_ROTATIONAL = 1 };
int cfdh_set_formulation(cfdh_ctx *ctx, int form);
int cfdh_set_pressure_boundaries(cfdh_ctx *ctx, int n, const int32_t *markers, const double *values, double beta_nitsche);


int cfdh_set_schur_pcd(cfdh_ctx *ctx, int inlet_marker, int outlet_marker, int time_term);
int cfdh_set_ksp_forcing(cfdh_ctx *ctx, int version, double rtol_0, double rtol_max, double gamma, double alpha, double threshold);
int cfdh_get_newton_history(cfdh_ctx *ctx, int32_t *n, double *fnorm, double *ksp_rtol, int32_t *ksp_its, double *ksp_rel_res);
int cfdh_get_pcd_operator(cfdh_ctx *ctx, int64_t *nnz, int32_t *rowptr, int32_t *col, double *vals, double *mass_diag);
int cfdh_apply_preconditioner(cfdh_ctx *ctx, const double *r, double *z);

#define CFDH_AMG_HIER_A 0
#define CFDH_AMG_HIER_P 1
#define CFDH_AMG_HIER_H 2
#define CFDH_AMG_OP_A 0
#define CFDH_AMG_OP_P 1
#define CFDH_AMG_OP_G 2
#define CFDH_AMG_OP_SB 3
#define CFDH_AMG_OP_SC 4
int cfdh_get_amg_operator(cfdh_ctx *ctx, int hier, int level, int which, int64_t *nrow, int64_t *ncol, int64_t *nnz, int32_t *rowptr,
                          int32_t *col, double *vals);
#define CFDH_AMG_VEC_DINV 0
#define CFDH_AMG_VEC_WDINV 1
#define CFDH_AMG_VEC_AGG 2
#define CFDH_AMG_VEC_COARSE_INV 3
#define CFDH_AMG_VEC_D 4
#define CFDH_AMG_VEC_LAMBDA 5
#define CFDH_AMG_VEC_CC_SCALARS 6
#define CFDH_AMG_VEC_CC_ML 7
#define CFDH_AMG_VEC_CC_PBC 8
#define CFDH_AMG_VEC_SPGEMM_ROWS 9
#define CFDH_AMG_VEC_SHAPE 10
#define CFDH_AMG_VEC_ORDER 11
#define CFDH_AMG_VEC_A00_LMAX 12
#define CFDH_AMG_VEC_A00_DINV 13
int cfdh_get_amg_vectors(cfdh_ctx *ctx, int hier, int level, int which, int64_t *n, double *out);


int cfdh_create_ipcs(cfdh_ctx **out, int device, int gdim, int64_t nn, int64_t nvert, int64_t nc, const int32_t *cells,
                     const double *node_coords, int64_t nfacets, const int32_t *facet_cells, const int32_t *facet_local,
                     const int32_t *facet_marker);
int cfdh_ipcs_set_form(cfdh_ctx *ctx, double conv_coeff, double force_coeff);
int cfdh_ipcs_set_tolerances(cfdh_ctx *ctx, const double rtol[3], double atol, const int32_t max_it[3]);
typedef struct cfdh_ipcs_stats {
  int32_t its[3], reason[3];
  double rel_res[3];
  double ms_assemble, ms_solve[3], ms_total;
  int32_t launches, host_syncs;
} cfdh_ipcs_stats;
int cfdh_ipcs_step(cfdh_ctx *ctx, cfdh_ipcs_stats *stats);
int cfdh_ipcs_get_operator(cfdh_ctx *ctx, int which, int64_t *nnz, int32_t *rowptr, int32_t *col, double *vals);
int cfdh_ipcs_get_intermediate(cfdh_ctx *ctx, int which, double *out);
int cfdh_ipcs_apply_pressure_pc(cfdh_ctx *ctx, const double *r, double *z);

int cfdh_set_previous2(cfdh_ctx *ctx, const double *u_prev2);
int cfdh_get_previous2(cfdh_ctx *ctx, double *u_prev2);
int cfdh_shift_history(cfdh_ctx *ctx);


int cfdh_assemble(cfdh_ctx *ctx, int want_jacobian);
int cfdh_get_csr(cfdh_ctx *ctx, int64_t *nnz, int32_t *rowptr, int32_t *col, double *vals);
int cfdh_spmv(cfdh_ctx *ctx, const double *x, double *y);


int cfdh_solve_step(cfdh_ctx *ctx, cfdh_stats *stats);

int cfdh_functional(cfdh_ctx *ctx, int kind, int marker, double *out);

int cfdh_wall_shear_stress(cfdh_ctx *ctx, double *shear);


int cfdh_set_halo(cfdh_ctx *ctx, int nnbr, const int32_t *nbr_rank, const int64_t *send_ptr,
                  const int32_t *send_idx, const int64_t *recv_ptr, const int32_t *recv_idx);
int cfdh_set_global_pressure_space(cfdh_ctx *ctx, int64_t nv_global, int64_t nc_global, const int32_t *cells_global,
                                   const double *coords_global, const int32_t *owned_global, int64_t n_pbc,
                                   const int32_t *pbc_nodes_global);
int cfdh_comm_unique_id(void *id128);
int cfdh_comm_init(cfdh_ctx *ctx, const void *id128, int rank, int nranks);
typedef int (*cfdh_allreduce_fn)(void *user, double *buf, int n, int op);
typedef int (*cfdh_exchange_fn)(void *user, const double *sendbuf, double *recvbuf);
int cfdh_comm_set_callbacks(cfdh_ctx *ctx, cfdh_allreduce_fn ar, cfdh_exchange_fn ex, void *user, int rank, int nranks);


int cfdh_profile_enable(cfdh_ctx *ctx, int on);
int cfdh_profile_get(cfdh_ctx *ctx, int kind, double *total_ms, int64_t *launches);
int cfdh_profile_reset(cfdh_ctx *ctx);
int64_t cfdh_info(const cfdh_ctx *ctx, int what);

#ifdef __cplusplus
}
#endif
#endif
```

Measured before the change: 420.8.

## Remap blocks across XCDs and reuse A01·p product in FGMRES operator apply

Adds an XCD-aware block index remap to most SpMV and smoother kernels, so consecutive logical blocks sit on the same chiplet and share its L2. It also caches the A01·z_p product computed in the Schur preconditioner stage and reuses it in a new fused full SpMV that skips the A01 term when forming A·z in FGMRES. A third change resets the GMRES projection bound after discarding Krylov vectors, and a new API exposes the iteration operator for testing. The cached product is only valid when r and z match the last preconditioner apply, which adds state tracking and forces graph recapture whenever that setting changes.

```diff
diff --git a/cfd_hemodynamic_amd/_lib.py b/cfd_hemodynamic_amd/_lib.py
--- a/cfd_hemodynamic_amd/_lib.py
+++ b/cfd_hemodynamic_amd/_lib.py
@@ -51,7 +51,7 @@
     "cfdh_shift_history", "cfdh_set_boundary_terms", "cfdh_set_formulation", "cfdh_set_pressure_boundaries", "cfdh_assemble", "cfdh_get_csr", "cfdh_spmv", "cfdh_solve_step",
     "cfdh_functional", "cfdh_wall_shear_stress", "cfdh_set_global_pressure_space", "cfdh_set_halo", "cfdh_comm_unique_id", "cfdh_comm_init", "cfdh_comm_set_callbacks",
     "cfdh_profile_enable", "cfdh_profile_get", "cfdh_profile_reset", "cfdh_info",
-    "cfdh_set_schur_pcd", "cfdh_set_ksp_forcing", "cfdh_get_newton_history", "cfdh_get_pcd_operator", "cfdh_apply_preconditioner",
+    "cfdh_set_schur_pcd", "cfdh_set_ksp_forcing", "cfdh_get_newton_history", "cfdh_get_pcd_operator", "cfdh_apply_preconditioner", "cfdh_xcd_block", "cfdh_apply_iteration_operator",
     "cfdh_get_amg_operator", "cfdh_get_amg_vectors",
     "cfdh_create_ipcs", "cfdh_ipcs_set_form", "cfdh_ipcs_set_tolerances", "cfdh_ipcs_step", "cfdh_ipcs_get_operator", "cfdh_ipcs_get_intermediate",
     "cfdh_ipcs_apply_pressure_pc",
@@ -130,6 +130,8 @@
     L.cfdh_get_newton_history.argtypes = [vp, ip, dp, dp, ip, dp]
     L.cfdh_get_pcd_operator.argtypes = [vp, lp, ip, ip, dp, dp]
     L.cfdh_apply_preconditioner.argtypes = [vp, dp, dp]
+    L.cfdh_xcd_block.argtypes = [C.c_int, C.c_int]
+    L.cfdh_apply_iteration_operator.argtypes = [vp, dp, C.c_int, dp, dp, dp]
     L.cfdh_get_amg_operator.argtypes = [vp, C.c_int, C.c_int, C.c_int, lp, lp, lp, ip, ip, dp]
     L.cfdh_get_amg_vectors.argtypes = [vp, C.c_int, C.c_int, C.c_int, lp, dp]
     L.cfdh_create_ipcs.argtypes = [C.POINTER(vp), C.c_int, C.c_int, C.c_int64, C.c_int64, C.c_int64, ip, dp, C.c_int64, ip, ip, ip]
@@ -431,6 +433,14 @@
         self._chk(self.L.cfdh_apply_preconditioner(self.h, _dp(r), _dp(z)))
         return z
 
+    def apply_iteration_operator(self, R):
+        R = np.ascontiguousarray(np.atleast_2d(R), dtype=np.float64)
+        if R.shape[1] != (self.dim + 1) * self.nv:
+            raise ValueError("monolithic vectors of (gdim + 1) nv entries expected")
+        z, w, h = np.zeros(R.shape[1]), np.zeros(R.shape[1]), np.zeros(R.shape[0] + 1)
+        self._chk(self.L.cfdh_apply_iteration_operator(self.h, _dp(R), R.shape[0], _dp(z), _dp(w), _dp(h)))
+        return z, w, h
+
     def get_amg_operator(self, hier, level, which, raw=False):
         import scipy.sparse as sp
         nr, nc, nnz = C.c_int64(), C.c_int64(), C.c_int64()
diff --git a/cfd_hemodynamic_amd/csrc/cfdh_api.cpp b/cfd_hemodynamic_amd/csrc/cfdh_api.cpp
--- a/cfd_hemodynamic_amd/csrc/cfdh_api.cpp
+++ b/cfd_hemodynamic_amd/csrc/cfdh_api.cpp
@@ -92,6 +92,8 @@
   do {
     if (hipSetDevice(device) != hipSuccess) { rc = cfdh_fail(nullptr, CFDH_E_HIP, "hipSetDevice(%d) failed", device); break; }
     if (hipStreamCreateWithFlags(&c->stream, hipStreamNonBlocking) != hipSuccess) { rc = cfdh_fail(nullptr, CFDH_E_HIP, "hipStreamCreate failed"); break; }
+    rc = k_upload_switches(c);
+    if (rc) break;
     rc = gdim == 3 ? k3_upload_quadrature(c) : k_upload_quadrature(c);
     if (rc) break;
     if (etype != 0) {
@@ -590,6 +592,8 @@
   return 0;
 }
 
+int cfdh_xcd_block(int b, int nb) { return (nb > 0 && b >= 0 && b < nb) ? xcd_block(b, nb) : -1; }
+
 int cfdh_apply_preconditioner(cfdh_ctx *c, const double *r, double *z) {
   NOT_IPCS(c, "cfdh_apply_preconditioner");
   if (!c || !r || !z) return CFDH_E_ARG;
@@ -606,6 +610,37 @@
     const int v = c->iperm[k], d = c->dim;
     for (int i = 0; i < d; i++) z[(size_t)d * v + i] = o[(size_t)d * k + i];
     z[(size_t)d * c->nv + v] = o[(size_t)d * c->nvo + k];
+  }
+  return 0;
+}
+
+int cfdh_apply_iteration_operator(cfdh_ctx *c, const double *R, int nvec, double *z, double *w, double *h) {
+  NOT_IPCS(c, "cfdh_apply_iteration_operator");
+  if (!c || !R || !z || !w || !h || nvec < 1 || nvec > 200) return CFDH_E_ARG;
+  ENTER(c);
+  if (c->nranks > 1 || c->nvo != c->nv) return cfdh_fail(c, CFDH_E_STATE, "cfdh_apply_iteration_operator: one GPU only");
+  if (!c->jac_valid) return cfdh_fail(c, CFDH_E_STATE, "no Jacobian assembled yet");
+  CHK(cfdh_pc_update(c, false));
+  const size_t N = (size_t)(c->dim + 1) * c->nv, ld = ((size_t)c->NL + 1) & ~(size_t)1;
+  dbuf<double> Vd, wd, hd;
+  HIPCHK(c, Vd.alloc(ld * nvec)); HIPCHK(c, wd.alloc(c->dvec.n)); HIPCHK(c, hd.alloc((size_t)nvec + 1));
+  std::vector<double> hv;
+  for (int v = 0; v < nvec; v++) {
+    pack_vec(c, R + v * N, R + v * N + (size_t)c->dim * c->nv, hv, nullptr);
+    CHK(upload_vec(c, hv, Vd.p + v * ld));
+  }
+  CHK(cfdh_pc_apply(c, Vd.p, c->dvec.p));
+  CHK(cfdh_iter_product(c, Vd.p, c->dvec.p, wd.p));
+  CHK(v_multidot(c, c->NO, Vd.p, (int)ld, nvec, wd.p, hd.p, true));
+  std::vector<double> o, ow;
+  CHK(download_vec(c, c->dvec.p, o));
+  CHK(download_vec(c, wd.p, ow));
+  HIPCHK(c, hipMemcpy(h, hd.p, sizeof(double) * ((size_t)nvec + 1), hipMemcpyDeviceToHost));
+  for (int k = 0; k < c->nvo; k++) {
+    const int v = c->iperm[k], d = c->dim;
+    for (int i = 0; i < d; i++) { z[(size_t)d * v + i] = o[(size_t)d * k + i]; w[(size_t)d * v + i] = ow[(size_t)d * k + i]; }
+    z[(size_t)d * c->nv + v] = o[(size_t)d * c->nvo + k];
+    w[(size_t)d * c->nv + v] = ow[(size_t)d * c->nvo + k];
   }
   return 0;
 }
@@ -1216,6 +1251,7 @@
   int rc = 0;
   if (hipSetDevice(device) != hipSuccess) rc = cfdh_fail(nullptr, CFDH_E_HIP, "hipSetDevice(%d) failed", device);
   else if (hipStreamCreateWithFlags(&c->stream, hipStreamNonBlocking) != hipSuccess) rc = cfdh_fail(nullptr, CFDH_E_HIP, "hipStreamCreate failed");
+  else if ((rc = k_upload_switches(c)) != 0) {}
   else rc = cfdh_ipcs_create(c, gdim, nn, nvert, nc, cells, node_coords, nfacets, facet_cells, facet_local, facet_marker);
   if (rc) {
     g_cfdh_last_error = c->err.empty() ? g_cfdh_last_error : c->err;
diff --git a/cfd_hemodynamic_amd/csrc/cfdh_internal.hpp b/cfd_hemodynamic_amd/csrc/cfdh_internal.hpp
--- a/cfd_hemodynamic_amd/csrc/cfdh_internal.hpp
+++ b/cfd_hemodynamic_amd/csrc/cfdh_internal.hpp
@@ -31,6 +31,11 @@
   return y;
 }
 #endif
+
+__host__ __device__ __forceinline__ int xcd_block(int b, int nb) {
+  const int x = b & 7, q = nb >> 3, r = nb & 7;
+  return x * q + (x < r ? x : r) + (b >> 3);
+}
 
 template <class T>
 struct dbuf {
@@ -256,6 +261,10 @@
   dbuf<double> cheb_coef;
   struct PcGraph { const double *r; double *z; hipGraphExec_t exec[6]; };
   std::vector<PcGraph> pc_graphs;
+  dbuf<double> a01q;
+  double *a01q_out = nullptr;
+  const double *a01q_r = nullptr, *a01q_z = nullptr;
+  bool a01q_captured = false;
   bool pc_graph_valid = false, capturing = false, use_graph = true;
   AmgHier hS;
   AmgHier hL;
@@ -424,11 +433,13 @@
 void prof_flush(cfdh_ctx *c);
 
 int k_upload_quadrature(cfdh_ctx *c);
+int k_upload_switches(cfdh_ctx *c);
 int k_halo_pack(cfdh_ctx *c, const double *vec);
 int v_pointwise_mult(cfdh_ctx *c, int n, const double *a, const double *b, double *out);
 int k_moments(cfdh_ctx *c);
 int k_assemble(cfdh_ctx *c, const double *xstate, int mode);
 int k_spmv_full(cfdh_ctx *c, const double *x, double *y);
+int k_spmv_full_reuse(cfdh_ctx *c, const double *x, const double *qu, double *y);
 int k_spmv_full_multi(cfdh_ctx *c, const double *X, double *Y, int ld, int nvec);
 int k_spmv_block(cfdh_ctx *c, int blk, const double *x, double *y, const double *b, double alpha);
 int k_spmv_block_ghost(cfdh_ctx *c, int blk, const double *xv, double *y, const double *b);
@@ -484,6 +495,7 @@
 
 int cfdh_pc_update(cfdh_ctx *c, bool force_refresh);
 int cfdh_pc_apply(cfdh_ctx *c, const double *r, double *z);
+int cfdh_iter_product(cfdh_ctx *c, const double *r, const double *z, double *w);
 int cfdh_host_threads();
 int cfdh_fgmres(cfdh_ctx *c, const double *b, double *x, int *its, int *reason, double bnorm = -1.0);
 int v_norm2_pair(cfdh_ctx *c, int n, const double *x, const double *y, double *nx, double *ny);
diff --git a/cfd_hemodynamic_amd/csrc/cfdh_kernels.hip b/cfd_hemodynamic_amd/csrc/cfdh_kernels.hip
--- a/cfd_hemodynamic_amd/csrc/cfdh_kernels.hip
+++ b/cfd_hemodynamic_amd/csrc/cfdh_kernels.hip
@@ -10,6 +10,16 @@
 
 __constant__ double d_qw[CFDH_NQ];
 __constant__ double d_ql[CFDH_NQ][3];
+
+__constant__ int d_xcd_map = 1;
+__device__ __forceinline__ int logical_block() {
+  return d_xcd_map ? xcd_block((int)blockIdx.x, (int)gridDim.x) : (int)blockIdx.x;
+}
+int k_upload_switches(cfdh_ctx *c) {
+  static const int on = !(getenv("CFDH_XCD_MAP") && getenv("CFDH_XCD_MAP")[0] == '0');
+  HIPCHK(c, hipMemcpyToSymbol(HIP_SYMBOL(d_xcd_map), &on, sizeof(int)));
+  return 0;
+}
 
 int k_upload_quadrature(cfdh_ctx *c) {
   HIPCHK(c, hipMemcpyToSymbol(HIP_SYMBOL(d_qw), CFDH_QW, sizeof(CFDH_QW)));
@@ -562,7 +572,7 @@
                                                         const double *__restrict__ A01, const double *__restrict__ A10,
                                                         const double *__restrict__ A11, const double *__restrict__ x,
                                                         double *__restrict__ y) {
-  const int gid = blockIdx.x * TPB + threadIdx.x;
+  const int gid = logical_block() * TPB + threadIdx.x;
   const int row = gid >> 3, l = gid & 7;
   double a0 = 0, a1 = 0, a2 = 0;
   if (row < nvo) {
@@ -592,7 +602,7 @@
                                                               const double *__restrict__ A00, const double *__restrict__ A01,
                                                               const double *__restrict__ A10, const double *__restrict__ A11,
                                                               const double *__restrict__ X, double *__restrict__ Y, size_t ld) {
-  const int gid = blockIdx.x * TPB + threadIdx.x;
+  const int gid = logical_block() * TPB + threadIdx.x;
   const int row = gid >> 3, l = gid & 7;
   double a0[NV], a1[NV], a2[NV];
 #pragma unroll
@@ -653,11 +663,49 @@
   return 0;
 }
 
+__global__ __launch_bounds__(TPB) void spmv_full_reuse_kernel(int nvo, const int *__restrict__ vptr, const int *__restrict__ vcol,
+                                                              const double *__restrict__ A00, const double *__restrict__ A10,
+                                                              const double *__restrict__ A11, const double *__restrict__ x,
+                                                              const double *__restrict__ q, double *__restrict__ y) {
+  const int gid = logical_block() * TPB + threadIdx.x;
+  const int row = gid >> 3, l = gid & 7;
+  double a0 = 0, a1 = 0, a2 = 0;
+  double2 qq = make_double2(0.0, 0.0);
+  if (row < nvo) {
+    const int ks = vptr[row], ke = vptr[row + 1];
+    if (l == 0) qq = *(const double2 *)(q + 2 * (size_t)row);
+    for (int k = ks + l; k < ke; k += 8) {
+      const int w = vcol[k];
+      const double2 xu = *(const double2 *)(x + 2 * (size_t)w);
+      const double xp = x[2 * (size_t)nvo + w];
+      const double2 b0 = *(const double2 *)(A00 + 4 * (size_t)k), b1 = *(const double2 *)(A00 + 4 * (size_t)k + 2);
+      const double2 c10 = *(const double2 *)(A10 + 2 * (size_t)k);
+      const double c11 = A11[k];
+      a0 += b0.x * xu.x + b0.y * xu.y;
+      a1 += b1.x * xu.x + b1.y * xu.y;
+      a2 += c10.x * xu.x + c10.y * xu.y + c11 * xp;
+    }
+  }
+  a0 = group8_sum(a0); a1 = group8_sum(a1); a2 = group8_sum(a2);
+  if (row < nvo && l == 0) {
+    *(double2 *)(y + 2 * (size_t)row) = make_double2(a0 + qq.x, a1 + qq.y);
+    y[2 * (size_t)nvo + row] = a2;
+  }
+}
+int k_spmv_full_reuse(cfdh_ctx *c, const double *x, const double *qu, double *y) {
+  if (c->dim == 3 || c->gen || c->nranks > 1 || c->nvo != c->nv) return cfdh_fail(c, CFDH_E_STATE, "k_spmv_full_reuse: one rank, 2-D P1 only");
+  const long long nthreads = 8ll * c->nvo;
+  hipLaunchKernelGGL(spmv_full_reuse_kernel, dim3((unsigned)((nthreads + TPB - 1) / TPB)), dim3(TPB), 0, c->stream, c->nvo,
+                     c->vptr.p, c->vcol.p, c->A00.p, c->A10.p, c->A11.p, x, qu, y);
+  HIPCHK(c, hipGetLastError());
+  return 0;
+}
+
 template <int BLK, int MODE>
 __global__ __launch_bounds__(TPB) void spmv_blk_kernel(int nvo, const int *__restrict__ vptr, const int *__restrict__ vcol,
                                                        const double *__restrict__ A, const double *__restrict__ x,
                                                        double *__restrict__ y, const double *__restrict__ bvec) {
-  const int gid = blockIdx.x * TPB + threadIdx.x;
+  const int gid = logical_block() * TPB + threadIdx.x;
   const int row = gid >> 3, l = gid & 7;
   double a0 = 0, a1 = 0;
   if (row < nvo) {
@@ -697,8 +745,9 @@
 
 __global__ __launch_bounds__(TPB) void spmv_a01_resid_kernel(int nvo, const int *__restrict__ vptr, const int *__restrict__ vcol,
                                                              const double *__restrict__ A, const double *__restrict__ x,
-                                                             double *__restrict__ y, const double *__restrict__ bvec) {
-  const int gid = blockIdx.x * TPB + threadIdx.x;
+                                                             double *__restrict__ y, const double *__restrict__ bvec,
+                                                             double *__restrict__ qout) {
+  const int gid = logical_block() * TPB + threadIdx.x;
   const int row = gid >> 2, l = gid & 3;
   double a0 = 0, a1 = 0;
   double2 bb = make_double2(0.0, 0.0);
@@ -722,14 +771,17 @@
     }
   }
   a0 = quad_sum(a0); a1 = quad_sum(a1);
-  if (row < nvo && l == 0) *(double2 *)(y + 2 * (size_t)row) = make_double2(bb.x - a0, bb.y - a1);
+  if (row < nvo && l == 0) {
+    *(double2 *)(y + 2 * (size_t)row) = make_double2(bb.x - a0, bb.y - a1);
+    if (qout) *(double2 *)(qout + 2 * (size_t)row) = make_double2(a0, a1);
+  }
 }
 
 template <int GB>
 __global__ __launch_bounds__(TPB) void spmv_blk_ghost_kernel(int nvo, const int *__restrict__ vptr, const int *__restrict__ vcol,
                                                              const double *__restrict__ A, const double *__restrict__ xv,
                                                              double *__restrict__ y, const double *__restrict__ bvec) {
-  const int gid = blockIdx.x * TPB + threadIdx.x;
+  const int gid = logical_block() * TPB + threadIdx.x;
   const int row = gid >> 3, l = gid & 7;
   double a0 = 0, a1 = 0;
   if (row < nvo) {
@@ -778,7 +830,7 @@
     if (mode) {
       const long long n4 = 4ll * c->nvo;
       hipLaunchKernelGGL(spmv_a01_resid_kernel, dim3((unsigned)((n4 + TPB - 1) / TPB)), block, 0, c->stream, c->nvo, c->vptr.p,
-                         c->vcol.p, c->A01.p, x, y, b);
+                         c->vcol.p, c->A01.p, x, y, b, c->a01q_out);
     } else {
       LAUNCH_BLK(2, 0, c->A01.p);
     }
@@ -814,7 +866,7 @@
                                                             double *__restrict__ dnew, double *__restrict__ x,
                                                             const double *__restrict__ coef, int kstep) {
   const double c1 = coef[2 * kstep], c2 = coef[2 * kstep + 1], itheta = coef[0];
-  const int gid = blockIdx.x * TPB + threadIdx.x;
+  const int gid = logical_block() * TPB + threadIdx.x;
   const int row = gid >> 3, l = gid & 7;
   double a0 = 0, a1 = 0;
   if (row < nvo) {
@@ -958,7 +1010,7 @@
 __global__ __launch_bounds__(TPB) void csr_spmv_kernel(int n, const int *__restrict__ rowptr, const int *__restrict__ col,
                                                        const double *__restrict__ val, const T *__restrict__ x,
                                                        T *__restrict__ y, const T *__restrict__ b) {
-  const int gid = blockIdx.x * TPB + threadIdx.x;
+  const int gid = logical_block() * TPB + threadIdx.x;
   const int row = gid >> 3, l = gid & 7;
   T a = vzero((const T *)nullptr);
   if (row < n) {
@@ -1000,7 +1052,7 @@
                                                             const double *__restrict__ rin, double *__restrict__ rout,
                                                             const double *__restrict__ dold, double *__restrict__ dnew,
                                                             double *__restrict__ x, double c1, double c2, double itheta) {
-  const int gid = blockIdx.x * TPB + threadIdx.x;
+  const int gid = logical_block() * TPB + threadIdx.x;
   const int row = gid >> 3, l = gid & 7;
   double a = 0;
   if (row < n) {
@@ -1027,7 +1079,7 @@
                                                              const double *__restrict__ val, const double *__restrict__ dinv,
                                                              const double *__restrict__ b, const double *__restrict__ x,
                                                              double *__restrict__ r, double *__restrict__ d0, double itheta) {
-  const int gid = blockIdx.x * TPB + threadIdx.x;
+  const int gid = logical_block() * TPB + threadIdx.x;
   const int row = gid >> 3, l = gid & 7;
   double a = 0;
   if (row < n) {
@@ -1090,7 +1142,7 @@
                                                                const double *__restrict__ dinv, const double *__restrict__ b,
                                                                double *__restrict__ x, const double *__restrict__ ml,
                                                                double *__restrict__ y, double c1, double c2) {
-  const int row = blockIdx.x * TPB + threadIdx.x;
+  const int row = logical_block() * TPB + threadIdx.x;
   if (row >= n) return;
   const int sl = row >> 6, lane = row & 63;
   const int p0 = sptr[sl], w = (sptr[sl + 1] - p0) >> 6;
@@ -1127,7 +1179,7 @@
 __global__ __launch_bounds__(TPB) void jacobi_pre_kernel(int n, const int *__restrict__ rowptr, const int *__restrict__ col,
                                                          const double *__restrict__ val, const double *__restrict__ wdinv,
                                                          const T *__restrict__ b, T *__restrict__ xa, T *__restrict__ r) {
-  const int gid = blockIdx.x * TPB + threadIdx.x;
+  const int gid = logical_block() * TPB + threadIdx.x;
   const int row = gid >> 3, l = gid & 7;
   T a = vzero((const T *)nullptr);
   if (row < n) {
@@ -1149,7 +1201,7 @@
                                                           const double *__restrict__ val, const double *__restrict__ wdinv,
                                                           const T *__restrict__ b, const T *__restrict__ xin,
                                                           T *__restrict__ xout) {
-  const int gid = blockIdx.x * TPB + threadIdx.x;
+  const int gid = logical_block() * TPB + threadIdx.x;
   const int row = gid >> 3, l = gid & 7;
   T a = vzero((const T *)nullptr);
   if (row < n) {
@@ -1166,7 +1218,7 @@
 __global__ __launch_bounds__(TPB) void sell_spmv_kernel(int n, const int *__restrict__ sptr, const int *__restrict__ scol,
                                                         const float *__restrict__ sval, const T *__restrict__ x,
                                                         T *__restrict__ y, const T *__restrict__ b) {
-  const int row = blockIdx.x * TPB + threadIdx.x;
+  const int row = logical_block() * TPB + threadIdx.x;
   if (row >= n) return;
   const int sl = row >> 6, lane = row & 63;
   const int p0 = sptr[sl], w = (sptr[sl + 1] - p0) >> 6;
@@ -1185,7 +1237,7 @@
 __global__ __launch_bounds__(TPB) void sell_jacobi_pre_kernel(int n, const int *__restrict__ sptr, const int *__restrict__ scol,
                                                               const float *__restrict__ svalw, const double *__restrict__ wdinv,
                                                               const T *__restrict__ b, T *__restrict__ xa, T *__restrict__ r) {
-  const int row = blockIdx.x * TPB + threadIdx.x;
+  const int row = logical_block() * TPB + threadIdx.x;
   if (row >= n) return;
   const int sl = row >> 6, lane = row & 63;
   const int p0 = sptr[sl], w = (sptr[sl + 1] - p0) >> 6;
@@ -1204,7 +1256,7 @@
                                                                const float *__restrict__ sval, const double *__restrict__ wdinv,
                                                                const T *__restrict__ b, const T *__restrict__ xin,
                                                                T *__restrict__ xout) {
-  const int row = blockIdx.x * TPB + threadIdx.x;
+  const int row = logical_block() * TPB + threadIdx.x;
   if (row >= n) return;
   const int sl = row >> 6, lane = row & 63;
   const int p0 = sptr[sl], w = (sptr[sl + 1] - p0) >> 6;
@@ -1291,7 +1343,7 @@
 template <int LPR, typename VT, typename T>
 __global__ __launch_bounds__(TPB) void fused_down_kernel(int n, const int *__restrict__ rowptr, const int *__restrict__ col,
                                                          const VT *__restrict__ val, const T *__restrict__ x, T *__restrict__ y) {
-  const int gid = blockIdx.x * TPB + threadIdx.x;
+  const int gid = logical_block() * TPB + threadIdx.x;
   const int row = gid / LPR, l = gid % LPR;
   T a = vzero((const T *)nullptr);
   if (row < n) {
@@ -1317,7 +1369,7 @@
                                                            const double *__restrict__ vlC, const T *__restrict__ xc,
                                                            T *__restrict__ x, double ea, double eb, const double *__restrict__ ezH,
                                                            const double *__restrict__ er, const unsigned char *__restrict__ epbc) {
-  const int gid = blockIdx.x * TPB + threadIdx.x;
+  const int gid = logical_block() * TPB + threadIdx.x;
   const int row = gid >> 3, l = gid & 7;
   T a = vzero((const T *)nullptr);
   if (row < n) {
@@ -1355,7 +1407,7 @@
                                                             const float *__restrict__ svC, const T *__restrict__ xc,
                                                             T *__restrict__ x, double ea, double eb, const double *__restrict__ ezH,
                                                             const double *__restrict__ er, const unsigned char *__restrict__ epbc) {
-  const int row = blockIdx.x * TPB + threadIdx.x;
+  const int row = logical_block() * TPB + threadIdx.x;
   if (row >= n) return;
   const int sl = __builtin_amdgcn_readfirstlane(row >> 6), lane = row & 63;
   T a = vzero((const T *)nullptr);
@@ -1395,7 +1447,7 @@
                                                              const double *__restrict__ vlB, const T *__restrict__ b,
                                                              const float *__restrict__ D, int nc, const T *__restrict__ bc,
                                                              T *__restrict__ x) {
-  const int gid = blockIdx.x * TPB + threadIdx.x;
+  const int gid = logical_block() * TPB + threadIdx.x;
   const int row = gid >> 6, l = gid & 63;
   T a = vzero((const T *)nullptr);
   if (row < n) {
diff --git a/cfd_hemodynamic_amd/csrc/cfdh_solver.cpp b/cfd_hemodynamic_amd/csrc/cfdh_solver.cpp
--- a/cfd_hemodynamic_amd/csrc/cfdh_solver.cpp
+++ b/cfd_hemodynamic_amd/csrc/cfdh_solver.cpp
@@ -492,6 +492,12 @@
     c->n_pc_builds++;
   }
   return 0;
+}
+
+static bool a01_reuse(const cfdh_ctx *c) {
+  static const bool on = !(getenv("CFDH_REUSE_A01") && getenv("CFDH_REUSE_A01")[0] == '0');
+  return on && c->nranks <= 1 && c->dim == 2 && !c->gen && c->nvo == c->nv && c->opt.pc_type == 1 && c->opt.schur_full != 0 &&
+         !c->singular && c->a01q.p != nullptr;
 }
 
 static bool ras_ghost_rhs() {
@@ -622,7 +628,12 @@
       case 3:
         if (c->opt.schur_full) {
           if (multi) CHK(k_spmv_block_ghost(c, 2, c->pcw.p, c->ras ? c->pcw.p : c->pu0.p, ru));
-          else CHK(k_spmv_block(c, 2, zp, c->pu0.p, ru, 0));
+          else {
+            c->a01q_out = a01_reuse(c) ? c->a01q.p : nullptr;
+            const int rc = k_spmv_block(c, 2, zp, c->pu0.p, ru, 0);
+            c->a01q_out = nullptr;
+            CHK(rc);
+          }
           if (multi && c->ras) {
             if (!ras_ghost_rhs()) CHK(v_zero(c, c->NL - c->NO, c->pcw.p + c->NO));
           }
@@ -697,6 +708,14 @@
   const bool graph = c->use_graph && !c->prof_on;
   const bool multi = c->nranks > 1 && c->opt.pc_type == 1;
   if (multi && !c->pcw.p) { HIPCHK(c, c->pcw.alloc(c->NL)); HIPCHK(c, c->pcw.zero(c->stream)); }
+  if (!multi && !c->a01q.p && c->dim == 2 && !c->gen) {
+    c->pc_graph_valid = false;
+    HIPCHK(c, c->a01q.alloc(2 * (size_t)c->nvo));
+  }
+  const bool reuse = a01_reuse(c);
+  if (graph && c->pc_graph_valid && reuse != c->a01q_captured) c->pc_graph_valid = false;
+  c->a01q_captured = reuse;
+  c->a01q_r = c->a01q_z = nullptr;
   if (!graph) {
     for (int st = 0; st < 6; st++) { CHK(pc_stage(c, r, z, st)); CHK(pc_exchange(c, st)); }
   } else {
@@ -734,7 +753,14 @@
     }
   }
   if (c->singular) CHK(v_sub_mean(c, nvo, z + (size_t)c->dim * nvo));
-  return 0;
+  if (reuse) { c->a01q_r = r; c->a01q_z = z; }
+  return 0;
+}
+
+int cfdh_iter_product(cfdh_ctx *c, const double *r, const double *z, double *w) {
+  const bool reuse = c->a01q_r == r && c->a01q_z == z && r != nullptr;
+  c->a01q_r = c->a01q_z = nullptr;
+  return reuse ? k_spmv_full_reuse(c, z, c->a01q.p, w) : k_spmv_full(c, z, w);
 }
 
 static int ensure_krylov(cfdh_ctx *c) {
@@ -996,7 +1022,7 @@
       double *slot = c->h_ring_dev + (size_t)(jj % cfdh_ctx::KRING) * rs;
       CHK(cfdh_pc_apply(c, vj, zj));
       CHK(comm_halo(c, zj));
-      CHK(k_spmv_full(c, zj, w));
+      CHK(cfdh_iter_product(c, vj, zj, w));
       if (use32) {
         CHK(v_multidot32(c, n, V32, (int)ld32, jj + 1, w, hd, slot));
         CHK(v_gs_update32(c, n, V32, (int)ld32, jj + 1, hd, w, vn, V32 + (size_t)(jj + 1) * ld32, s_dev, slot + (jj + 2)));
@@ -1028,7 +1054,7 @@
         const bool refine = !(nrm2 > eta2 * ww);
         double hnorm;
         if (refine) {
-          if (jl > j + 1) { c->n_krylov_discarded += jl - (j + 1); jl = j + 1; }
+          if (jl > j + 1) { c->n_krylov_discarded += jl - (j + 1); jl = j + 1; upto = jl; }
           CHK(v_multidot(c, n, V, (int)ld, j + 1, vn, hd + (m + 2), true));
           CHK(v_multiaxpy(c, n, V, (int)ld, j + 1, hd + (m + 2), vn));
           if (use32) CHK(v_norm_to_dev(c, n, vn, hd + 2 * (m + 2)));
diff --git a/include/cfdh.h b/include/cfdh.h
--- a/include/cfdh.h
+++ b/include/cfdh.h
@@ -112,6 +112,8 @@
 int cfdh_get_newton_history(cfdh_ctx *ctx, int32_t *n, double *fnorm, double *ksp_rtol, int32_t *ksp_its, double *ksp_rel_res);
 int cfdh_get_pcd_operator(cfdh_ctx *ctx, int64_t *nnz, int32_t *rowptr, int32_t *col, double *vals, double *mass_diag);
 int cfdh_apply_preconditioner(cfdh_ctx *ctx, const double *r, double *z);
+int cfdh_apply_iteration_operator(cfdh_ctx *ctx, const double *R, int nvec, double *z, double *w, double *h);
+int cfdh_xcd_block(int b, int nb);
 
 #define CFDH_AMG_HIER_A 0
 #define CFDH_AMG_HIER_P 1
```

After: 417.0. About the same (-0.9%).
